# simdjson/simdjson

Hardware: NVIDIA H100
Metric: stage1 GB/s (bytes in / s) vs HBM roofline at 1/2/4/8 H100; CPU ref GB/s (higher is better)
Workload: dtype u8

## Files before the change

include/sjb200.h:

```cpp
#ifndef SJB200_H
#define SJB200_H

#include <stddef.h>
#include <stdint.h>

#if defined(__GNUC__)
#define SJB200_API __attribute__((visibility("default")))
#else
#define SJB200_API
#endif

#ifdef __cplusplus
extern "C" {
#endif

enum {
  SJB200_SUCCESS = 0,
  SJB200_CAPACITY = 1,
  SJB200_MEMALLOC = 2,
  SJB200_UTF8_ERROR = 11,
  SJB200_EMPTY = 13,
  SJB200_UNESCAPED_CHARS = 14,
  SJB200_UNCLOSED_STRING = 15,
  SJB200_UNSUPPORTED_ARCHITECTURE = 16,
  SJB200_UNEXPECTED_ERROR = 24
};

enum {
  SJB200_REGULAR = 0,
  SJB200_STREAMING_PARTIAL = 1,
  SJB200_STREAMING_FINAL = 2,
  SJB200_JSON_SEQUENCE_PARTIAL = 3,
  SJB200_JSON_SEQUENCE_FINAL = 4,
  SJB200_COMMA_DELIMITED_PARTIAL = 5,
  SJB200_COMMA_DELIMITED_FINAL = 6
};

typedef struct sjb200_ctx sjb200_ctx;

SJB200_API int sjb200_create(int device, size_t capacity_bytes, sjb200_ctx **out);
SJB200_API void sjb200_destroy(sjb200_ctx *ctx);
SJB200_API int sjb200_set_capacity(sjb200_ctx *ctx, size_t capacity_bytes);
SJB200_API size_t sjb200_capacity(const sjb200_ctx *ctx);
SJB200_API size_t sjb200_index_words(size_t capacity_bytes);
SJB200_API int sjb200_device(const sjb200_ctx *ctx);
SJB200_API const char *sjb200_last_cuda_error(const sjb200_ctx *ctx);
SJB200_API int sjb200_set_option(sjb200_ctx *ctx, const char *key, long value);
SJB200_API double sjb200_get_stat(sjb200_ctx *ctx, const char *key);

SJB200_API long sjb200_get_debug_timeline(sjb200_ctx *ctx, unsigned long long *out, size_t max_tiles);

SJB200_API int sjb200_pin_host_memory(sjb200_ctx *ctx, void *ptr, size_t bytes);
SJB200_API int sjb200_unpin_host_memory(sjb200_ctx *ctx, void *ptr);

SJB200_API int sjb200_stage1(sjb200_ctx *ctx, const uint8_t *buf, size_t len, int mode, uint32_t *idx_out, uint32_t *n_inout);
SJB200_API int sjb200_minify(sjb200_ctx *ctx, const uint8_t *buf, size_t len, uint8_t *dst, size_t *dst_len);
SJB200_API int sjb200_validate_utf8(sjb200_ctx *ctx, const uint8_t *buf, size_t len);

SJB200_API int sjb200_stage1_dev(sjb200_ctx *ctx, const uint8_t *d_buf, size_t len, int mode, uint32_t *d_idx, uint32_t *n_inout,
                      void *stream);
SJB200_API int sjb200_minify_dev(sjb200_ctx *ctx, const uint8_t *d_buf, size_t len, uint8_t *d_dst, size_t *dst_len, void *stream);
SJB200_API int sjb200_validate_utf8_dev(sjb200_ctx *ctx, const uint8_t *d_buf, size_t len, void *stream);

typedef struct {
  const uint8_t *d_buf;
  size_t len;
  uint32_t *d_idx;
  uint32_t n_structural_indexes;
  int error;
} sjb200_doc;
SJB200_API int sjb200_stage1_dev_batch(sjb200_ctx *ctx, sjb200_doc *docs, int ndocs, int mode, void *stream);

typedef struct {
  uint32_t index;
  uint32_t byte;
} sjb200_doc_boundary;
SJB200_API int sjb200_document_table_dev(sjb200_ctx *ctx, const uint8_t *d_buf, const uint32_t *d_idx, uint32_t n, sjb200_doc_boundary *d_table,
                              uint32_t capacity, uint32_t *ndocs_out, void *stream);

typedef struct {
  int error;
  uint32_t first_error_index;
  uint32_t n_strings;
  uint64_t string_bytes;
} sjb200_tokens_result;
SJB200_API size_t sjb200_string_buf_capacity(size_t len);
SJB200_API int sjb200_tokens_dev(sjb200_ctx *ctx, const uint8_t *d_buf, size_t len, const uint32_t *d_idx, uint32_t n, uint8_t *d_type, uint64_t *d_payload,
                      uint8_t *d_strbuf, size_t strbuf_capacity, sjb200_tokens_result *out, void *stream);

SJB200_API int sjb200_stage1_dev_enqueue(sjb200_ctx *ctx, const uint8_t *d_buf, size_t len, int mode, uint32_t *d_idx, void *stream);
SJB200_API int sjb200_stage1_dev_finish(sjb200_ctx *ctx, uint32_t *n_inout);
SJB200_API int sjb200_minify_dev_enqueue(sjb200_ctx *ctx, const uint8_t *d_buf, size_t len, uint8_t *d_dst, void *stream);
SJB200_API int sjb200_minify_dev_finish(sjb200_ctx *ctx, size_t *dst_len);
SJB200_API int sjb200_validate_utf8_dev_enqueue(sjb200_ctx *ctx, const uint8_t *d_buf, size_t len, void *stream);
SJB200_API int sjb200_validate_utf8_dev_finish(sjb200_ctx *ctx);

typedef struct {
  uint32_t ttable;
  uint32_t state_out;
  uint32_t flags;
  uint32_t reserved;
  uint64_t count;
} sjb200_shard_result;
SJB200_API int sjb200_stage1_shard_dev(sjb200_ctx *ctx, const uint8_t *d_buf, size_t len, uint32_t state_in, int last_shard,
                            uint32_t *d_idx, sjb200_shard_result *out, void *stream);
SJB200_API int sjb200_stage1_shard_dev_enqueue(sjb200_ctx *ctx, const uint8_t *d_buf, size_t len, uint32_t *d_idx, void *d_result,
                                    void *stream);
typedef struct sjb200_comm sjb200_comm;
#define SJB200_COMM_HANDLE_BYTES 64
typedef struct {
  uint64_t count;
  uint64_t base;
  uint64_t total_count;
  uint32_t state_in;
  uint32_t state_out;
  uint32_t final_state;
  uint32_t flags;
  uint32_t flags_all;
  uint32_t rescanned;
} sjb200_sharded_result;
SJB200_API int sjb200_comm_create(sjb200_ctx *ctx, int rank, int nranks , sjb200_comm **out);
SJB200_API void sjb200_comm_destroy(sjb200_comm *comm);
SJB200_API int sjb200_comm_get_handle(sjb200_comm *comm, void *handle );
SJB200_API int sjb200_comm_connect(sjb200_comm *comm, const void *handles );
SJB200_API int sjb200_comm_connect_local(sjb200_comm *comm, sjb200_comm *const *all );
SJB200_API int sjb200_stage1_sharded(sjb200_comm *comm, const uint8_t *d_shard, size_t len, int last_shard, uint32_t *d_idx,
                          sjb200_sharded_result *out, void *stream);
SJB200_API int sjb200_stage1_sharded_enqueue(sjb200_comm *comm, const uint8_t *d_shard, size_t len, int last_shard, uint32_t *d_idx,
                                  void *stream);
SJB200_API int sjb200_stage1_sharded_finish(sjb200_comm *comm, sjb200_sharded_result *out);

SJB200_API int sjb200_minify_sharded_enqueue(sjb200_comm *comm, const uint8_t *d_shard, size_t len, uint8_t *d_dst, void *stream);
SJB200_API int sjb200_minify_sharded_finish(sjb200_comm *comm, sjb200_sharded_result *out);
SJB200_API int sjb200_minify_sharded(sjb200_comm *comm, const uint8_t *d_shard, size_t len, uint8_t *d_dst, sjb200_sharded_result *out,
                          void *stream);
SJB200_API int sjb200_validate_utf8_sharded_enqueue(sjb200_comm *comm, const uint8_t *d_shard, size_t len, void *stream);
SJB200_API int sjb200_validate_utf8_sharded_finish(sjb200_comm *comm, sjb200_sharded_result *out);
SJB200_API int sjb200_validate_utf8_sharded(sjb200_comm *comm, const uint8_t *d_shard, size_t len, sjb200_sharded_result *out, void *stream);

typedef struct {
  sjb200_sharded_result shard;
  uint64_t n;
  uint64_t kept;
  uint64_t bytes_before;
  uint64_t total_bytes;
  uint32_t first_starts_document;
  uint32_t reserved;
} sjb200_sharded_stream_result;
SJB200_API int sjb200_stage1_sharded_stream_enqueue(sjb200_comm *comm, const uint8_t *d_shard, size_t len, int last_shard, int mode, uint32_t *d_idx,
                                         void *stream);
SJB200_API int sjb200_stage1_sharded_stream_finish(sjb200_comm *comm, sjb200_sharded_stream_result *out);
SJB200_API int sjb200_stage1_sharded_stream(sjb200_comm *comm, const uint8_t *d_shard, size_t len, int last_shard, int mode, uint32_t *d_idx,
                                 sjb200_sharded_stream_result *out, void *stream);

SJB200_API int sjb200_document_table_shard_dev(sjb200_ctx *ctx, const uint8_t *d_shard, const uint32_t *d_idx, uint32_t kept, int first_starts_document,
                                    sjb200_doc_boundary *d_table, uint32_t capacity, uint32_t *ndocs_out, void *stream);

typedef struct {
  uint64_t count;
  uint32_t len;
  uint32_t first_byte;
  uint32_t last_byte;
  uint32_t start_index;
  uint32_t start_byte;
  int32_t net_obj;
  int32_t net_arr;
  uint32_t role_first;
  uint32_t role_last;
  uint32_t has_start;
} sjb200_stream_summary;
typedef struct {
  uint64_t kept;
  uint64_t bytes_before;
  uint32_t first_starts_document;
  uint32_t nrewrites;
  uint32_t rewrite_pos[2];
  uint32_t rewrite_val[2];
} sjb200_stream_rank;
typedef struct {
  int error;
  uint32_t n_written;
  uint64_t n;
  uint64_t total_bytes;
} sjb200_stream_fold_result;
SJB200_API int sjb200_stream_fold(int mode, int nranks, uint32_t final_state, uint32_t flags_all, const sjb200_stream_summary *sums,
                       sjb200_stream_fold_result *res, sjb200_stream_rank *ranks );

SJB200_API uint32_t sjb200_fold_state(const uint32_t *ttables, int nshards_before);
SJB200_API size_t sjb200_shard_cut(const uint8_t *buf, size_t len, size_t nominal);
SJB200_API size_t sjb200_shard_cut_line(const uint8_t *buf, size_t len, size_t nominal, size_t window);

#ifdef __cplusplus
}
#endif
#endif
```

simdjson_b200/capi.py:

```python
import ctypes as C
import os

_HERE = os.path.dirname(os.path.abspath(__file__))
LIB_PATH = os.environ.get("SJB200_LIB") or os.path.join(_HERE, "libsjb200.so")

EXPORTS = [
    "sjb200_create", "sjb200_destroy", "sjb200_set_capacity", "sjb200_capacity", "sjb200_index_words", "sjb200_device",
    "sjb200_last_cuda_error", "sjb200_set_option", "sjb200_get_stat", "sjb200_pin_host_memory", "sjb200_unpin_host_memory", "sjb200_get_debug_timeline",
    "sjb200_stage1", "sjb200_minify", "sjb200_validate_utf8",
    "sjb200_stage1_dev", "sjb200_minify_dev", "sjb200_validate_utf8_dev", "sjb200_stage1_dev_batch",
    "sjb200_document_table_dev", "sjb200_stage1_dev_enqueue", "sjb200_stage1_dev_finish", "sjb200_minify_dev_enqueue", "sjb200_minify_dev_finish",
    "sjb200_validate_utf8_dev_enqueue", "sjb200_validate_utf8_dev_finish",
    "sjb200_stage1_shard_dev", "sjb200_stage1_shard_dev_enqueue", "sjb200_fold_state", "sjb200_shard_cut", "sjb200_shard_cut_line",
    "sjb200_comm_create", "sjb200_comm_destroy", "sjb200_comm_get_handle", "sjb200_comm_connect", "sjb200_comm_connect_local",
    "sjb200_stage1_sharded", "sjb200_stage1_sharded_enqueue", "sjb200_stage1_sharded_finish",
    "sjb200_minify_sharded", "sjb200_minify_sharded_enqueue", "sjb200_minify_sharded_finish",
    "sjb200_validate_utf8_sharded", "sjb200_validate_utf8_sharded_enqueue", "sjb200_validate_utf8_sharded_finish",
    "sjb200_tokens_dev", "sjb200_string_buf_capacity",
    "sjb200_stage1_sharded_stream", "sjb200_stage1_sharded_stream_enqueue", "sjb200_stage1_sharded_stream_finish",
    "sjb200_document_table_shard_dev", "sjb200_stream_fold",
]
COMM_HANDLE_BYTES = 64

SUCCESS, CAPACITY, MEMALLOC, UTF8_ERROR, EMPTY, UNESCAPED_CHARS, UNCLOSED_STRING, UNSUPPORTED_ARCHITECTURE, UNEXPECTED_ERROR = 0, 1, 2, 11, 13, 14, 15, 16, 24
ERROR_NAMES = {0: "SUCCESS", 1: "CAPACITY", 2: "MEMALLOC", 3: "TAPE_ERROR", 5: "STRING_ERROR", 6: "T_ATOM_ERROR", 7: "F_ATOM_ERROR", 8: "N_ATOM_ERROR",
               9: "NUMBER_ERROR", 10: "BIGINT_ERROR", 11: "UTF8_ERROR", 13: "EMPTY", 14: "UNESCAPED_CHARS", 15: "UNCLOSED_STRING",
               16: "UNSUPPORTED_ARCHITECTURE", 24: "UNEXPECTED_ERROR"}

REGULAR, STREAMING_PARTIAL, STREAMING_FINAL, JSON_SEQUENCE_PARTIAL, JSON_SEQUENCE_FINAL, COMMA_DELIMITED_PARTIAL, COMMA_DELIMITED_FINAL = range(7)


class Doc(C.Structure):
    _fields_ = [("d_buf", C.c_void_p), ("len", C.c_size_t), ("d_idx", C.c_void_p), ("n_structural_indexes", C.c_uint32), ("error", C.c_int)]


class TokensResult(C.Structure):
    _fields_ = [("error", C.c_int), ("first_error_index", C.c_uint32), ("n_strings", C.c_uint32), ("string_bytes", C.c_uint64)]


class ShardResult(C.Structure):
    _fields_ = [("ttable", C.c_uint32), ("state_out", C.c_uint32), ("flags", C.c_uint32), ("reserved", C.c_uint32), ("count", C.c_uint64)]


class ShardedResult(C.Structure):
    _fields_ = [("count", C.c_uint64), ("base", C.c_uint64), ("total_count", C.c_uint64), ("state_in", C.c_uint32), ("state_out", C.c_uint32),
                ("final_state", C.c_uint32), ("flags", C.c_uint32), ("flags_all", C.c_uint32), ("rescanned", C.c_uint32)]


class ShardedStreamResult(C.Structure):
    _fields_ = [("shard", ShardedResult), ("n", C.c_uint64), ("kept", C.c_uint64), ("bytes_before", C.c_uint64), ("total_bytes", C.c_uint64),
                ("first_starts_document", C.c_uint32), ("reserved", C.c_uint32)]


class StreamSummary(C.Structure):
    _fields_ = [("count", C.c_uint64), ("len", C.c_uint32), ("first_byte", C.c_uint32), ("last_byte", C.c_uint32), ("start_index", C.c_uint32),
                ("start_byte", C.c_uint32), ("net_obj", C.c_int32), ("net_arr", C.c_int32), ("role_first", C.c_uint32), ("role_last", C.c_uint32),
                ("has_start", C.c_uint32)]


class StreamRank(C.Structure):
    _fields_ = [("kept", C.c_uint64), ("bytes_before", C.c_uint64), ("first_starts_document", C.c_uint32), ("nrewrites", C.c_uint32),
                ("rewrite_pos", C.c_uint32 * 2), ("rewrite_val", C.c_uint32 * 2)]


class StreamFoldResult(C.Structure):
    _fields_ = [("error", C.c_int), ("n_written", C.c_uint32), ("n", C.c_uint64), ("total_bytes", C.c_uint64)]


def load():
    if not os.path.exists(LIB_PATH):
        raise ImportError(
            f"{LIB_PATH} is missing: build it with `python -c 'import __graft_entry__ as g; g.build()'` "
            "(nvcc, sm_90a).  simdjson_b200 has no CPU fallback.")
    L = C.CDLL(LIB_PATH)
    u8p, u32p, vp, sz = C.POINTER(C.c_uint8), C.POINTER(C.c_uint32), C.c_void_p, C.c_size_t
    sig = {
        "sjb200_create": (C.c_int, [C.c_int, sz, C.POINTER(vp)]),
        "sjb200_destroy": (None, [vp]),
        "sjb200_set_capacity": (C.c_int, [vp, sz]),
        "sjb200_capacity": (sz, [vp]),
        "sjb200_index_words": (sz, [sz]),
        "sjb200_device": (C.c_int, [vp]),
        "sjb200_last_cuda_error": (C.c_char_p, [vp]),
        "sjb200_set_option": (C.c_int, [vp, C.c_char_p, C.c_long]),
        "sjb200_get_stat": (C.c_double, [vp, C.c_char_p]),
        "sjb200_get_debug_timeline": (C.c_long, [vp, vp, sz]),
        "sjb200_pin_host_memory": (C.c_int, [vp, vp, sz]),
        "sjb200_unpin_host_memory": (C.c_int, [vp, vp]),
        "sjb200_stage1": (C.c_int, [vp, vp, sz, C.c_int, vp, u32p]),
        "sjb200_minify": (C.c_int, [vp, vp, sz, vp, C.POINTER(sz)]),
        "sjb200_validate_utf8": (C.c_int, [vp, vp, sz]),
        "sjb200_stage1_dev": (C.c_int, [vp, vp, sz, C.c_int, vp, u32p, vp]),
        "sjb200_minify_dev": (C.c_int, [vp, vp, sz, vp, C.POINTER(sz), vp]),
        "sjb200_validate_utf8_dev": (C.c_int, [vp, vp, sz, vp]),
        "sjb200_stage1_dev_batch": (C.c_int, [vp, C.POINTER(Doc), C.c_int, C.c_int, vp]),
        "sjb200_document_table_dev": (C.c_int, [vp, vp, vp, C.c_uint32, vp, C.c_uint32, u32p, vp]),
        "sjb200_stage1_dev_enqueue": (C.c_int, [vp, vp, sz, C.c_int, vp, vp]),
        "sjb200_stage1_dev_finish": (C.c_int, [vp, u32p]),
        "sjb200_minify_dev_enqueue": (C.c_int, [vp, vp, sz, vp, vp]),
        "sjb200_minify_dev_finish": (C.c_int, [vp, C.POINTER(sz)]),
        "sjb200_validate_utf8_dev_enqueue": (C.c_int, [vp, vp, sz, vp]),
        "sjb200_validate_utf8_dev_finish": (C.c_int, [vp]),
        "sjb200_stage1_shard_dev": (C.c_int, [vp, vp, sz, C.c_uint32, C.c_int, vp, C.POINTER(ShardResult), vp]),
        "sjb200_stage1_shard_dev_enqueue": (C.c_int, [vp, vp, sz, vp, vp, vp]),
        "sjb200_fold_state": (C.c_uint32, [u32p, C.c_int]),
        "sjb200_shard_cut": (sz, [vp, sz, sz]),
        "sjb200_shard_cut_line": (sz, [vp, sz, sz, sz]),
        "sjb200_comm_create": (C.c_int, [vp, C.c_int, C.c_int, C.POINTER(vp)]),
        "sjb200_comm_destroy": (None, [vp]),
        "sjb200_comm_get_handle": (C.c_int, [vp, vp]),
        "sjb200_comm_connect": (C.c_int, [vp, vp]),
        "sjb200_comm_connect_local": (C.c_int, [vp, C.POINTER(vp)]),
        "sjb200_stage1_sharded": (C.c_int, [vp, vp, sz, C.c_int, vp, C.POINTER(ShardedResult), vp]),
        "sjb200_stage1_sharded_enqueue": (C.c_int, [vp, vp, sz, C.c_int, vp, vp]),
        "sjb200_stage1_sharded_finish": (C.c_int, [vp, C.POINTER(ShardedResult)]),
        "sjb200_minify_sharded": (C.c_int, [vp, vp, sz, vp, C.POINTER(ShardedResult), vp]),
        "sjb200_minify_sharded_enqueue": (C.c_int, [vp, vp, sz, vp, vp]),
        "sjb200_minify_sharded_finish": (C.c_int, [vp, C.POINTER(ShardedResult)]),
        "sjb200_validate_utf8_sharded": (C.c_int, [vp, vp, sz, C.POINTER(ShardedResult), vp]),
        "sjb200_validate_utf8_sharded_enqueue": (C.c_int, [vp, vp, sz, vp]),
        "sjb200_validate_utf8_sharded_finish": (C.c_int, [vp, C.POINTER(ShardedResult)]),
        "sjb200_tokens_dev": (C.c_int, [vp, vp, sz, vp, C.c_uint32, vp, vp, vp, sz, C.POINTER(TokensResult), vp]),
        "sjb200_string_buf_capacity": (sz, [sz]),
        "sjb200_stage1_sharded_stream": (C.c_int, [vp, vp, sz, C.c_int, C.c_int, vp, C.POINTER(ShardedStreamResult), vp]),
        "sjb200_stage1_sharded_stream_enqueue": (C.c_int, [vp, vp, sz, C.c_int, C.c_int, vp, vp]),
        "sjb200_stage1_sharded_stream_finish": (C.c_int, [vp, C.POINTER(ShardedStreamResult)]),
        "sjb200_document_table_shard_dev": (C.c_int, [vp, vp, vp, C.c_uint32, C.c_int, vp, C.c_uint32, u32p, vp]),
        "sjb200_stream_fold": (C.c_int, [C.c_int, C.c_int, C.c_uint32, C.c_uint32, C.POINTER(StreamSummary), C.POINTER(StreamFoldResult),
                                         C.POINTER(StreamRank)]),
    }
    for name, (res, args) in sig.items():
        fn = getattr(L, name)
        fn.restype = res
        fn.argtypes = args
    _ = u8p
    return L
```

simdjson_b200/csrc/sjb200_capi.cu:

```cuda
#include <cuda.h>
#include <cuda_runtime.h>
#include <ctype.h>
#include <stdint.h>
#include <stdlib.h>
#include <string.h>

#include <algorithm>
#include <chrono>
#include <new>
#include <string>
#include <vector>

#include "../../include/sjb200.h"
#include "sjb200_bits.cuh"
#include "sjb200_docs.h"
#include "sjb200_tape.h"
#include "sjb200_finish.h"
#include "sjb200_hostpipe.h"
#include "sjb200_kernels.cuh"

using namespace sjb200;

namespace {

typedef CUresult (*PFN_encodeTiled)(CUtensorMap *, CUtensorMapDataType, cuuint32_t, void *, const cuuint64_t *, const cuuint64_t *,
                                    const cuuint32_t *, const cuuint32_t *, CUtensorMapInterleave, CUtensorMapSwizzle,
                                    CUtensorMapL2promotion, CUtensorMapFloatOOBfill);

constexpr int kCarrySlots = 1024;
constexpr size_t kMaxBytes = 0xFFFFFFFFull;

struct PendingCall {
  int kind = -1;
  int mode = 0;
  int early_error = -1;
  size_t len = 0;
  const uint8_t *d_buf = nullptr;
  uint32_t *d_idx = nullptr;
  uint8_t *d_dst = nullptr;
  cudaStream_t stream = nullptr;
  int carry_slot = 0;
};

}

struct sjb200_ctx {
  int device = 0;
  int sm_count = 0;
  size_t capacity = 0;
  cudaStream_t stream = nullptr;
  cudaStream_t copy_stream = nullptr;
  cudaStream_t out_stream = nullptr;
  std::vector<cudaEvent_t> chunk_events;
  uint8_t *d_in = nullptr;    size_t d_in_bytes = 0;
  uint32_t *d_idx = nullptr;  size_t d_idx_words = 0;
  uint8_t *d_out = nullptr;   size_t d_out_bytes = 0;
  Carry *d_carry = nullptr;
  uint32_t *d_flags = nullptr;
  uint32_t *d_ticket = nullptr;
  unsigned long long *d_count_desc = nullptr;
  size_t desc_tiles = 0;
  StreamFinish *d_sfin = nullptr;
  uint32_t *d_doc_scratch = nullptr; size_t doc_scratch_words = 0; uint32_t *d_ndocs = nullptr;
  void *d_tok_scratch = nullptr; size_t tok_scratch_bytes = 0; TokenTotals *d_tok_tot = nullptr;
  uint32_t *d_park = nullptr; size_t d_park_words = 0;
  int grid_u = 0;
  Carry *h_carry = nullptr;
  uint32_t *h_flags = nullptr;
  uint8_t *h_small = nullptr;
  StreamFinish *h_sfin = nullptr;
  uint8_t *h_tails = nullptr; uint8_t *d_tails = nullptr; const uint8_t **d_tail_ptrs = nullptr; size_t tails_cap = 0;
  uint32_t epoch = 0;
  int grid4 = 0;
  long opt_tok_stage = 1;
  long opt_use_tma = 1, opt_grid = 0, opt_chunk_bytes = 4 << 20, opt_time_kernel = 0;
  cudaEvent_t ev_k0 = nullptr, ev_k1 = nullptr;
  bool ev_valid = false;
  std::vector<cudaEvent_t> ev_pool;
  std::vector<uint32_t> ev_docs;
  size_t ev_used = 0;
  uint32_t ev_last_docs = 1;
  uint8_t *h_doctab = nullptr; uint8_t *d_doctab = nullptr; size_t doctab_bytes = 0;
  long opt_debug_timeline = 0;
  unsigned long long *d_debug = nullptr; size_t debug_tiles = 0; uint32_t debug_last_tiles = 0;
  unsigned long long launches = 0;
  unsigned long long ew_launches = 0;
  PFN_encodeTiled encode = nullptr;
  uint8_t *h_ring = nullptr; size_t ring_slot_bytes = 0; int ring_slots = 0;
  std::vector<cudaEvent_t> ring_events;
  CopyPool *pool = nullptr;
  long opt_force_grid = 0;
  long opt_ew_min_bytes = 0;
  long opt_host_skip_scan = 0;
  long opt_copy_threads = 4;
  long opt_ring_slots = 8;
  long opt_first_chunk_bytes = 512 << 10;
  long opt_stage_min_bytes = 1 << 20;
  long opt_zero_copy_out = 1;
  unsigned long long xchg_polls = 0, xchg_second_rounds = 0;
  double xchg_wait_ms = 0, xchg_evsync_ms = 0, xchg_enqueue_ms = 0;
  double t_wait_ms = 0, t_issue_ms = 0, t_sync_ms = 0;
  int last_input_path = 0, last_output_path = 0;
  PendingCall pending;
  std::string last_error;
};

namespace {

struct DeviceGuard {
  int prev = -1;
  explicit DeviceGuard(int dev) {
    cudaGetDevice(&prev);
    if (prev != dev) cudaSetDevice(dev);
  }
  ~DeviceGuard() {
    int cur = -1;
    cudaGetDevice(&cur);
    if (prev >= 0 && cur != prev) cudaSetDevice(prev);
  }
};

bool ok(sjb200_ctx *c, cudaError_t e, const char *what) {
  if (e == cudaSuccess) return true;
  c->last_error = std::string(what) + ": " + cudaGetErrorString(e);
  (void)cudaGetLastError();
  return false;
}

size_t index_words(size_t capacity) { return ((capacity + 63) / 64) * 64 + 9; }
uint32_t tiles_of(size_t len) { return uint32_t((len + kTileBytes - 1) / kTileBytes); }

template <typename T>
bool dev_alloc(sjb200_ctx *c, T **p, size_t count, const char *what) {
  void *q = nullptr;
  if (!ok(c, cudaMalloc(&q, count * sizeof(T)), what)) return false;
  *p = static_cast<T *>(q);
  return true;
}

void free_sized(sjb200_ctx *c) {
  cudaFree(c->d_in); c->d_in = nullptr; c->d_in_bytes = 0;
  cudaFree(c->d_idx); c->d_idx = nullptr; c->d_idx_words = 0;
  cudaFree(c->d_out); c->d_out = nullptr; c->d_out_bytes = 0;
  cudaFree(c->d_count_desc); c->d_count_desc = nullptr;
  c->desc_tiles = 0;
}

bool ensure_desc_n(sjb200_ctx *c, size_t need) {
  need = std::max<size_t>(need, 1);
  if (need <= c->desc_tiles) return true;
  cudaFree(c->d_count_desc); c->d_count_desc = nullptr;
  c->desc_tiles = 0;
  const size_t n = std::max(need, size_t(tiles_of(c->capacity)) + 1);
  if (!dev_alloc(c, &c->d_count_desc, n, "cudaMalloc(count_desc)")) return false;
  if (!ok(c, cudaMemsetAsync(c->d_count_desc, 0, n * sizeof(unsigned long long), c->stream), "memset desc")) return false;
  if (!ok(c, cudaStreamSynchronize(c->stream), "sync")) return false;
  c->desc_tiles = n;
  c->epoch = 0;
  return true;
}
bool ensure_desc(sjb200_ctx *c, size_t len) { return ensure_desc_n(c, tiles_of(len)); }

bool next_epoch(sjb200_ctx *c, cudaStream_t launch_stream, uint32_t *epoch) {
  c->epoch++;
  if (c->epoch >= (1u << 18)) {
    if (!ok(c, cudaMemsetAsync(c->d_count_desc, 0, c->desc_tiles * sizeof(unsigned long long), launch_stream), "memset desc")) return false;
    c->epoch = 1;
  }
  *epoch = c->epoch;
  return true;
}

bool make_tensor_map(sjb200_ctx *c, CUtensorMap *map, const uint8_t *d_buf, size_t len, bool *usable, int box_rows = kScan4BoxRows) {
  memset(map, 0, sizeof(*map));
  *usable = false;
  const uint64_t rows = len / 128;
  if (!c->opt_use_tma || c->encode == nullptr || rows == 0) return true;
  if ((reinterpret_cast<uintptr_t>(d_buf) & 15u) != 0) return true;
  cuuint64_t dims[2] = {128, rows};
  cuuint64_t strides[1] = {128};
  cuuint32_t box[2] = {128, (cuuint32_t)box_rows};
  cuuint32_t estr[2] = {1, 1};
  CUresult r = c->encode(map, CU_TENSOR_MAP_DATA_TYPE_UINT8, 2, const_cast<uint8_t *>(d_buf), dims, strides, box, estr,
                         CU_TENSOR_MAP_INTERLEAVE_NONE, CU_TENSOR_MAP_SWIZZLE_128B, CU_TENSOR_MAP_L2_PROMOTION_L2_256B,
                         CU_TENSOR_MAP_FLOAT_OOB_FILL_NONE);
  if (r != CUDA_SUCCESS) {
    c->last_error = "cuTensorMapEncodeTiled failed (" + std::to_string(int(r)) + "); using plain loads";
    return true;
  }
  *usable = true;
  return true;
}

bool use_scan4(const sjb200_ctx *, int kind) { return kind == kIndex || kind == kMinify; }
bool map_for(sjb200_ctx *c, int kind, CUtensorMap *map, const uint8_t *d_buf, size_t len, bool *usable) {
  (void)kind;
  return make_tensor_map(c, map, d_buf, len, usable, kScan4BoxRows);
}
int grid_cap(sjb200_ctx *c, int kind) {
  (void)kind;
  if (c->grid4 == 0) c->grid4 = scan4_max_ctas_per_sm() * c->sm_count;
  return c->opt_grid > 0 ? int(c->opt_grid) : c->grid4;
}
int grid_for(sjb200_ctx *c, int kind, uint32_t nelements) {
  if (c->opt_force_grid > 0) return int(c->opt_force_grid);
  return int(std::max<uint32_t>(1, std::min<uint32_t>(uint32_t(grid_cap(c, kind)), nelements)));
}

struct XchgTarget {
  unsigned long long *peer[kMaxRanks];
  uint32_t nranks, rank, slot, seq, kind;
};

cudaEvent_t time_begin(sjb200_ctx *c, cudaStream_t stream) {
  if (!c->opt_time_kernel) return nullptr;
  if (c->ev_used + 2 > c->ev_pool.size() && c->ev_pool.size() < 4096) {
    cudaEvent_t a, b;
    cudaEventCreate(&a); cudaEventCreate(&b);
    c->ev_pool.push_back(a); c->ev_pool.push_back(b);
    c->ev_docs.push_back(1);
  }
  if (c->ev_used + 2 > c->ev_pool.size()) return nullptr;
  cudaEventRecord(c->ev_pool[c->ev_used], stream);
  c->ev_used += 2;
  return c->ev_pool[c->ev_used - 1];
}
void time_end(sjb200_ctx *c, cudaStream_t stream, cudaEvent_t e1, bool launched, uint32_t docs) {
  if (!e1) return;
  cudaEventRecord(e1, stream);
  c->ev_docs[c->ev_used / 2 - 1] = docs;
  c->ev_k0 = c->ev_pool[c->ev_used - 2]; c->ev_k1 = e1; c->ev_valid = launched; c->ev_last_docs = docs;
}

bool enqueue_scan(sjb200_ctx *c, int kind, const CUtensorMap *map, bool tma, const uint8_t *d_buf, size_t len, uint32_t tile_begin,
                  uint32_t ntiles, bool has_last_tile, uint32_t prev_word, uint32_t *d_idx, uint8_t *d_dst, int carry_in_slot,
                  cudaStream_t stream, int carry_out_slot = -1, bool write_sentinels = false, Carry *external_out = nullptr,
                  Carry *host_out = nullptr, const XchgTarget *xchg = nullptr) {
  if (carry_out_slot < 0) carry_out_slot = (carry_in_slot < 0) ? 1 : (carry_in_slot ^ 1);
  ScanParams p;
  memset(&p, 0, sizeof(p));
  p.buf = d_buf;
  p.len = len;
  p.pos_base = 0;
  p.prev_word = prev_word;
  p.check_eof = has_last_tile ? 1u : 0u;
  p.use_tma = tma ? 1u : 0u;
  p.tile_begin = tile_begin;
  p.ntiles = ntiles;
  if (!next_epoch(c, stream, &p.epoch)) return false;
  p.idx_out = d_idx;
  p.dst = d_dst;
  p.carry_in = (carry_in_slot < 0) ? nullptr : c->d_carry + carry_in_slot;
  p.write_sentinels = write_sentinels ? 1u : 0u;
  p.carry_out = external_out ? external_out : c->d_carry + carry_out_slot;
  p.carry_out_host = use_scan4(c, kind) ? host_out : nullptr;
  p.flags = c->d_flags;
  p.count_desc = c->d_count_desc;
  p.ticket = c->d_ticket;
  if (xchg) {
    for (int r = 0; r < kMaxRanks; r++) p.xchg_peer[r] = xchg->peer[r];
    p.xchg_nranks = xchg->nranks; p.xchg_rank = xchg->rank; p.xchg_slot = xchg->slot; p.xchg_seq = xchg->seq; p.xchg_kind = xchg->kind;
  }
  p.debug = nullptr;
  if (c->opt_debug_timeline) {
    const uint32_t rows = std::max<uint32_t>(ntiles, 4096);
    if (c->debug_tiles < rows) {
      cudaFree(c->d_debug); c->d_debug = nullptr; c->debug_tiles = 0;
      if (dev_alloc(c, &c->d_debug, size_t(rows) * 8, "cudaMalloc(debug)")) c->debug_tiles = rows;
    }
    if (c->d_debug) { cudaMemsetAsync(c->d_debug, 0, size_t(rows) * 64, stream); p.debug = c->d_debug; c->debug_last_tiles = rows; }
  }
  cudaEvent_t e1 = time_begin(c, stream);
  bool launched;
  if (use_scan4(c, kind)) {
    const uint32_t tpe = uint32_t(scan4_tiles_per_element());
    const uint32_t nelem = (ntiles + tpe - 1) / tpe;
    const int grid = grid_for(c, kind, nelem);
    const bool ew = kind == kIndex && c->opt_ew_min_bytes > 0 && uint64_t(ntiles) * kTileBytes >= uint64_t(c->opt_ew_min_bytes);
    if (ew || scan4_parks_in_global()) {
      const size_t need = std::max(ew ? scan4_ew_park_words(grid_cap(c, kind)) : 0, scan4_parks_in_global() ? scan4_park_words(grid_cap(c, kind)) : 0);
      if (c->d_park_words < need) {
        cudaStreamSynchronize(c->stream);
        cudaFree(c->d_park); c->d_park = nullptr; c->d_park_words = 0;
        if (!dev_alloc(c, &c->d_park, need, "cudaMalloc(park)")) return false;
        c->d_park_words = need;
      }
      p.park = c->d_park;
    }
    launched = ew ? ok(c, launch_scan4_ew(map, p, grid, stream), "launch scan4 (emit warps)") : ok(c, launch_scan4(map, p, grid, kind == kMinify ? 2 : 0, stream), "launch scan4");
    c->ew_launches += (launched && ew) ? 1 : 0;
  } else {
    if (c->grid_u == 0) c->grid_u = utf8v2_max_ctas_per_sm() * c->sm_count;
    const uint64_t nblocks = (uint64_t(ntiles) * kTileBytes + 4095) / 4096;
    const uint64_t want = (nblocks + uint64_t(utf8v2_warps_per_cta()) - 1) / uint64_t(utf8v2_warps_per_cta());
    const int grid = c->opt_force_grid > 0 ? int(c->opt_force_grid) : int(std::max<uint64_t>(1, std::min<uint64_t>(uint64_t(c->opt_grid > 0 ? c->opt_grid : c->grid_u), want)));
    p.carry_out_host = host_out;
    launched = ok(c, launch_utf8v2(map, p, grid, stream), "launch utf8v2");
  }
  time_end(c, stream, e1, launched, 1);
  c->launches += launched ? 1 : 0;
  return launched;
}

class NullIndexWriter final : public IndexWriter {
 public:
  bool set3(uint32_t, uint32_t, uint32_t, uint32_t) override { return false; }
  bool final_fixup(uint32_t, uint32_t) override { return false; }
};
class NullReader final : public StructuralReader {
 public:
  uint32_t position(uint32_t) override { return 0; }
  uint8_t character(uint32_t) override { return 0; }
};

bool is_filter_mode(int mode) { return mode >= SJB200_JSON_SEQUENCE_PARTIAL; }

bool fetch_result(sjb200_ctx *c, cudaStream_t s) {
  return ok(c, cudaMemcpyAsync(c->h_carry + 1, c->d_carry + 1, sizeof(Carry), cudaMemcpyDeviceToHost, s), "D2H result");
}

}

extern "C" size_t sjb200_index_words(size_t capacity) { return index_words(capacity); }

extern "C" int sjb200_create(int device, size_t capacity, sjb200_ctx **out) {
  if (!out) return SJB200_UNEXPECTED_ERROR;
  *out = nullptr;
  int ndev = 0;
  if (cudaGetDeviceCount(&ndev) != cudaSuccess || device < 0 || device >= ndev) {
    (void)cudaGetLastError();
    return SJB200_UNSUPPORTED_ARCHITECTURE;
  }
  cudaDeviceProp prop;
  if (cudaGetDeviceProperties(&prop, device) != cudaSuccess || prop.major != 9 || prop.minor != 0) {
    (void)cudaGetLastError();
    return SJB200_UNSUPPORTED_ARCHITECTURE;
  }
  sjb200_ctx *c = new (std::nothrow) sjb200_ctx();
  if (!c) return SJB200_MEMALLOC;
  c->device = device;
  c->sm_count = prop.multiProcessorCount;
  DeviceGuard g(device);
  bool good = ok(c, cudaStreamCreateWithFlags(&c->stream, cudaStreamNonBlocking), "stream") &&
              ok(c, cudaStreamCreateWithFlags(&c->copy_stream, cudaStreamNonBlocking), "stream") &&
              ok(c, cudaStreamCreateWithFlags(&c->out_stream, cudaStreamNonBlocking), "stream") &&
              dev_alloc(c, &c->d_carry, kCarrySlots, "cudaMalloc(carry)") && dev_alloc(c, &c->d_flags, 1 + kCarrySlots, "cudaMalloc(flags)") &&
              dev_alloc(c, &c->d_ticket, 4, "cudaMalloc(ticket)") &&
              ok(c, cudaMemset(c->d_ticket, 0, 4 * sizeof(uint32_t)), "memset ticket") &&
              ok(c, cudaMemset(c->d_flags, 0, (1 + kCarrySlots) * sizeof(uint32_t)), "memset flags");
  void *hp = nullptr;
  good = good && ok(c, cudaMallocHost(&hp, kCarrySlots * sizeof(Carry)), "cudaMallocHost");
  c->h_carry = static_cast<Carry *>(hp);
  good = good && ok(c, cudaMallocHost(&hp, sizeof(uint32_t)), "cudaMallocHost");
  c->h_flags = static_cast<uint32_t *>(hp);
  good = good && ok(c, cudaMallocHost(&hp, 64), "cudaMallocHost");
  c->h_small = static_cast<uint8_t *>(hp);
  good = good && ok(c, cudaMallocHost(&hp, kCarrySlots * sizeof(StreamFinish)), "cudaMallocHost");
  c->h_sfin = static_cast<StreamFinish *>(hp);
  good = good && dev_alloc(c, &c->d_sfin, kCarrySlots, "cudaMalloc(stream finish)") && dev_alloc(c, &c->d_ndocs, 1, "cudaMalloc(ndocs)");
  if (good) {
    void *fn = nullptr;
    cudaDriverEntryPointQueryResult qres;
    if (cudaGetDriverEntryPoint("cuTensorMapEncodeTiled", &fn, cudaEnableDefault, &qres) == cudaSuccess &&
        qres == cudaDriverEntryPointSuccess)
      c->encode = reinterpret_cast<PFN_encodeTiled>(fn);
    else
      (void)cudaGetLastError();
  }
  if (!good) {
    sjb200_destroy(c);
    return SJB200_MEMALLOC;
  }
  for (const char *key : {"copy_threads", "ring_slots", "chunk_bytes", "first_chunk_bytes", "stage_min_bytes", "zero_copy_out"}) {
    std::string env = std::string("SJB200_") + key;
    for (auto &ch : env) ch = char(toupper((unsigned char)ch));
    if (const char *v = getenv(env.c_str())) sjb200_set_option(c, key, atol(v));
  }
  int rc = sjb200_set_capacity(c, capacity);
  if (rc != SJB200_SUCCESS) {
    sjb200_destroy(c);
    return rc;
  }
  *out = c;
  return SJB200_SUCCESS;
}

extern "C" void sjb200_destroy(sjb200_ctx *c) {
  if (!c) return;
  DeviceGuard g(c->device);
  if (c->stream) cudaStreamSynchronize(c->stream);
  free_sized(c);
  cudaFree(c->d_carry); cudaFree(c->d_flags); cudaFree(c->d_ticket); cudaFree(c->d_sfin); cudaFree(c->d_doc_scratch); cudaFree(c->d_ndocs); cudaFree(c->d_tok_scratch); cudaFree(c->d_tok_tot); cudaFree(c->d_tails); cudaFree(c->d_tail_ptrs); cudaFree(c->d_debug); cudaFree(c->d_park); cudaFree(c->d_doctab);
  if (c->h_doctab) cudaFreeHost(c->h_doctab);
  if (c->h_carry) cudaFreeHost(c->h_carry);
  if (c->h_flags) cudaFreeHost(c->h_flags);
  if (c->h_small) cudaFreeHost(c->h_small);
  if (c->h_sfin) cudaFreeHost(c->h_sfin);
  if (c->h_tails) cudaFreeHost(c->h_tails);
  delete c->pool; c->pool = nullptr;
  if (c->h_ring) cudaFreeHost(c->h_ring);
  for (auto e : c->ring_events) cudaEventDestroy(e);
  for (auto e : c->ev_pool) cudaEventDestroy(e);
  for (auto e : c->chunk_events) cudaEventDestroy(e);
  if (c->stream) cudaStreamDestroy(c->stream);
  if (c->copy_stream) cudaStreamDestroy(c->copy_stream);
  if (c->out_stream) cudaStreamDestroy(c->out_stream);
  delete c;
}

extern "C" int sjb200_set_capacity(sjb200_ctx *c, size_t capacity) {
  if (!c) return SJB200_UNEXPECTED_ERROR;
  if (capacity > kMaxBytes) return SJB200_CAPACITY;
  DeviceGuard g(c->device);
  if (capacity != c->capacity) {
    cudaStreamSynchronize(c->stream);
    free_sized(c);
  }
  c->capacity = capacity;
  if (!ensure_desc(c, capacity)) return SJB200_MEMALLOC;
  return SJB200_SUCCESS;
}

extern "C" size_t sjb200_capacity(const sjb200_ctx *c) { return c ? c->capacity : 0; }
extern "C" int sjb200_device(const sjb200_ctx *c) { return c ? c->device : -1; }
extern "C" const char *sjb200_last_cuda_error(const sjb200_ctx *c) { return c ? c->last_error.c_str() : ""; }

extern "C" long sjb200_get_debug_timeline(sjb200_ctx *c, unsigned long long *out, size_t max_tiles) {
  if (!c || !c->d_debug || !out) return 0;
  DeviceGuard g(c->device);
  const size_t n = std::min<size_t>(max_tiles, c->debug_last_tiles);
  cudaDeviceSynchronize();
  if (cudaMemcpy(out, c->d_debug, n * 64, cudaMemcpyDeviceToHost) != cudaSuccess) { (void)cudaGetLastError(); return 0; }
  return long(n);
}

extern "C" int sjb200_pin_host_memory(sjb200_ctx *c, void *ptr, size_t bytes) {
  if (!c || !ptr || bytes == 0) return SJB200_UNEXPECTED_ERROR;
  DeviceGuard g(c->device);
  return ok(c, cudaHostRegister(ptr, bytes, cudaHostRegisterPortable | cudaHostRegisterMapped), "cudaHostRegister") ? SJB200_SUCCESS : SJB200_MEMALLOC;
}
extern "C" int sjb200_unpin_host_memory(sjb200_ctx *c, void *ptr) {
  if (!c || !ptr) return SJB200_UNEXPECTED_ERROR;
  DeviceGuard g(c->device);
  return ok(c, cudaHostUnregister(ptr), "cudaHostUnregister") ? SJB200_SUCCESS : SJB200_UNEXPECTED_ERROR;
}

extern "C" double sjb200_get_stat(sjb200_ctx *c, const char *key) {
  if (!c || !key) return -1.0;
  if (!strcmp(key, "kernel_ms")) {
    if (!c->ev_valid) return -1.0;
    DeviceGuard g(c->device);
    float ms = 0.f;
    if (cudaEventElapsedTime(&ms, c->ev_k0, c->ev_k1) != cudaSuccess) { (void)cudaGetLastError(); return -1.0; }
    return double(ms) / double(c->ev_last_docs);
  }
  if (!strcmp(key, "kernel_ms_mean")) {
    DeviceGuard g(c->device);
    double sum = 0;
    size_t n = 0;
    for (size_t i = 0; i + 1 < c->ev_used; i += 2) {
      float ms = 0.f;
      if (cudaEventElapsedTime(&ms, c->ev_pool[i], c->ev_pool[i + 1]) == cudaSuccess) { sum += ms; n += c->ev_docs[i / 2]; } else (void)cudaGetLastError();
    }
    c->ev_used = 0;
    c->ev_valid = false;
    return n ? sum / double(n) : -1.0;
  }
  if (!strcmp(key, "launches")) return double(c->launches);
  if (!strcmp(key, "ew_launches")) return double(c->ew_launches);
  if (!strcmp(key, "grid_index")) return double(grid_for(c, kIndex, 0xFFFFFFFFu));
  if (!strcmp(key, "sm_count")) return double(c->sm_count);
  if (!strcmp(key, "host_wait_ms")) return c->t_wait_ms;
  if (!strcmp(key, "xchg_polls")) return double(c->xchg_polls);
  if (!strcmp(key, "xchg_second_rounds")) return double(c->xchg_second_rounds);
  if (!strcmp(key, "xchg_wait_ms")) return c->xchg_wait_ms;
  if (!strcmp(key, "xchg_evsync_ms")) return c->xchg_evsync_ms;
  if (!strcmp(key, "xchg_enqueue_ms")) return c->xchg_enqueue_ms;
  if (!strcmp(key, "host_issue_ms")) return c->t_issue_ms;
  if (!strcmp(key, "host_sync_ms")) return c->t_sync_ms;
  if (!strcmp(key, "input_path")) return double(c->last_input_path);
  if (!strcmp(key, "output_path")) return double(c->last_output_path);
  return -1.0;
}

extern "C" int sjb200_set_option(sjb200_ctx *c, const char *key, long value) {
  if (!c || !key) return SJB200_UNEXPECTED_ERROR;
  if (!strcmp(key, "use_tma")) c->opt_use_tma = value;
  else if (!strcmp(key, "grid")) c->opt_grid = value;
  else if (!strcmp(key, "tok_stage")) c->opt_tok_stage = value ? 1 : 0;
  else if (!strcmp(key, "time_kernel")) c->opt_time_kernel = value;
  else if (!strcmp(key, "debug_timeline")) c->opt_debug_timeline = value;
  else if (!strcmp(key, "chunk_bytes")) c->opt_chunk_bytes = std::max<long>(2 * kTileBytes, (value / (2 * kTileBytes)) * (2 * kTileBytes));
  else if (!strcmp(key, "force_grid")) c->opt_force_grid = value;
  else if (!strcmp(key, "ew_min_bytes")) c->opt_ew_min_bytes = value;
  else if (!strcmp(key, "host_skip_scan")) c->opt_host_skip_scan = value;
  else if (!strcmp(key, "copy_threads")) c->opt_copy_threads = std::max<long>(0, std::min<long>(value, 64));
  else if (!strcmp(key, "ring_slots")) c->opt_ring_slots = std::max<long>(2, std::min<long>(value, 64));
  else if (!strcmp(key, "stage_min_bytes")) c->opt_stage_min_bytes = std::max<long>(0, value);
  else if (!strcmp(key, "first_chunk_bytes")) c->opt_first_chunk_bytes = std::max<long>(2 * kTileBytes, (value / (2 * kTileBytes)) * (2 * kTileBytes));
  else if (!strcmp(key, "zero_copy_out")) c->opt_zero_copy_out = value;
  else return SJB200_UNEXPECTED_ERROR;
  return SJB200_SUCCESS;
}

namespace {
bool stage1_prepare(sjb200_ctx *c, PendingCall &pc, const uint8_t *d_buf, size_t len, int mode, uint32_t *d_idx, cudaStream_t s, int slot,
                    const uint8_t *tail3 ) {
  pc = PendingCall();
  pc.kind = kIndex; pc.mode = mode; pc.d_buf = d_buf; pc.d_idx = d_idx; pc.stream = s; pc.len = len; pc.carry_slot = slot;
  if (mode < SJB200_REGULAR || mode > SJB200_COMMA_DELIMITED_FINAL) { pc.early_error = SJB200_UNEXPECTED_ERROR; return false; }
  if (len > c->capacity) { pc.early_error = SJB200_CAPACITY; return false; }
  if (len == 0) { pc.early_error = SJB200_EMPTY; return false; }
  if (mode != SJB200_REGULAR) {
    const size_t k = std::min<size_t>(3, len);
    if (!tail3) {
      if (!ok(c, cudaMemcpyAsync(c->h_small, d_buf + len - k, k, cudaMemcpyDeviceToHost, s), "D2H tail") ||
          !ok(c, cudaStreamSynchronize(s), "sync"))
        { pc.early_error = SJB200_UNEXPECTED_ERROR; return false; }
      tail3 = c->h_small;
    }
    len = trim_partial_utf8_tail(tail3, k, len);
    pc.len = len;
    if (len == 0) { pc.early_error = SJB200_UTF8_ERROR; return false; }
  }
  return true;
}

void stage1_stream_epilogue(sjb200_ctx *c, PendingCall &pc) {
  if (pc.mode == SJB200_STREAMING_PARTIAL || pc.mode == SJB200_STREAMING_FINAL) {
    c->launches++;
    const int slot = pc.carry_slot;
    if (!ok(c, launch_stream_finish(pc.d_buf, pc.d_idx, c->d_carry + slot, uint32_t(pc.len), pc.mode, c->d_sfin + slot, c->h_sfin + slot, pc.stream), "stream finish"))
      pc.early_error = SJB200_UNEXPECTED_ERROR;
  }
}

void stage1_enqueue_into(sjb200_ctx *c, PendingCall &pc, const uint8_t *d_buf, size_t len, int mode, uint32_t *d_idx, cudaStream_t s, int slot) {
  if (!stage1_prepare(c, pc, d_buf, len, mode, d_idx, s, slot, nullptr)) return;
  len = pc.len;
  if (!ensure_desc(c, len)) { pc.early_error = SJB200_MEMALLOC; return; }
  CUtensorMap map;
  bool tma = false;
  map_for(c, kIndex, &map, d_buf, len, &tma);
  if (!enqueue_scan(c, kIndex, &map, tma, d_buf, len, 0, tiles_of(len), true, 0x20202020u, d_idx, nullptr, -1, s, slot, true, nullptr,
                    c->h_carry + slot) ||
      (!use_scan4(c, kIndex) &&
       !ok(c, cudaMemcpyAsync(c->h_carry + slot, c->d_carry + slot, sizeof(Carry), cudaMemcpyDeviceToHost, s), "D2H result")))
    { pc.early_error = SJB200_UNEXPECTED_ERROR; return; }
  stage1_stream_epilogue(c, pc);
}

int stage1_finish_from(sjb200_ctx *c, const PendingCall &pc, uint32_t *n_inout) {
  if (pc.early_error >= 0) return pc.early_error;
  if (pc.mode == SJB200_STREAMING_PARTIAL || pc.mode == SJB200_STREAMING_FINAL) {
    const StreamFinish &r = c->h_sfin[pc.carry_slot];
    if (r.n_written && n_inout) *n_inout = r.n;
    return r.err;
  }
  FinishInput in;
  in.mode = pc.mode; in.len = pc.len;
  in.count = c->h_carry[pc.carry_slot].count;
  in.state = c->h_carry[pc.carry_slot].state;
  in.flags = c->h_carry[pc.carry_slot].flags;
  in.sentinels_written = true;
  int rc;
  uint32_t n_local = n_inout ? *n_inout : 0;
  if (is_filter_mode(pc.mode)) {
    if (in.flags & kFlagInternal) return SJB200_UNEXPECTED_ERROR;
    if (in.flags & kFlagCtl) return SJB200_UNESCAPED_CHARS;
    uint32_t n = uint32_t(in.count);
    n_local = n;
    if (n == 0) { if (n_inout) *n_inout = 0; return SJB200_EMPTY; }
    const bool unclosed = (in.state >> 1) & 1u;
    const bool partial = (pc.mode == SJB200_JSON_SEQUENCE_PARTIAL || pc.mode == SJB200_COMMA_DELIMITED_PARTIAL);
    if (unclosed) {
      n--;
      if (partial) { n_local = n; if (n == 0) { if (n_inout) *n_inout = 0; return SJB200_CAPACITY; } }
    }
    const size_t need = filter_scratch_words(n);
    if (c->doc_scratch_words < need) {
      cudaFree(c->d_doc_scratch); c->d_doc_scratch = nullptr; c->doc_scratch_words = 0;
      if (!dev_alloc(c, &c->d_doc_scratch, need, "cudaMalloc(filter scratch)")) return SJB200_MEMALLOC;
      c->doc_scratch_words = need;
    }
    c->launches += 4;
    if (!ok(c, launch_stream_filter(pc.d_buf, uint32_t(pc.len), pc.d_idx, n, pc.mode, in.flags, c->d_doc_scratch, c->d_sfin + pc.carry_slot,
                                    c->h_sfin + pc.carry_slot, pc.stream), "stream filter") ||
        !ok(c, cudaStreamSynchronize(pc.stream), "sync"))
      return SJB200_UNEXPECTED_ERROR;
    const StreamFinish &r = c->h_sfin[pc.carry_slot];
    if (n_inout) *n_inout = r.n;
    return r.err;
  } else {
    NullReader reader;
    NullIndexWriter writer;
    bool dirty = false;
    rc = finish_stage1(in, reader, writer, &n_local, nullptr, nullptr, &dirty);
  }
  if (n_inout) *n_inout = n_local;
  return rc;
}

}

extern "C" int sjb200_stage1_dev_enqueue(sjb200_ctx *c, const uint8_t *d_buf, size_t len, int mode, uint32_t *d_idx, void *stream) {
  if (!c) return SJB200_UNEXPECTED_ERROR;
  DeviceGuard g(c->device);
  stage1_enqueue_into(c, c->pending, d_buf, len, mode, d_idx, stream ? static_cast<cudaStream_t>(stream) : c->stream, 1);
  return SJB200_SUCCESS;
}

extern "C" int sjb200_stage1_dev_finish(sjb200_ctx *c, uint32_t *n_inout) {
  if (!c || c->pending.kind != kIndex) return SJB200_UNEXPECTED_ERROR;
  DeviceGuard g(c->device);
  PendingCall pc = c->pending;
  c->pending.kind = -1;
  if (pc.early_error < 0 && !ok(c, cudaStreamSynchronize(pc.stream), "sync")) return SJB200_UNEXPECTED_ERROR;
  return stage1_finish_from(c, pc, n_inout);
}

namespace {
bool ranges_overlap(const void *a, size_t an, const void *b, size_t bn) {
  const uintptr_t x = reinterpret_cast<uintptr_t>(a), y = reinterpret_cast<uintptr_t>(b);
  return x < y + bn && y < x + an;
}
size_t out_bytes(const PendingCall &pc) { return 4 * (pc.len + 3); }

int enqueue_doc_groups(sjb200_ctx *c, std::vector<PendingCall> &calls, cudaStream_t s) {
  constexpr uint64_t kMaxGroupElems = 1u << 20;
  const uint32_t tpe = uint32_t(scan4_tiles_per_element());
  auto elems_of = [&](const PendingCall &pc) { return uint64_t((tiles_of(pc.len) + tpe - 1) / tpe); };
  std::vector<std::vector<int>> groups;
  uint64_t g_elems = 0, max_elems = 0;
  for (int i = 0; i < int(calls.size()); i++) {
    const PendingCall &pc = calls[size_t(i)];
    if (pc.early_error >= 0) continue;
    bool split = groups.empty() || groups.back().size() == size_t(kMaxLaunchDocs) || g_elems + elems_of(pc) > kMaxGroupElems;
    for (size_t k = 0; !split && k < groups.back().size(); k++) {
      const PendingCall &q = calls[size_t(groups.back()[k])];
      split = ranges_overlap(pc.d_buf, pc.len, q.d_idx, out_bytes(q)) || ranges_overlap(pc.d_idx, out_bytes(pc), q.d_idx, out_bytes(q)) ||
              ranges_overlap(pc.d_idx, out_bytes(pc), q.d_buf, q.len);
    }
    if (split) { groups.emplace_back(); g_elems = 0; }
    groups.back().push_back(i);
    g_elems += elems_of(pc);
    max_elems = std::max(max_elems, g_elems);
  }
  if (groups.empty()) return SJB200_SUCCESS;
  if (!ensure_desc_n(c, max_elems)) return SJB200_MEMALLOC;
  std::vector<size_t> off(groups.size() + 1, 0);
  for (size_t g = 0; g < groups.size(); g++) {
    const size_t n = groups[g].size() > 1 ? groups[g].size() : 0;
    off[g + 1] = off[g] + ((n * sizeof(DocEntry) + 127) & ~size_t(127)) + n * sizeof(CUtensorMap);
  }
  if (off.back() > c->doctab_bytes) {
    if (c->h_doctab) cudaFreeHost(c->h_doctab);
    cudaFree(c->d_doctab);
    c->h_doctab = nullptr; c->d_doctab = nullptr; c->doctab_bytes = 0;
    void *hp = nullptr;
    if (!ok(c, cudaMallocHost(&hp, off.back()), "cudaMallocHost(doc tables)") || !dev_alloc(c, &c->d_doctab, off.back(), "cudaMalloc(doc tables)"))
      return SJB200_MEMALLOC;
    c->h_doctab = static_cast<uint8_t *>(hp);
    c->doctab_bytes = off.back();
  }
  static_assert(sizeof(DocEntry) == 64 && sizeof(CUtensorMap) == 128, "table layout");
  for (size_t g = 0; g < groups.size(); g++) {
    const std::vector<int> &G = groups[g];
    if (G.size() == 1) {
      PendingCall &pc = calls[size_t(G[0])];
      CUtensorMap map;
      bool tma = false;
      map_for(c, kIndex, &map, pc.d_buf, pc.len, &tma);
      if (!enqueue_scan(c, kIndex, &map, tma, pc.d_buf, pc.len, 0, tiles_of(pc.len), true, 0x20202020u, pc.d_idx, nullptr, -1, s, pc.carry_slot, true,
                        nullptr, c->h_carry + pc.carry_slot))
        pc.early_error = SJB200_UNEXPECTED_ERROR;
      else
        stage1_stream_epilogue(c, pc);
      continue;
    }
    const size_t n = G.size();
    DocEntry *he = reinterpret_cast<DocEntry *>(c->h_doctab + off[g]);
    const size_t maps_at = off[g] + ((n * sizeof(DocEntry) + 127) & ~size_t(127));
    CUtensorMap *hm = reinterpret_cast<CUtensorMap *>(c->h_doctab + maps_at);
    const CUtensorMap *dm = reinterpret_cast<const CUtensorMap *>(c->d_doctab + maps_at);
    uint32_t elems = 0, tiles = 0;
    for (size_t k = 0; k < n; k++) {
      const PendingCall &pc = calls[size_t(G[k])];
      bool tma = false;
      map_for(c, kIndex, &hm[k], pc.d_buf, pc.len, &tma);
      DocEntry &e = he[k];
      e.buf = pc.d_buf;
      e.idx_out = pc.d_idx;
      e.carry_out = c->d_carry + pc.carry_slot;
      e.carry_out_host = c->h_carry + pc.carry_slot;
      e.flags = c->d_flags + 1 + pc.carry_slot;
      e.tmap = tma ? static_cast<const void *>(dm + k) : nullptr;
      e.len = uint32_t(pc.len);
      e.scan_end = uint32_t(pc.len);
      e.first_elem = elems;
      e.nelem = uint32_t(elems_of(pc));
      elems += e.nelem;
      tiles += tiles_of(pc.len);
    }
    ScanParams p;
    memset(&p, 0, sizeof(p));
    p.prev_word = 0x20202020u;
    p.check_eof = 1;
    p.write_sentinels = 1;
    p.ntiles = tiles;
    p.flags = c->d_flags;
    p.count_desc = c->d_count_desc;
    p.ticket = c->d_ticket;
    p.docs = reinterpret_cast<const DocEntry *>(c->d_doctab + off[g]);
    p.ndocs = uint32_t(n);
    bool good = next_epoch(c, s, &p.epoch) &&
                ok(c, cudaMemcpyAsync(c->d_doctab + off[g], c->h_doctab + off[g], off[g + 1] - off[g], cudaMemcpyHostToDevice, s), "H2D doc table");
    if (good) {
      CUtensorMap unused;
      memset(&unused, 0, sizeof(unused));
      cudaEvent_t e1 = time_begin(c, s);
      good = ok(c, launch_scan4(&unused, p, grid_for(c, kIndex, elems), 0, s), "launch scan4 (documents)");
      time_end(c, s, e1, good, uint32_t(n));
      c->launches += good ? 1 : 0;
    }
    for (size_t k = 0; k < n; k++) {
      PendingCall &pc = calls[size_t(G[k])];
      if (good) stage1_stream_epilogue(c, pc);
      else pc.early_error = SJB200_UNEXPECTED_ERROR;
    }
  }
  return SJB200_SUCCESS;
}
}

extern "C" int sjb200_stage1_dev_batch(sjb200_ctx *c, sjb200_doc *docs, int ndocs, int mode, void *stream) {
  if (!c || (!docs && ndocs > 0) || ndocs < 0) return SJB200_UNEXPECTED_ERROR;
  DeviceGuard g(c->device);
  cudaStream_t s = stream ? static_cast<cudaStream_t>(stream) : c->stream;
  std::vector<PendingCall> calls;
  int done = 0;
  while (done < ndocs) {
    const int group = std::min(ndocs - done, kCarrySlots - 2);
    calls.assign(size_t(group), PendingCall());
    const uint8_t *tails = nullptr;
    if (mode != SJB200_REGULAR) {
      if (c->tails_cap < size_t(group)) {
        if (c->h_tails) cudaFreeHost(c->h_tails);
        cudaFree(c->d_tails); cudaFree(c->d_tail_ptrs);
        c->h_tails = nullptr; c->d_tails = nullptr; c->d_tail_ptrs = nullptr; c->tails_cap = 0;
        void *hp = nullptr;
        if (!ok(c, cudaMallocHost(&hp, size_t(group) * 20), "cudaMallocHost(tails)") || !dev_alloc(c, &c->d_tails, size_t(group) * 4, "cudaMalloc(tails)") ||
            !dev_alloc(c, &c->d_tail_ptrs, size_t(group) * 2, "cudaMalloc(tail ptrs)"))
          return SJB200_MEMALLOC;
        c->h_tails = static_cast<uint8_t *>(hp);
        c->tails_cap = size_t(group);
      }
      const uint8_t **hptr = reinterpret_cast<const uint8_t **>(c->h_tails);
      uint64_t *hlen = reinterpret_cast<uint64_t *>(c->h_tails + size_t(group) * 8);
      uint8_t *hout = c->h_tails + size_t(group) * 16;
      for (int i = 0; i < group; i++) { hptr[i] = docs[done + i].d_buf; hlen[i] = (docs[done + i].len <= c->capacity) ? docs[done + i].len : 0; }
      const uint64_t *dlen = reinterpret_cast<const uint64_t *>(c->d_tail_ptrs + group);
      if (!ok(c, cudaMemcpyAsync(c->d_tail_ptrs, c->h_tails, size_t(group) * 16, cudaMemcpyHostToDevice, s), "H2D tail ptrs") ||
          !ok(c, launch_gather_tails(c->d_tail_ptrs, dlen, uint32_t(group), c->d_tails, s), "gather tails") ||
          !ok(c, cudaMemcpyAsync(hout, c->d_tails, size_t(group) * 4, cudaMemcpyDeviceToHost, s), "D2H tails") || !ok(c, cudaStreamSynchronize(s), "sync"))
        return SJB200_UNEXPECTED_ERROR;
      c->launches++;
      tails = hout;
    }
    for (int i = 0; i < group; i++) {
      sjb200_doc &d = docs[done + i];
      stage1_prepare(c, calls[size_t(i)], d.d_buf, d.len, mode, d.d_idx, s, 1 + i, tails ? tails + 4 * size_t(i) : nullptr);
    }
    const int rc = enqueue_doc_groups(c, calls, s);
    if (rc != SJB200_SUCCESS) return rc;
    if (!ok(c, cudaStreamSynchronize(s), "sync")) return SJB200_UNEXPECTED_ERROR;
    for (int i = 0; i < group; i++) {
      sjb200_doc &d = docs[done + i];
      d.error = stage1_finish_from(c, calls[size_t(i)], &d.n_structural_indexes);
    }
    done += group;
  }
  return SJB200_SUCCESS;
}

extern "C" int sjb200_document_table_dev(sjb200_ctx *c, const uint8_t *d_buf, const uint32_t *d_idx, uint32_t n, sjb200_doc_boundary *d_table,
                                         uint32_t capacity, uint32_t *ndocs_out, void *stream) {
  return sjb200_document_table_shard_dev(c, d_buf, d_idx, n, 1, d_table, capacity, ndocs_out, stream);
}

extern "C" int sjb200_document_table_shard_dev(sjb200_ctx *c, const uint8_t *d_buf, const uint32_t *d_idx, uint32_t n, int first_starts_document,
                                               sjb200_doc_boundary *d_table, uint32_t capacity, uint32_t *ndocs_out, void *stream) {
  if (!c || !d_buf || !d_idx || !ndocs_out || (capacity && !d_table)) return SJB200_UNEXPECTED_ERROR;
  *ndocs_out = 0;
  if (n == 0) return SJB200_SUCCESS;
  DeviceGuard g(c->device);
  cudaStream_t s = stream ? static_cast<cudaStream_t>(stream) : c->stream;
  const size_t need = doc_table_scratch_words(n);
  if (c->doc_scratch_words < need) {
    cudaFree(c->d_doc_scratch); c->d_doc_scratch = nullptr; c->doc_scratch_words = 0;
    if (!dev_alloc(c, &c->d_doc_scratch, need, "cudaMalloc(doc scratch)")) return SJB200_MEMALLOC;
    c->doc_scratch_words = need;
  }
  static_assert(sizeof(sjb200_doc_boundary) == sizeof(sjb200_doc_boundary_t), "layout");
  if (!ok(c, launch_doc_table(d_buf, d_idx, n, first_starts_document != 0, c->d_doc_scratch, reinterpret_cast<sjb200_doc_boundary_t *>(d_table), capacity,
                              c->d_ndocs, s), "doc table") ||
      !ok(c, cudaMemcpyAsync(c->h_small, c->d_ndocs, sizeof(uint32_t), cudaMemcpyDeviceToHost, s), "D2H ndocs") || !ok(c, cudaStreamSynchronize(s), "sync"))
    return SJB200_UNEXPECTED_ERROR;
  c->launches += 3;
  memcpy(ndocs_out, c->h_small, sizeof(uint32_t));
  return SJB200_SUCCESS;
}

extern "C" size_t sjb200_string_buf_capacity(size_t len) { return ((5 * (len / 3) + 64) + 63) / 64 * 64; }

extern "C" int sjb200_tokens_dev(sjb200_ctx *c, const uint8_t *d_buf, size_t len, const uint32_t *d_idx, uint32_t n, uint8_t *d_type, uint64_t *d_payload,
                                 uint8_t *d_strbuf, size_t strbuf_capacity, sjb200_tokens_result *out, void *stream) {
  if (!c || !out || (n && (!d_buf || !d_idx || !d_type || !d_payload)) || (strbuf_capacity && !d_strbuf)) return SJB200_UNEXPECTED_ERROR;
  out->error = SJB200_SUCCESS; out->first_error_index = 0xFFFFFFFFu; out->n_strings = 0; out->string_bytes = 0;
  DeviceGuard g(c->device);
  cudaStream_t s = stream ? static_cast<cudaStream_t>(stream) : c->stream;
  const size_t need = tokens_scratch_bytes(n);
  if (c->tok_scratch_bytes < need) {
    cudaFree(c->d_tok_scratch); c->d_tok_scratch = nullptr; c->tok_scratch_bytes = 0;
    if (cudaMalloc(&c->d_tok_scratch, need) != cudaSuccess) { c->last_error = "cudaMalloc(token scratch)"; return SJB200_MEMALLOC; }
    c->tok_scratch_bytes = need;
  }
  if (!c->d_tok_tot && cudaMalloc(reinterpret_cast<void **>(&c->d_tok_tot), sizeof(TokenTotals)) != cudaSuccess) { c->last_error = "cudaMalloc(token totals)"; return SJB200_MEMALLOC; }
  static_assert(sizeof(TokenTotals) <= 64, "h_small");
  if (!ok(c, launch_tokens(d_buf, len, d_idx, n, d_type, d_payload, d_strbuf, strbuf_capacity, c->d_tok_scratch, c->d_tok_tot, int(c->opt_tok_stage), s), "tokens") ||
      !ok(c, cudaMemcpyAsync(c->h_small, c->d_tok_tot, sizeof(TokenTotals), cudaMemcpyDeviceToHost, s), "D2H token totals") || !ok(c, cudaStreamSynchronize(s), "sync"))
    return SJB200_UNEXPECTED_ERROR;
  c->launches += n ? 3 : 1;
  TokenTotals t;
  memcpy(&t, c->h_small, sizeof(t));
  out->n_strings = t.n_strings;
  out->string_bytes = t.string_bytes;
  if (t.first_error != ~0ull) {
    out->first_error_index = uint32_t(t.first_error >> 8);
    out->error = int(t.first_error & 0xFFull);
  } else if (t.string_bytes > strbuf_capacity) {
    out->error = SJB200_CAPACITY;
  }
  return out->error;
}

extern "C" int sjb200_stage1_dev(sjb200_ctx *c, const uint8_t *d_buf, size_t len, int mode, uint32_t *d_idx, uint32_t *n_inout,
                                 void *stream) {
  int rc = sjb200_stage1_dev_enqueue(c, d_buf, len, mode, d_idx, stream);
  if (rc != SJB200_SUCCESS) return rc;
  return sjb200_stage1_dev_finish(c, n_inout);
}

extern "C" int sjb200_minify_dev_enqueue(sjb200_ctx *c, const uint8_t *d_buf, size_t len, uint8_t *d_dst, void *stream) {
  if (!c) return SJB200_UNEXPECTED_ERROR;
  DeviceGuard g(c->device);
  cudaStream_t s = stream ? static_cast<cudaStream_t>(stream) : c->stream;
  PendingCall &pc = c->pending;
  pc = PendingCall();
  pc.kind = kMinify; pc.d_buf = d_buf; pc.d_dst = d_dst; pc.stream = s; pc.len = len;
  if (len > kMaxBytes) { pc.early_error = SJB200_CAPACITY; return SJB200_SUCCESS; }
  if (len == 0) { pc.early_error = SJB200_SUCCESS; return SJB200_SUCCESS; }
  if (!ensure_desc(c, len)) { pc.early_error = SJB200_MEMALLOC; return SJB200_SUCCESS; }
  CUtensorMap map;
  bool tma = false;
  map_for(c, kMinify, &map, d_buf, len, &tma);
  if (!enqueue_scan(c, kMinify, &map, tma, d_buf, len, 0, tiles_of(len), true, 0x20202020u, nullptr, d_dst, -1, s, 1) ||
      !fetch_result(c, s))
    pc.early_error = SJB200_UNEXPECTED_ERROR;
  pc.carry_slot = 1;
  return SJB200_SUCCESS;
}

extern "C" int sjb200_minify_dev_finish(sjb200_ctx *c, size_t *dst_len) {
  if (!c || c->pending.kind != kMinify) return SJB200_UNEXPECTED_ERROR;
  DeviceGuard g(c->device);
  PendingCall pc = c->pending;
  c->pending.kind = -1;
  if (dst_len) *dst_len = 0;
  if (pc.early_error >= 0) return pc.early_error;
  if (!ok(c, cudaStreamSynchronize(pc.stream), "sync")) return SJB200_UNEXPECTED_ERROR;
  if (c->h_carry[pc.carry_slot].flags & kFlagInternal) return SJB200_UNEXPECTED_ERROR;
  if ((c->h_carry[pc.carry_slot].state >> 1) & 1u) return SJB200_UNCLOSED_STRING;
  if (dst_len) *dst_len = size_t(c->h_carry[pc.carry_slot].count);
  return SJB200_SUCCESS;
}

extern "C" int sjb200_minify_dev(sjb200_ctx *c, const uint8_t *d_buf, size_t len, uint8_t *d_dst, size_t *dst_len, void *stream) {
  int rc = sjb200_minify_dev_enqueue(c, d_buf, len, d_dst, stream);
  if (rc != SJB200_SUCCESS) return rc;
  return sjb200_minify_dev_finish(c, dst_len);
}

extern "C" int sjb200_validate_utf8_dev_enqueue(sjb200_ctx *c, const uint8_t *d_buf, size_t len, void *stream) {
  if (!c) return SJB200_UNEXPECTED_ERROR;
  DeviceGuard g(c->device);
  cudaStream_t s = stream ? static_cast<cudaStream_t>(stream) : c->stream;
  PendingCall &pc = c->pending;
  pc = PendingCall();
  pc.kind = kUtf8; pc.d_buf = d_buf; pc.stream = s; pc.len = len;
  if (len == 0) { pc.early_error = SJB200_SUCCESS; return SJB200_SUCCESS; }
  if (len > kMaxBytes) { pc.early_error = SJB200_CAPACITY; return SJB200_SUCCESS; }
  CUtensorMap map;
  bool tma = false;
  map_for(c, kUtf8, &map, d_buf, len, &tma);
  if (!enqueue_scan(c, kUtf8, &map, tma, d_buf, len, 0, tiles_of(len), true, 0x20202020u, nullptr, nullptr, -1, s, 1) ||
      !fetch_result(c, s))
    pc.early_error = SJB200_UNEXPECTED_ERROR;
  return SJB200_SUCCESS;
}

extern "C" int sjb200_validate_utf8_dev_finish(sjb200_ctx *c) {
  if (!c || c->pending.kind != kUtf8) return -1;
  DeviceGuard g(c->device);
  PendingCall pc = c->pending;
  c->pending.kind = -1;
  if (pc.early_error == SJB200_SUCCESS) return 1;
  if (pc.early_error > 0) return -1;
  if (!ok(c, cudaStreamSynchronize(pc.stream), "sync")) return -1;
  if (c->h_carry[1].flags & kFlagInternal) return -1;
  return (c->h_carry[1].flags & kFlagUtf8) ? 0 : 1;
}

extern "C" int sjb200_validate_utf8_dev(sjb200_ctx *c, const uint8_t *d_buf, size_t len, void *stream) {
  if (sjb200_validate_utf8_dev_enqueue(c, d_buf, len, stream) != SJB200_SUCCESS) return -1;
  return sjb200_validate_utf8_dev_finish(c);
}

namespace {

bool ensure_input(sjb200_ctx *c, size_t len) {
  const size_t need = std::max(len, c->capacity) + 256;
  if (c->d_in_bytes >= need) return true;
  cudaFree(c->d_in); c->d_in = nullptr; c->d_in_bytes = 0;
  if (!dev_alloc(c, &c->d_in, need, "cudaMalloc(input)")) return false;
  c->d_in_bytes = need;
  return true;
}
bool ensure_index(sjb200_ctx *c, size_t len) {
  const size_t need = index_words(std::max(len, c->capacity));
  if (c->d_idx_words >= need) return true;
  cudaFree(c->d_idx); c->d_idx = nullptr; c->d_idx_words = 0;
  if (!dev_alloc(c, &c->d_idx, need, "cudaMalloc(index)")) return false;
  c->d_idx_words = need;
  return true;
}
bool ensure_output(sjb200_ctx *c, size_t len) {
  const size_t need = len + 256;
  if (c->d_out_bytes >= need) return true;
  cudaFree(c->d_out); c->d_out = nullptr; c->d_out_bytes = 0;
  if (!dev_alloc(c, &c->d_out, need, "cudaMalloc(output)")) return false;
  c->d_out_bytes = need;
  return true;
}

bool ensure_ring(sjb200_ctx *c, size_t slot_bytes) {
  const int slots = int(c->opt_ring_slots);
  if (c->h_ring && c->ring_slot_bytes >= slot_bytes && c->ring_slots == slots) return true;
  if (c->h_ring) { cudaFreeHost(c->h_ring); c->h_ring = nullptr; c->ring_slot_bytes = 0; c->ring_slots = 0; }
  void *q = nullptr;
  if (!ok(c, cudaMallocHost(&q, slot_bytes * size_t(slots)), "cudaMallocHost(ring)")) return false;
  c->h_ring = static_cast<uint8_t *>(q);
  c->ring_slot_bytes = slot_bytes;
  c->ring_slots = slots;
  while (c->ring_events.size() < size_t(slots)) {
    cudaEvent_t e;
    if (!ok(c, cudaEventCreateWithFlags(&e, cudaEventDisableTiming), "event")) return false;
    c->ring_events.push_back(e);
  }
  return true;
}
bool ensure_pool(sjb200_ctx *c) {
  if (!c->pool) c->pool = new (std::nothrow) CopyPool();
  return c->pool && c->pool->start(int(c->opt_copy_threads));
}

bool scan_host_document(sjb200_ctx *c, int kind, const uint8_t *buf, size_t len, uint32_t *d_idx, uint8_t *d_dst, void *host_out,
                        size_t elt, bool direct_out, int *final_slot) {
  size_t chunk = size_t(c->opt_chunk_bytes);
  const size_t min_chunk = ((len / (kCarrySlots - 8)) / (2 * kTileBytes) + 1) * (2 * kTileBytes);
  if (chunk < min_chunk) chunk = min_chunk;
  std::vector<size_t> bounds;
  bounds.push_back(0);
  for (size_t c0 = std::min<size_t>(chunk, size_t(c->opt_first_chunk_bytes)); bounds.back() < len;) {
    bounds.push_back(std::min(len, bounds.back() + c0));
    c0 = std::min(chunk, c0 * 2);
  }
  const size_t nchunks = bounds.size() - 1;
  const bool drain = !direct_out && elt != 0 && host_out != nullptr;
  while (c->chunk_events.size() < 2 * nchunks) {
    cudaEvent_t e;
    if (!ok(c, cudaEventCreateWithFlags(&e, cudaEventDisableTiming), "event")) return false;
    c->chunk_events.push_back(e);
  }
  int in_path = 0;
  {
    cudaPointerAttributes attr;
    if (cudaPointerGetAttributes(&attr, buf) == cudaSuccess) {
      if (attr.type == cudaMemoryTypeHost) in_path = 2;
    } else {
      (void)cudaGetLastError();
    }
    if (in_path == 0 && c->opt_copy_threads > 0 && len >= size_t(c->opt_stage_min_bytes) && ensure_ring(c, chunk) && ensure_pool(c)) in_path = 1;
  }
  c->last_input_path = in_path;
  c->last_output_path = direct_out ? 1 : 0;
  CUtensorMap map;
  bool tma = false;
  map_for(c, kind, &map, c->d_in, len, &tma);
  auto launch_chunk = [&](size_t k, const uint8_t *src) -> bool {
    const size_t off = bounds[k];
    const size_t bytes = bounds[k + 1] - off;
    cudaEvent_t copied = c->chunk_events[2 * k], scanned = c->chunk_events[2 * k + 1];
    if (!ok(c, cudaMemcpyAsync(c->d_in + off, src, bytes, cudaMemcpyHostToDevice, c->copy_stream), "H2D chunk") ||
        !ok(c, cudaEventRecord(copied, c->copy_stream), "event record") || !ok(c, cudaStreamWaitEvent(c->stream, copied, 0), "wait event"))
      return false;
    const bool last = (k + 1 == nchunks);
    if (c->opt_host_skip_scan) return true;
    if (!enqueue_scan(c, kind, &map, tma, c->d_in, len, uint32_t(off / kTileBytes), tiles_of(bytes), last, 0x20202020u, d_idx, d_dst,
                      k == 0 ? -1 : int(k), c->stream, int(k + 1), false, nullptr, c->h_carry + k + 1))
      return false;
    if (!use_scan4(c, kind) &&
        !ok(c, cudaMemcpyAsync(c->h_carry + k + 1, c->d_carry + k + 1, sizeof(Carry), cudaMemcpyDeviceToHost, c->stream), "D2H carry"))
      return false;
    return !drain || ok(c, cudaEventRecord(scanned, c->stream), "event record");
  };
  if (in_path == 1) {
    CopyPool &pool = *c->pool;
    const int slots = c->ring_slots;
    pool.begin(buf, bounds.data(), nchunks, c->h_ring, c->ring_slot_bytes, slots);
    pool.allow(size_t(slots));
    size_t issued = 0, released = 0;
    uint32_t idle = 0;
    bool good = true;
// ... 675 lines not shown
```

simdjson_b200/csrc/sjb200_kernels.cu:

```cuda
#include "sjb200_kernels.cuh"

#include "sjb200_bits.cuh"
#include "sjb200_scan4.cuh"
#include "sjb200_utf8.cuh"

namespace sjb200 {

__global__ void __launch_bounds__(scan4::kThreads4, (SJB200_SCAN4_WARPS > 8) ? 1 : SJB200_SCAN4_MIN_CTAS)
    scan4_kernel(const __grid_constant__ CUtensorMap tmap, const ScanParams p) {
  extern __shared__ uint8_t smem_raw4[];
  scan4::scan4_body<0>(&tmap, p, smem_raw4, sj_smem_u32(smem_raw4));
}
__global__ void __launch_bounds__(scan4::kThreads4, (SJB200_SCAN4_WARPS > 8) ? 1 : SJB200_SCAN4_MIN_CTAS)
    scan4_minify_kernel(const __grid_constant__ CUtensorMap tmap, const ScanParams p) {
  extern __shared__ uint8_t smem_raw4[];
  scan4::scan4_body<2>(&tmap, p, smem_raw4, sj_smem_u32(smem_raw4));
}

__global__ void __launch_bounds__(utf8v2::kThreadsU, utf8v2::kCtasPerSmU)
    utf8v2_kernel(const __grid_constant__ CUtensorMap tmap, const ScanParams p) {
  extern __shared__ uint8_t smem_raw_u[];
  utf8v2::utf8_body(&tmap, p, smem_raw_u, sj_smem_u32(smem_raw_u));
}

__global__ void gather_tails_kernel(const uint8_t *const *bufs, const uint64_t *lens, uint32_t ndocs, uint8_t *out) {
  const uint32_t i = blockIdx.x * blockDim.x + threadIdx.x;
  if (i >= ndocs) return;
  const uint64_t len = lens[i];
  const uint32_t k = len < 3 ? uint32_t(len) : 3u;
  for (uint32_t b = 0; b < 4; b++) out[4 * i + b] = (b < k) ? bufs[i][len - k + b] : 0;
}
__global__ void write_sentinels_kernel(uint32_t *idx, uint32_t n, uint32_t a, uint32_t b, uint32_t c) {
  idx[n] = a;
  idx[n + 1] = b;
  idx[n + 2] = c;
}

__global__ void xchg_post_kernel(ScanParams p, unsigned long long w0, unsigned long long w1) {
  const uint32_t r = threadIdx.x;
  if (r < p.xchg_nranks) {
    unsigned long long *rec = p.xchg_peer[r] + (size_t(p.xchg_slot) * kMaxRanks + p.xchg_rank) * 2;
    sj_st_sys_u64(rec, w0);
    sj_st_sys_u64(rec + 1, w1);
  }
}

cudaError_t launch_scan4(const CUtensorMap *tmap, const ScanParams &p, int grid, int mode, cudaStream_t stream) {
  static bool configured[64] = {};
  int dev = 0;
  cudaGetDevice(&dev);
  if (dev < 0 || dev >= 64 || !configured[dev]) {
    cudaError_t e = cudaFuncSetAttribute(scan4_kernel, cudaFuncAttributeMaxDynamicSharedMemorySize, scan4::kSmemBytes4);
    if (e == cudaSuccess) e = cudaFuncSetAttribute(scan4_minify_kernel, cudaFuncAttributeMaxDynamicSharedMemorySize, scan4::kSmemBytes4);
    if (e != cudaSuccess) return e;
    if (dev >= 0 && dev < 64) configured[dev] = true;
  }
  if (mode == 2) scan4_minify_kernel<<<grid, scan4::kThreads4, scan4::kSmemBytes4, stream>>>(*tmap, p);
  else scan4_kernel<<<grid, scan4::kThreads4, scan4::kSmemBytes4, stream>>>(*tmap, p);
  return cudaGetLastError();
}

cudaError_t launch_utf8v2(const CUtensorMap *tmap, const ScanParams &p, int grid, cudaStream_t stream) {
  static bool configured[64] = {};
  int dev = 0;
  cudaGetDevice(&dev);
  if (dev < 0 || dev >= 64 || !configured[dev]) {
    cudaError_t e = cudaFuncSetAttribute(utf8v2_kernel, cudaFuncAttributeMaxDynamicSharedMemorySize, utf8v2::kSmemBytesU);
    if (e != cudaSuccess) return e;
    if (dev >= 0 && dev < 64) configured[dev] = true;
  }
  utf8v2_kernel<<<grid, utf8v2::kThreadsU, utf8v2::kSmemBytesU, stream>>>(*tmap, p);
  return cudaGetLastError();
}
int utf8v2_max_ctas_per_sm() {
  int n = 0;
  cudaFuncSetAttribute(utf8v2_kernel, cudaFuncAttributeMaxDynamicSharedMemorySize, utf8v2::kSmemBytesU);
  cudaError_t e = cudaOccupancyMaxActiveBlocksPerMultiprocessor(&n, utf8v2_kernel, utf8v2::kThreadsU, utf8v2::kSmemBytesU);
  return (e == cudaSuccess && n > 0) ? n : 1;
}
int utf8v2_warps_per_cta() { return utf8v2::kWarpsU; }

size_t scan4_park_words(int grid) { return size_t(grid) * scan4::kParkRing * scan4::kParkSlotWords + 8; }
int scan4_parks_in_global() { return scan4::kGPark > 0 ? 1 : 0; }
int scan4_tiles_per_element() { return scan4::kElemBytes / kTileBytes; }

int scan4_max_ctas_per_sm() {
  int n = 0;
  cudaFuncSetAttribute(scan4_kernel, cudaFuncAttributeMaxDynamicSharedMemorySize, scan4::kSmemBytes4);
  cudaError_t e = cudaOccupancyMaxActiveBlocksPerMultiprocessor(&n, scan4_kernel, scan4::kThreads4, scan4::kSmemBytes4);
  return (e == cudaSuccess && n > 0) ? n : 1;
}

cudaError_t launch_gather_tails(const uint8_t *const *bufs, const uint64_t *lens, uint32_t ndocs, uint8_t *out, cudaStream_t stream) {
  if (ndocs == 0) return cudaSuccess;
  gather_tails_kernel<<<(ndocs + 127) / 128, 128, 0, stream>>>(bufs, lens, ndocs, out);
  return cudaGetLastError();
}

cudaError_t launch_xchg_post(const ScanParams &p, unsigned long long w0, unsigned long long w1, cudaStream_t stream) {
  xchg_post_kernel<<<1, 32, 0, stream>>>(p, w0, w1);
  return cudaGetLastError();
}

cudaError_t launch_write_sentinels(uint32_t *idx, uint32_t n, uint32_t a, uint32_t b, uint32_t c, cudaStream_t stream) {
  write_sentinels_kernel<<<1, 1, 0, stream>>>(idx, n, a, b, c);
  return cudaGetLastError();
}

}
```

simdjson_b200/csrc/sjb200_kernels.cuh:

```cuda
#pragma once
#include <cuda.h>
#include <cuda_runtime.h>
#include <stdint.h>

#include "sjb200_common.h"
#include "sjb200_params.h"

namespace sjb200 {

cudaError_t launch_scan4(const CUtensorMap *tmap, const ScanParams &p, int grid, int mode ,
                         cudaStream_t stream);
size_t scan4_park_words(int grid);
int scan4_tiles_per_element();
int scan4_parks_in_global();
int scan4_max_ctas_per_sm();
cudaError_t launch_scan4_ew(const CUtensorMap *tmap, const ScanParams &p, int grid, cudaStream_t stream);
size_t scan4_ew_park_words(int grid);
constexpr int kScan4BoxRows = 32;
cudaError_t launch_utf8v2(const CUtensorMap *tmap, const ScanParams &p, int grid, cudaStream_t stream);
int utf8v2_max_ctas_per_sm();
int utf8v2_warps_per_cta();
cudaError_t launch_gather_tails(const uint8_t *const *bufs, const uint64_t *lens, uint32_t ndocs, uint8_t *out, cudaStream_t stream);
cudaError_t launch_xchg_post(const ScanParams &p, unsigned long long w0, unsigned long long w1, cudaStream_t stream);
cudaError_t launch_write_sentinels(uint32_t *idx, uint32_t n, uint32_t a, uint32_t b, uint32_t c, cudaStream_t stream);

}
```

simdjson_b200/csrc/sjb200_params.h:

```cpp
#pragma once
#include <stddef.h>
#include <stdint.h>

#include "sjb200_common.h"

namespace sjb200 {

constexpr int kTileBytes = 32 * 1024;
constexpr int kTileRows = kTileBytes / 128;
constexpr int kMaxRanks = 8;
constexpr int kXchgSteps = 64;
#ifndef SJB200_SCAN4_MIN_CTAS
#define SJB200_SCAN4_MIN_CTAS 2
#endif

enum : int { kIndex = 0, kMinify = 1, kUtf8 = 2, kStream = 3 };

struct Carry {
  uint64_t count;
  uint32_t state;
  uint32_t ttable;
  uint32_t flags;
  uint32_t reserved;
};

struct DocEntry {
  const uint8_t *buf;
  uint32_t *idx_out;
  Carry *carry_out;
  Carry *carry_out_host;
  uint32_t *flags;
  const void *tmap;
  uint32_t len;
  uint32_t scan_end;
  uint32_t first_elem;
  uint32_t nelem;
};
constexpr int kMaxLaunchDocs = 64;

struct ScanParams {
  const uint8_t *buf;
  uint64_t len;
  uint32_t pos_base;
  uint32_t prev_word;
  uint32_t check_eof;
  uint32_t use_tma;
  uint32_t tile_begin;
  uint32_t ntiles;
  uint32_t epoch;
  uint32_t *idx_out;
  uint8_t *dst;
  uint32_t write_sentinels;
  const Carry *carry_in;
  Carry *carry_out;
  Carry *carry_out_host;
  uint32_t *flags;
  unsigned long long *count_desc;
  uint32_t *ticket;
  uint32_t *park;
  unsigned long long *debug;
  unsigned long long *xchg_peer[kMaxRanks];
  uint32_t xchg_nranks, xchg_rank, xchg_slot, xchg_seq;
  uint32_t xchg_kind;
  const DocEntry *docs;
  uint32_t ndocs;
};

#if defined(__CUDACC__)
#define SJ_PARAMS_HD __host__ __device__
#else
#define SJ_PARAMS_HD
#endif
SJ_PARAMS_HD inline unsigned long long xchg_word0(uint32_t seq, uint64_t count) {
  return ((unsigned long long)(seq & 0x7FFFFFFFu) << 33) | (count & 0x1FFFFFFFFull);
}
SJ_PARAMS_HD inline unsigned long long xchg_word1(uint32_t seq, uint32_t state, uint32_t ttable, uint32_t flags, int kind) {
  return ((unsigned long long)seq << 32) | ((unsigned long long)(uint32_t(kind) & 3u) << 24) | ((unsigned long long)(flags & 0xFFu) << 16) |
         ((unsigned long long)(ttable & 0x3Fu) << 8) | (state & 7u);
}
SJ_PARAMS_HD inline int xchg_kind(unsigned long long w1) { return int(uint32_t(w1 >> 24) & 3u); }
SJ_PARAMS_HD inline bool xchg_complete(unsigned long long w0, unsigned long long w1, uint32_t seq) {
  return uint32_t(w0 >> 33) == (seq & 0x7FFFFFFFu) && uint32_t(w1 >> 32) == seq;
}
SJ_PARAMS_HD inline uint64_t xchg_count(unsigned long long w0) { return w0 & 0x1FFFFFFFFull; }

constexpr int kSumWords = 8;
constexpr size_t kXchgRecordWords = size_t(kXchgSteps) * 2 * kMaxRanks * 2;
constexpr size_t kXchgWindowWords = kXchgRecordWords + size_t(kXchgSteps) * kMaxRanks * kSumWords;
SJ_PARAMS_HD inline size_t xchg_summary_at(uint32_t seq, uint32_t rank) {
  return kXchgRecordWords + (size_t(seq % uint32_t(kXchgSteps)) * kMaxRanks + rank) * kSumWords;
}

}
```

simdjson_b200/csrc/sjb200_scan4.cuh:

```cuda
#pragma once
#include "sjb200_bits.cuh"
#include "sjb200_params.h"
#include "sjb200_simt.cuh"

namespace sjb200 {
namespace scan4 {

#ifndef SJB200_SCAN4_WARPS
#define SJB200_SCAN4_WARPS 16
#endif
constexpr int kScanWarps = SJB200_SCAN4_WARPS;
constexpr int kBlockBytes = 4096;
constexpr int kBlockRows = kBlockBytes / 128;
constexpr int kChainWarps = 1;
#ifndef SJB200_SCAN4_EMITW
#define SJB200_SCAN4_EMITW 0
#endif
constexpr int kEmitWarps = SJB200_SCAN4_EMITW;
constexpr int kThreads4 = 32 * (kScanWarps + kChainWarps + kEmitWarps);
#ifndef SJB200_SCAN4_PARK
#define SJB200_SCAN4_PARK 3
#endif
constexpr int kPark = SJB200_SCAN4_PARK;
constexpr int kLag = kPark - 1;
constexpr int kNS = 32;
constexpr int kParkSlotWords = 2 * kScanWarps * 32 * 4 + kScanWarps * 32;
#ifndef SJB200_SCAN4_GPARK
#define SJB200_SCAN4_GPARK 8
#endif
constexpr int kGPark = (SJB200_SCAN4_EMITW > 0) ? SJB200_SCAN4_GPARK : 0;
constexpr int kParkRing = (kGPark > 0) ? kGPark : 1;
constexpr int kParkFree = (kGPark > 0) ? kGPark : kPark;
#ifndef SJB200_SCAN4_LOOKK
#define SJB200_SCAN4_LOOKK 10
#endif
constexpr int kLookK = SJB200_SCAN4_LOOKK;
static_assert(kLag >= 1 && 2 * kLag + 3 <= kNS && 2 * kGPark + 4 <= kNS && (kNS & (kNS - 1)) == 0, "slot ring");
#ifndef SJB200_SCAN4_TRACE
#define SJB200_SCAN4_TRACE 0
#endif
constexpr int kTraceIters = 8, kTracePoints = 12;
#if SJB200_SCAN4_TRACE
#define SJ_TRACE4(pt)                                                                                              \
  do {                                                                                                             \
    if (lane == 0 && (warp == 0 || warp == 9) && j < uint32_t(kTraceIters)) S->trace[warp ? 1 : 0][j][pt] = sj_clock32(); \
  } while (0)
#else
#define SJ_TRACE4(pt) do { } while (0)
#endif
constexpr uint32_t kSpinLimit4 = 1u << 21;
constexpr uint32_t kStageWords = kBlockBytes / 4;
constexpr int kElemBytes = kScanWarps * kBlockBytes;
static_assert(kElemBytes % kTileBytes == 0 && kScanWarps <= 16, "an element is a whole number of tiles of the launch parameter block");
SJ_DEV uint32_t elements_of(const ScanParams &p) { return uint32_t((uint64_t(p.ntiles) * kTileBytes + kElemBytes - 1) / kElemBytes); }

enum : uint32_t { kDescNone = 0, kDescAgg = 1, kDescInc = 2 };

struct Smem {
  uint8_t ring[kScanWarps][2][kBlockBytes];
  uint8_t estage[kEmitWarps > 0 ? kEmitWarps : 1][kBlockBytes];
  sj_u4 park[kGPark > 0 ? 1 : kPark][2][kGPark > 0 ? 1 : kScanWarps * 32];
  uint32_t parkpre[kGPark > 0 ? 1 : kPark][kGPark > 0 ? 1 : kScanWarps * 32];
  uint32_t compact_lut[16];
  alignas(16) DocEntry doc[kMaxLaunchDocs];
  uint32_t ndocs;
  uint32_t ticket[kNS];
  uint32_t tdoc[kNS];
  uint32_t summary[kNS][kScanWarps];
  uint32_t arrived[kNS];
  uint32_t elem[kNS][4];
  uint32_t pre[kNS][2][kScanWarps];
  uint32_t res_pol[kNS][kScanWarps];
  uint32_t res_base[kNS][kScanWarps];
  sj_mbar_t full[kScanWarps][2];
  sj_mbar_t ticket_ready[kNS];
  sj_mbar_t scanned[kNS];
  sj_mbar_t resolved[kNS];
  sj_mbar_t efull[kEmitWarps > 0 ? kEmitWarps : 1];
  sj_mbar_t park_free[kParkFree];
  uint32_t emitted_cnt[kNS];
  uint32_t emit_next;
  uint32_t scan_done;
#if SJB200_SCAN4_TRACE
  uint32_t trace[2][kTraceIters][kTracePoints];
  unsigned long long trace_cta[4];
#endif
};
constexpr int kSmemBytes4 = int(sizeof(Smem)) + 1024;

SJ_DEV uint32_t swz(uint32_t off) { return off ^ ((off >> 3) & 0x70u); }

SJ_DEV unsigned long long pack_agg(uint32_t epoch, uint32_t par, uint32_t c0, uint32_t c1) {
  return ((unsigned long long)epoch << 46) | ((unsigned long long)kDescAgg << 44) | ((unsigned long long)(par & 1u) << 38) |
         ((unsigned long long)c1 << 19) | c0;
}
SJ_DEV unsigned long long pack_inc(uint32_t epoch, uint32_t s_out, uint32_t count) {
  return ((unsigned long long)epoch << 46) | ((unsigned long long)kDescInc << 44) | ((unsigned long long)(s_out & 1u) << 32) | count;
}

struct Eff {
  uint32_t p, a, b;
};
SJ_DEV Eff compose(const Eff &o, const Eff &n) {
  Eff r;
  r.p = o.p ^ n.p;
  r.a = o.a + (o.p ? n.b : n.a);
  r.b = o.b + (o.p ? n.a : n.b);
  return r;
}

#ifndef SJB200_SCAN4_POLL_SCALE
#define SJB200_SCAN4_POLL_SCALE 1
#endif
SJ_DEV bool wait_bar(sj_mbar_t *bar, uint32_t parity, const ScanParams &p, unsigned ns) {
  uint32_t spins = 0;
  while (!sj_mbar_try_wait(bar, parity)) {
    if (++spins > kSpinLimit4) {
      sj_atomic_or(p.flags, kFlagInternal);
      return false;
    }
    sj_nanosleep(ns * SJB200_SCAN4_POLL_SCALE);
  }
  return true;
}

SJ_DEV bool byte_is_scalar(uint32_t b) {
  const bool ws = b == 0x20u || b == 0x09u || b == 0x0Au || b == 0x0Du;
  const bool op = b == 0x2Cu || b == 0x3Au || b == 0x5Bu || b == 0x5Du || b == 0x7Bu || b == 0x7Du || b == 0x0Cu || b == 0x1Au;
  return !(ws || op);
}

SJ_DEV uint64_t run_back(const uint8_t *buf, uint64_t end, uint64_t floor, unsigned lane, bool *hit_floor) {
  uint64_t cur = end, total = 0;
  *hit_floor = false;
  uint32_t steps = 0;
  for (;;) {
    if (cur == floor) {
      *hit_floor = true;
      return total;
    }
    if (steps >= 4 && cur - floor >= 512 && ((reinterpret_cast<uintptr_t>(buf) + cur) & 15u) == 0) {
      const sj_u4 v = sj_ldg_u4(buf + cur - 16 * (uint64_t(lane) + 1));
      const bool allbs = (v.x == 0x5C5C5C5Cu) && (v.y == 0x5C5C5C5Cu) && (v.z == 0x5C5C5C5Cu) && (v.w == 0x5C5C5C5Cu);
      const uint32_t m = sj_ballot(!allbs);
      if (m == 0) {
        total += 512;
        cur -= 512;
        continue;
      }
      const uint32_t f = uint32_t(sj_ffs(m) - 1);
      total += 16ull * f;
      cur -= 16ull * f;
    }
    const uint64_t avail64 = cur - floor;
    const uint32_t avail = avail64 < 32 ? uint32_t(avail64) : 32u;
    const bool isbs = lane < avail && sj_ldg_u8(buf + cur - 1 - lane) == 0x5Cu;
    const uint32_t m = sj_ballot(!isbs);
    if (m != 0) {
      const uint32_t f = uint32_t(sj_ffs(m) - 1);
      total += f;
      if (f == avail && avail < 32) *hit_floor = true;
      return total;
    }
    total += 32;
    cur -= 32;
    steps++;
  }
}
SJ_DEV uint64_t run_forward(const uint8_t *buf, uint64_t begin, uint64_t limit, unsigned lane) {
  uint64_t cur = begin, total = 0;
  uint32_t steps = 0;
  for (;;) {
    if (cur >= limit) return total;
    if (steps >= 4 && limit - cur >= 512 && ((reinterpret_cast<uintptr_t>(buf) + cur) & 15u) == 0) {
      const sj_u4 v = sj_ldg_u4(buf + cur + 16 * uint64_t(lane));
      const bool allbs = (v.x == 0x5C5C5C5Cu) && (v.y == 0x5C5C5C5Cu) && (v.z == 0x5C5C5C5Cu) && (v.w == 0x5C5C5C5Cu);
      const uint32_t m = sj_ballot(!allbs);
      if (m == 0) {
        total += 512;
        cur += 512;
        continue;
      }
      const uint32_t f = uint32_t(sj_ffs(m) - 1);
      total += 16ull * f;
      cur += 16ull * f;
    }
    const uint64_t avail64 = limit - cur;
    const uint32_t avail = avail64 < 32 ? uint32_t(avail64) : 32u;
    const bool isbs = lane < avail && sj_ldg_u8(buf + cur + lane) == 0x5Cu;
    const uint32_t m = sj_ballot(!isbs);
    if (m != 0) return total + uint32_t(sj_ffs(m) - 1);
    total += 32;
    cur += 32;
    steps++;
  }
}

SJ_DEV uint32_t boundary_state(const uint8_t *buf, uint64_t pos, uint64_t launch_start, uint32_t cin_state, uint32_t pw, unsigned lane) {
  if (pos == launch_start) return cin_state & 5u;
  const uint32_t b1 = pw >> 24;
  if (b1 != 0x5Cu && b1 != 0x22u) return byte_is_scalar(b1) ? 4u : 0u;
  const uint32_t b2 = (pw >> 16) & 0xFFu, b3 = (pw >> 8) & 0xFFu, b4 = pw & 0xFFu;
  const bool isq = (b1 == 0x22u);
  uint32_t run = 0xFFFFFFFFu;
  if (pos - launch_start >= 4) {
    if (isq) {
      if (b2 != 0x5Cu) run = 0;
      else if (b3 != 0x5Cu) run = 1;
      else if (b4 != 0x5Cu) run = 2;
    } else {
      if (b2 != 0x5Cu) run = 1;
      else if (b3 != 0x5Cu) run = 2;
      else if (b4 != 0x5Cu) run = 3;
    }
  }
  uint32_t odd;
  if (run != 0xFFFFFFFFu) {
    odd = run & 1u;
  } else {
    const uint64_t end = isq ? pos - 1 : pos;
    bool hit = false;
    const uint64_t r = run_back(buf, end, launch_start, lane, &hit);
    odd = uint32_t(r + ((hit && (cin_state & 1u)) ? 1u : 0u)) & 1u;
  }
  if (isq) return odd << 2;
  return odd | 4u;
}

SJ_DEV uint32_t word_before(const uint8_t *buf, uint32_t prev_word, uint64_t pos) {
  if (pos == 0) return prev_word;
  if (pos >= 4 && ((reinterpret_cast<uintptr_t>(buf) + pos) & 3u) == 0) return sj_ldg_u32(buf + pos - 4);
  uint32_t w = 0;
  for (int d = 1; d <= 4; d++) {
    const uint32_t b = (pos >= uint64_t(d)) ? sj_ldg_u8(buf + pos - d) : ((prev_word >> (8 * (4 - d + int(pos)))) & 0xFFu);
    w |= b << (8 * (4 - d));
  }
  return w;
}

SJ_DEV void fill_block_guarded(uint8_t *T, const uint8_t *buf, uint64_t len, uint64_t bstart, unsigned lane) {
  const bool aligned = (reinterpret_cast<uintptr_t>(buf) & 15u) == 0;
  for (uint32_t c = lane; c < uint32_t(kBlockBytes / 16); c += 32) {
    const uint64_t g = bstart + uint64_t(c) * 16;
    sj_u4 v;
    if (aligned && g + 16 <= len) {
      v = sj_ldg_u4(buf + g);
    } else {
      uint32_t w[4];
      for (int k = 0; k < 4; k++) {
        uint32_t x = 0;
        for (int b = 0; b < 4; b++) {
          const uint64_t q = g + 4 * k + b;
          const uint32_t byte = (q < len) ? sj_ldg_u8(buf + q) : 0x20u;
          x |= byte << (8 * b);
        }
        w[k] = x;
      }
      v = sj_make_u4(w[0], w[1], w[2], w[3]);
    }
    *reinterpret_cast<sj_u4 *>(T + swz(c * 16)) = v;
  }
}

SJ_DEV void load_unit(const uint8_t *T, uint32_t off, uint32_t w[8]) {
  const sj_u4 a = *reinterpret_cast<const sj_u4 *>(T + swz(off));
  const sj_u4 b = *reinterpret_cast<const sj_u4 *>(T + swz(off + 16));
  w[0] = a.x; w[1] = a.y; w[2] = a.z; w[3] = a.w;
  w[4] = b.x; w[5] = b.y; w[6] = b.z; w[7] = b.w;
}

template <bool kMin>
SJ_DEV uint32_t scan_block(const uint8_t *T, uint32_t pw0, uint32_t e_in, uint32_t c_in, unsigned lane, uint32_t *flags, sj_u4 *park0,
                           sj_u4 *park1, uint32_t *parkpre, uint32_t valid_bytes) {
  const uint32_t lane_off = lane * 128u;
  uint32_t bs[4], qu[4], op[4], sc[4], cl[4];
  uint32_t uerr = 0;
  if (kMin) {
#pragma unroll
    for (int u = 0; u < 4; u++) {
      uint32_t w8[8], pl[8];
      load_unit(T, lane_off + 32u * u, w8);
      transpose32(w8, pl);
      const unit_classes c = classify(pl);
      bs[u] = c.bs; qu[u] = c.qu; op[u] = c.op; sc[u] = c.sc; cl[u] = 0;
    }
  } else {
    uint32_t hi = 0;
#pragma unroll
    for (int c = 0; c < 8; c++) {
      const sj_u4 v = *reinterpret_cast<const sj_u4 *>(T + swz(lane_off + 16u * c));
      hi |= v.x | v.y | v.z | v.w;
    }
    if (!sj_any((hi & 0x80808080u) != 0)) {
#pragma unroll
      for (int u = 0; u < 4; u++) {
        uint32_t w8[8], pl[8];
        load_unit(T, lane_off + 32u * u, w8);
        transpose32(w8, pl);
        const unit_classes c = classify(pl);
        bs[u] = c.bs; qu[u] = c.qu; op[u] = c.op; sc[u] = c.sc; cl[u] = c.ctl;
      }
      if (lane == 0 && utf8_carry_pending(utf8_carry_from_prev_word(pw0))) uerr = 1u;
    } else {
      const uint32_t pw = (lane == 0) ? pw0 : *reinterpret_cast<const uint32_t *>(T + swz(lane_off - 4));
      utf8_carry uc = utf8_carry_from_prev_word(pw);
#pragma unroll
      for (int u = 0; u < 4; u++) {
        uint32_t w8[8], pl[8];
        load_unit(T, lane_off + 32u * u, w8);
        transpose32(w8, pl);
        const unit_classes c = classify(pl);
        bs[u] = c.bs; qu[u] = c.qu; op[u] = c.op; sc[u] = c.sc; cl[u] = c.ctl;
        uerr |= utf8_check_unit(pl, uc);
      }
    }
  }
  if (!kMin && sj_any(uerr != 0) && lane == 0) sj_atomic_or(flags, kFlagUtf8);

  uint32_t qr[4];
  {
    const uint32_t bsany = bs[0] | bs[1] | bs[2] | bs[3];
    if (sj_any(bsany != 0)) {
      uint32_t escaped[4];
      const uint32_t esc_out0 = escape_scan<4>(bs, escaped);
#pragma unroll
      for (int u = 0; u < 4; u++) qr[u] = qu[u] & ~escaped[u];
      const bool allbs = (bs[0] & bs[1] & bs[2] & bs[3]) == 0xFFFFFFFFu;
      const uint32_t G = sj_ballot(esc_out0 != 0);
      const uint32_t P = sj_ballot(allbs);
      uint32_t cout_unused;
      const uint32_t carries = escape_carries(G, P, e_in & 1u, &cout_unused) & ~P;
      if (carries != 0) {
        const int nlead = leading_backslashes<4>(bs);
        const uint32_t bit = ((carries >> lane) & 1u) ? (1u << (nlead & 31)) : 0u;
#pragma unroll
        for (int u = 0; u < 4; u++) qr[u] ^= qu[u] & (((nlead >> 5) == u) ? bit : 0u);
      }
    } else {
#pragma unroll
      for (int u = 0; u < 4; u++) qr[u] = qu[u];
      if ((e_in & 1u) && lane == 0) qr[0] ^= qu[0] & 1u;
    }
  }

  const uint32_t lp = uint32_t(sj_popc(qr[0] ^ qr[1] ^ qr[2] ^ qr[3])) & 1u;
  const uint32_t pb = sj_ballot(lp != 0);
  uint32_t instr = uint32_t(sj_popc(pb & ((1u << lane) - 1u))) & 1u;
  const uint32_t par = uint32_t(sj_popc(pb)) & 1u;
  uint32_t scal_prev = sj_shfl_up((sc[3] & ~qr[3]) >> 31, 1);
  if (lane == 0) scal_prev = c_in & 1u;
  uint32_t prev_nq = scal_prev << 31;
  uint32_t e0[4], e1[4];
  uint32_t hit0 = 0, hit1 = 0, cnt = 0;
#pragma unroll
  for (int u = 0; u < 4; u++) {
    const uint32_t in_string = prefix_xor32(qr[u]) ^ (0u - instr);
    instr = in_string >> 31;
    if (kMin) {
      const uint32_t ws = ~(op[u] | sc[u]);
      const int nv = int(valid_bytes) - int(lane_off) - 32 * u;
      const uint32_t valid = nv >= 32 ? 0xFFFFFFFFu : (nv <= 0 ? 0u : ((1u << nv) - 1u));
      e0[u] = ~(ws & ~in_string) & valid;
      e1[u] = ~(ws & in_string) & valid;
      cnt += uint32_t(sj_popc(e0[u])) | (uint32_t(sj_popc(e1[u])) << 16);
      continue;
    }
    const uint32_t nq = sc[u] & ~qr[u];
    const uint32_t follows = shl_in(prev_nq, nq, 1);
    prev_nq = nq;
    const uint32_t pm = op[u] | (sc[u] & ~follows);
    const uint32_t tail0 = in_string ^ qr[u];
    e0[u] = pm & ~tail0;
    e1[u] = pm & tail0;
    hit0 |= cl[u] & in_string;
    hit1 |= cl[u] & ~in_string;
    cnt += uint32_t(sj_popc(e0[u])) | (uint32_t(sj_popc(e1[u])) << 16);
  }
  uint32_t incl = cnt;
#pragma unroll
  for (int d = 1; d < 32; d <<= 1) {
    const uint32_t t = sj_shfl_up(incl, d);
    if (int(lane) >= d) incl += t;
  }
  const uint32_t total = sj_shfl(incl, 31);
  const unsigned tid = sj_tid();
  park0[tid] = sj_make_u4(e0[0], e0[1], e0[2], e0[3]);
  park1[tid] = sj_make_u4(e1[0], e1[1], e1[2], e1[3]);
  parkpre[tid] = incl - cnt;
  const uint32_t h0 = sj_any(hit0 != 0) ? 1u : 0u, h1 = sj_any(hit1 != 0) ? 1u : 0u;
  return total | (par << 29) | (h0 << 30) | (h1 << 31);
}

#define SJ_EMIT_STEP(m, q, pb)                   \
  {                                              \
    const bool has = (m) != 0;                   \
    const uint32_t h = sj_bfind(m);              \
    (q)--;                                       \
    if (has) *(q) = (pb) + h;                    \
    (m) &= ~(1u << (h & 31u));                   \
  }
SJ_DEV void emit_columns(const sj_u4 ev, uint32_t off, uint32_t pos_lane, uint32_t *dst) {
  uint32_t m0 = ev.x, m1 = ev.y, m2 = ev.z, m3 = ev.w;
  const uint32_t c0 = uint32_t(sj_popc(m0)), c1 = uint32_t(sj_popc(m1)), c2 = uint32_t(sj_popc(m2)), c3 = uint32_t(sj_popc(m3));
  uint32_t *q0 = dst + (off + c0);
  uint32_t *q1 = q0 + c1, *q2 = q1 + c2, *q3 = q2 + c3;
  const uint32_t pb0 = pos_lane, pb1 = pos_lane + 32u, pb2 = pos_lane + 64u, pb3 = pos_lane + 96u;
  const uint32_t c01 = c0 > c1 ? c0 : c1, c23 = c2 > c3 ? c2 : c3;
  const uint32_t n = sj_reduce_max(c01 > c23 ? c01 : c23);
#pragma unroll 2
  for (uint32_t k = 0; k < n; k++) {
    SJ_EMIT_STEP(m0, q0, pb0)
    SJ_EMIT_STEP(m1, q1, pb1)
    SJ_EMIT_STEP(m2, q2, pb2)
    SJ_EMIT_STEP(m3, q3, pb3)
  }
}
#undef SJ_EMIT_STEP

SJ_DEV_NOINLINE void emit_columns_dense(const sj_u4 ev, uint32_t off, uint32_t pos_lane, uint32_t *dst) {
  const uint32_t m4[4] = {ev.x, ev.y, ev.z, ev.w};
// ... 17 lines not shown
  const uint32_t total = pol ? ((sum >> 16) & 0x1FFFu) : (sum & 0xFFFFu);
  if (total == 0) return;
  const uint32_t elem = S->ticket[ns];
  const DocEntry &D = S->doc[S->tdoc[ns]];
  const uint32_t off = (prew >> (16 * pol)) & 0xFFFFu;
  const uint32_t pos_lane = p.pos_base + p.tile_begin * uint32_t(kTileBytes) + (elem - D.first_elem) * uint32_t(kElemBytes) + warp * uint32_t(kBlockBytes) + lane * 128u;
  uint32_t *out = D.idx_out + (out_base + S->res_base[ns][warp]);
  if (total + 3 <= kStageWords) {
    const uint32_t a = uint32_t((reinterpret_cast<uintptr_t>(out) >> 2) & 3u);
    sj_syncwarp();
    emit_columns(ev, off, pos_lane, stg + a);
    sj_syncwarp();
    const uint32_t head = (total < ((4u - a) & 3u)) ? total : ((4u - a) & 3u);
    const uint32_t nvec = (total - head) >> 2;
    const uint32_t tail = total - head - (nvec << 2);
    if (lane < head) out[lane] = stg[a + lane];
    const sj_u4 *sv = reinterpret_cast<const sj_u4 *>(stg + a + head);
    sj_u4 *gv = reinterpret_cast<sj_u4 *>(out + head);
    for (uint32_t i = lane; i < nvec; i += 32) gv[i] = sv[i];
    if (lane < tail) out[head + (nvec << 2) + lane] = stg[a + head + (nvec << 2) + lane];
    sj_syncwarp();
  } else {
    emit_columns_dense(ev, off, pos_lane, out);
  }
  if (!SJB200_SCAN4_TRACE && p.debug != nullptr && warp == 0 && lane == 0) p.debug[uint64_t(elem) * 8 + 5] = sj_globaltimer();
}

SJ_DEV void emit_from_smem(Smem *S, const ScanParams &p, uint64_t out_base, uint32_t e, unsigned warp, unsigned lane, uint32_t *stg) {
  const uint32_t pol = S->res_pol[e % kNS][warp] & 1u;
  const unsigned tid = warp * 32 + lane;
  emit_block(S, p, out_base, e, warp, lane, S->park[kGPark > 0 ? 0 : e % kPark][pol][kGPark > 0 ? 0 : tid], S->parkpre[kGPark > 0 ? 0 : e % kPark][kGPark > 0 ? 0 : tid], stg);
}

SJ_DEV uint32_t *park_slot(const ScanParams &p, uint32_t e) { return p.park + (size_t(sj_cta()) * kParkRing + (e % uint32_t(kParkRing))) * size_t(kParkSlotWords); }

SJ_DEV uint32_t compact_entry(uint32_t nib) {
  uint32_t sel = 0, cnt = 0;
  for (uint32_t b = 0; b < 4; b++)
    if ((nib >> b) & 1u) { sel |= b << (4 * cnt); cnt++; }
  for (uint32_t i = cnt; i < 4; i++) sel |= 4u << (4 * i);
  return sel;
}

SJ_DEV bool minify_fetch_issue(Smem *S, const sj_tensor_map *tmap, const ScanParams &p, uint32_t e, unsigned warp, unsigned lane, uint8_t *slot, sj_mbar_t *bar,
                               uint64_t launch_start) {
  const uint64_t bstart = launch_start + uint64_t(S->ticket[e % kNS]) * kElemBytes + uint64_t(warp) * kBlockBytes;
  const uint64_t row = bstart / 128;
  const bool by_tma = p.use_tma && (row + kBlockRows <= p.len / 128);
  sj_syncwarp();
  if (by_tma && lane == 0) {
    sj_fence_proxy_async();
    sj_mbar_arrive_expect_tx(bar, kBlockBytes);
    sj_tma_load_rows(slot, tmap, bar, uint32_t(row));
  }
  return by_tma;
}

SJ_DEV bool emit_minify_block(Smem *S, const sj_tensor_map *tmap, const ScanParams &p, uint64_t out_base, uint32_t e, unsigned warp, unsigned lane,
                              const sj_u4 kv, uint32_t prew, uint8_t *slot, sj_mbar_t *bar, uint32_t parity, uint64_t launch_start, int fetched = -1) {
  const int ns = int(e % kNS);
  const uint32_t sum = S->summary[ns][warp];
  const uint32_t pol = S->res_pol[ns][warp] & 1u;
  const uint32_t total = pol ? ((sum >> 16) & 0x1FFFu) : (sum & 0xFFFFu);
  if (fetched < 0 && total == 0) return false;
  const uint32_t elem = S->ticket[ns];
  const uint64_t bstart = launch_start + uint64_t(elem) * kElemBytes + uint64_t(warp) * kBlockBytes;
  const bool by_tma = fetched < 0 ? minify_fetch_issue(S, tmap, p, e, warp, lane, slot, bar, launch_start) : fetched != 0;
  if (by_tma) {
    wait_bar(bar, parity, p, 32);
  } else {
    if (total == 0) return false;
    fill_block_guarded(slot, p.buf, p.len, bstart, lane);
    sj_syncwarp();
  }
  if (total == 0) return by_tma;
  uint32_t w[32];
#pragma unroll
  for (int c = 0; c < 8; c++) {
    const sj_u4 v = *reinterpret_cast<const sj_u4 *>(slot + swz(lane * 128u + 16u * c));
    w[4 * c] = v.x; w[4 * c + 1] = v.y; w[4 * c + 2] = v.z; w[4 * c + 3] = v.w;
  }
  const uint32_t off = (prew >> (16 * pol)) & 0xFFFFu;
  sj_syncwarp();
  if (off < uint32_t(kBlockBytes)) *reinterpret_cast<uint32_t *>(slot + swz(off & ~3u)) = 0u;
  if (lane == 31 && total < uint32_t(kBlockBytes)) *reinterpret_cast<uint32_t *>(slot + swz(total & ~3u)) = 0u;
  sj_syncwarp();
  const uint32_t keep[4] = {kv.x, kv.y, kv.z, kv.w};
  uint32_t cn[4];
#pragma unroll
  for (int q = 0; q < 4; q++) cn[q] = keep[q] - ((keep[q] >> 1) & 0x77777777u) - ((keep[q] >> 2) & 0x33333333u) - ((keep[q] >> 3) & 0x11111111u);
#pragma unroll
  for (int i = 0; i < 32; i++) w[i] = byte_perm(w[i], 0u, S->compact_lut[(keep[i >> 3] >> (4 * (i & 7))) & 15u]);
  const uint32_t wa0 = off & ~3u;
  uint32_t carry = 0, sh = 8u * (off & 3u), wa = wa0, first = 0;
#pragma unroll
  for (int i = 0; i < 32; i++) {
    const uint32_t c8 = (i & 7) == 0 ? (cn[i >> 3] << 3) & 0x38u : (cn[i >> 3] >> (4 * (i & 7) - 3)) & 0x38u;
    const uint32_t merged = carry | (w[i] << sh);
    const uint32_t tot = sh + c8;
    const bool done = tot >= 32u;
    const bool is_first = wa == wa0;
    if (done && !is_first) *reinterpret_cast<uint32_t *>(slot + swz(wa)) = merged;
    first = (done && is_first) ? merged : first;
    carry = done ? sj_funnel_l(w[i], 0u, int(sh)) : merged;
    wa += done ? 4u : 0u;
    sh = tot & 31u;
  }
  if (wa != wa0) sj_atomic_or(reinterpret_cast<uint32_t *>(slot + swz(wa0)), first);
  if (sh) sj_atomic_or(reinterpret_cast<uint32_t *>(slot + swz(wa)), carry);
  sj_syncwarp();
  uint8_t *dst = p.dst + (out_base + S->res_base[ns][warp]);
  const uint32_t a = uint32_t(reinterpret_cast<uintptr_t>(dst) & 15u);
  const uint32_t head = (total < ((16u - a) & 15u)) ? total : ((16u - a) & 15u);
  const uint32_t nvec = (total - head) >> 4;
  const uint32_t tail = total - head - (nvec << 4);
  if (lane < head) dst[lane] = slot[swz(lane)];
  const uint32_t hw = head >> 2;
  const int hs = int(8u * (head & 3u));
  for (uint32_t i = lane; i < nvec; i += 32) {
    const sj_u4 A = *reinterpret_cast<const sj_u4 *>(slot + swz(16u * i));
    sj_u4 B = A;
    if (head) B = *reinterpret_cast<const sj_u4 *>(slot + swz(16u * i + 16u));
    uint32_t x0, x1, x2, x3, x4;
    if (hw == 0) { x0 = A.x; x1 = A.y; x2 = A.z; x3 = A.w; x4 = B.x; }
    else if (hw == 1) { x0 = A.y; x1 = A.z; x2 = A.w; x3 = B.x; x4 = B.y; }
    else if (hw == 2) { x0 = A.z; x1 = A.w; x2 = B.x; x3 = B.y; x4 = B.z; }
    else { x0 = A.w; x1 = B.x; x2 = B.y; x3 = B.z; x4 = B.w; }
    *reinterpret_cast<sj_u4 *>(dst + head + 16u * i) = sj_make_u4(sj_funnel_r(x0, x1, hs), sj_funnel_r(x1, x2, hs), sj_funnel_r(x2, x3, hs), sj_funnel_r(x3, x4, hs));
  }
  if (lane < tail) dst[head + (nvec << 4) + lane] = slot[swz(head + (nvec << 4) + lane)];
  sj_syncwarp();
  if (p.debug != nullptr && warp == 0 && lane == 0) p.debug[uint64_t(elem) * 8 + 5] = sj_globaltimer();
  return by_tma;
}

SJ_DEV void compose_element(Smem *S, const ScanParams &p, int ns, uint32_t t, uint32_t doc_first, unsigned lane) {
  const uint32_t r = (lane < uint32_t(kScanWarps)) ? S->summary[ns][lane] : 0u;
  const uint32_t c0 = r & 0xFFFFu, c1 = (r >> 16) & 0x1FFFu, h0 = (r >> 30) & 1u, h1 = r >> 31;
  const uint32_t P = sj_ballot(((r >> 29) & 1u) != 0);
  const uint32_t s = uint32_t(sj_popc(P & ((1u << lane) - 1u))) & 1u;
  const uint32_t a = s ? c1 : c0, b = s ? c0 : c1;
  const uint32_t A = sj_reduce_add(a), B = sj_reduce_add(b);
  const uint32_t HA = sj_any((s ? h1 : h0) != 0) ? 1u : 0u, HB = sj_any((s ? h0 : h1) != 0) ? 1u : 0u;
  const uint32_t par = uint32_t(sj_popc(P)) & 1u;
  if (lane == 0) {
    if (t > doc_first) sj_st_relaxed_u64(p.count_desc + t, pack_agg(p.epoch, par, A, B));
    S->elem[ns][0] = par;
    S->elem[ns][1] = A;
    S->elem[ns][2] = B;
    S->elem[ns][3] = HA | (HB << 1);
  }
  uint32_t ia = a, ib = b;
#pragma unroll
  for (int d = 1; d < kScanWarps; d <<= 1) {
    const uint32_t xa = sj_shfl_up(ia, d), xb = sj_shfl_up(ib, d);
    if (int(lane) >= d) { ia += xa; ib += xb; }
  }
  if (lane < uint32_t(kScanWarps)) {
    S->pre[ns][0][lane] = (s << 31) | (ia - a);
    S->pre[ns][1][lane] = ((s ^ 1u) << 31) | (ib - b);
  }
  sj_syncwarp();
}

SJ_DEV void publish_ticket(Smem *S, uint32_t j, uint32_t value, uint32_t hint, unsigned lane) {
  if (lane == 0) {
    uint32_t d = hint;
    while (d + 1 < S->ndocs && S->doc[d + 1].first_elem <= value) d++;
    S->ticket[j % kNS] = value;
    S->tdoc[j % kNS] = d;
    sj_mbar_arrive(&S->ticket_ready[j % kNS]);
  }
  sj_syncwarp();
}

SJ_DEV uint32_t wait_ticket(Smem *S, uint32_t j, const ScanParams &p) {
  if (!wait_bar(&S->ticket_ready[j % kNS], (j / kNS) & 1u, p, 100)) return 0xFFFFFFFFu;
  return S->ticket[j % kNS];
}

SJ_DEV uint32_t launch_elements(const Smem *S) { return S->doc[S->ndocs - 1].first_elem + S->doc[S->ndocs - 1].nelem; }

SJ_DEV bool issue_load(Smem *S, uint32_t d, const ScanParams &p, uint32_t le, unsigned warp, unsigned lane, int r, uint32_t *pw_out, uint32_t *fenced) {
  const DocEntry &D = S->doc[d];
  const uint64_t bstart = uint64_t(p.tile_begin) * kTileBytes + uint64_t(le) * kElemBytes + uint64_t(warp) * kBlockBytes;
  const uint64_t row = bstart / 128;
  const bool full = D.tmap != nullptr && bstart < D.scan_end && (row + kBlockRows <= D.len / 128);
  sj_syncwarp();
  if (lane == 0) {
    if (full) {
      if (p.ndocs > 0 && d != *fenced) {
        sj_fence_tensormap_acquire(D.tmap);
        *fenced = d;
      }
      sj_fence_proxy_async();
      sj_mbar_arrive_expect_tx(&S->full[warp][r], kBlockBytes);
      sj_tma_load_rows(S->ring[warp][r], static_cast<const sj_tensor_map *>(D.tmap), &S->full[warp][r], uint32_t(row));
    }
    *pw_out = (bstart < D.len) ? word_before(D.buf, p.prev_word, bstart) : 0x20202020u;
  }
  return full;
}

template <int kMode>
SJ_DEV void emit_role(Smem *S, const sj_tensor_map *tmap, const ScanParams &p, const Carry &cin, unsigned lane, uint8_t *stage, sj_mbar_t *fetch_bar,
                      uint32_t fetch_phase);

template <int kMode>
SJ_DEV void scan_role(Smem *S, const sj_tensor_map *tmap, const ScanParams &p, const Carry &cin, unsigned warp, unsigned lane, uint32_t first_ticket) {
  const uint32_t nelem = launch_elements(S);
  const uint64_t launch_start = uint64_t(p.tile_begin) * kTileBytes;
  constexpr bool kMin = (kMode == 2);
  const uint64_t out_base = cin.count;
  uint32_t full_phase = 0;
  uint32_t pw_cur = 0x20202020u, pw_next = 0x20202020u;
  bool tma_cur = false, tma_next = false;
  if (warp == 0) publish_ticket(S, 0, first_ticket, 0, lane);
  uint32_t t = wait_ticket(S, 0, p);
  uint32_t fenced = 0xFFFFFFFFu;
  if (t < nelem) tma_cur = issue_load(S, S->tdoc[0], p, t - S->doc[S->tdoc[0]].first_elem, warp, lane, 0, &pw_cur, &fenced);
  if (warp == 0) {
    if (tma_cur) wait_bar(&S->full[0][0], 0u, p, 32);
    uint32_t a1 = 0;
    if (lane == 0) a1 = sj_atomic_add(p.ticket, 1u);
    publish_ticket(S, 1, a1, S->tdoc[0], lane);
  }
  uint32_t ne = 0;
  uint32_t j = 0;
  constexpr bool kEmitW = (kEmitWarps > 0);
  for (;; j++) {
    if (t >= nelem) break;
    const int r = int(j & 1u);
    SJ_TRACE4(0);
    const uint32_t tn = wait_ticket(S, j + 1, p);
    if (warp == (j % uint32_t(kScanWarps))) {
      uint32_t a = 0;
      if (lane == 0) a = sj_atomic_add(p.ticket, 1u);
      publish_ticket(S, j + 2, a, S->tdoc[(j + 1) % kNS], lane);
    }
    SJ_TRACE4(1);
    if (tn < nelem) {
      const uint32_t dn = S->tdoc[(j + 1) % kNS];
      tma_next = issue_load(S, dn, p, tn - S->doc[dn].first_elem, warp, lane, r ^ 1, &pw_next, &fenced);
    }
    SJ_TRACE4(2);
    uint8_t *T = S->ring[warp][r];
    const DocEntry &D = S->doc[S->tdoc[j % kNS]];
    const uint64_t bstart = launch_start + uint64_t(t - D.first_elem) * kElemBytes + uint64_t(warp) * kBlockBytes;
    if (!SJB200_SCAN4_TRACE && p.debug != nullptr && warp == 0 && lane == 0) {
      p.debug[uint64_t(t) * 8 + 0] = sj_globaltimer();
      p.debug[uint64_t(t) * 8 + 7] = ((unsigned long long)sj_smid() << 48) | ((unsigned long long)sj_cta() << 32) | j;
    }
    uint32_t summary = 0;
    if (bstart < D.scan_end) {
      if (tma_cur) {
        wait_bar(&S->full[warp][r], (full_phase >> r) & 1u, p, 32);
        full_phase ^= 1u << r;
      } else {
        fill_block_guarded(T, D.buf, D.len, bstart, lane);
        sj_syncwarp();
      }
      SJ_TRACE4(3);
      const uint32_t pw0 = sj_shfl(pw_cur, 0);
      const uint32_t st = boundary_state(D.buf, bstart, launch_start, cin.state, pw0, lane);
      SJ_TRACE4(4);
      {
        if (kEmitW && j >= uint32_t(kParkFree)) wait_bar(&S->park_free[j % kParkFree], ((j / kParkFree) - 1u) & 1u, p, 64);
        const uint64_t left = D.len - bstart;
        const uint32_t valid = left < uint64_t(kBlockBytes) ? uint32_t(left) : uint32_t(kBlockBytes);
        if (kEmitW && kGPark > 0) {
          uint32_t *slot = park_slot(p, j);
          summary = scan_block<kMin>(T, pw0, st & 1u, (st >> 2) & 1u, lane, D.flags, reinterpret_cast<sj_u4 *>(slot), reinterpret_cast<sj_u4 *>(slot) + kScanWarps * 32,
                                     slot + 2 * kScanWarps * 32 * 4, valid);
        } else {
          summary = scan_block<kMin>(T, pw0, st & 1u, (st >> 2) & 1u, lane, D.flags, S->park[j % kPark][0], S->park[j % kPark][1], S->parkpre[j % kPark], valid);
        }
      }
    }
    if (!SJB200_SCAN4_TRACE && p.debug != nullptr && warp == 0 && lane == 0) p.debug[uint64_t(t) * 8 + 1] = sj_globaltimer();
    int fetched = -1;
    if (kMin && !kEmitW && j >= uint32_t(kLag)) fetched = minify_fetch_issue(S, tmap, p, ne, warp, lane, T, &S->full[warp][r], launch_start) ? 1 : 0;
    SJ_TRACE4(5);
    {
      const int ns = int(j % kNS);
      uint32_t last = 0;
      if (lane == 0) {
        S->summary[ns][warp] = summary;
        sj_fence_block();
        last = (sj_atomic_add(&S->arrived[ns], 1u) == uint32_t(kScanWarps - 1)) ? 1u : 0u;
      }
      if (sj_shfl(last, 0)) {
        sj_fence_block();
        if (!SJB200_SCAN4_TRACE && p.debug != nullptr && lane == 0) p.debug[uint64_t(t) * 8 + 3] = sj_globaltimer();
        compose_element(S, p, ns, t, D.first_elem, lane);
        if (lane == 0) {
          S->arrived[ns] = 0;
          sj_mbar_arrive(&S->scanned[ns]);
        }
      }
    }
    SJ_TRACE4(6);
    SJ_TRACE4(7);
    if (!kEmitW && j >= uint32_t(kLag)) {
      wait_bar(&S->resolved[ne % kNS], (ne / kNS) & 1u, p, 64);
      SJ_TRACE4(8);
      if (!SJB200_SCAN4_TRACE && p.debug != nullptr && warp == 0 && lane == 0) p.debug[uint64_t(S->ticket[ne % kNS]) * 8 + 2] = sj_globaltimer();
      if (kMin) {
        const uint32_t pol = S->res_pol[ne % kNS][warp] & 1u;
        if (emit_minify_block(S, tmap, p, out_base, ne, warp, lane, S->park[kGPark > 0 ? 0 : ne % kPark][pol][kGPark > 0 ? 0 : warp * 32 + lane], S->parkpre[kGPark > 0 ? 0 : ne % kPark][kGPark > 0 ? 0 : warp * 32 + lane], T,
                              &S->full[warp][r], (full_phase >> r) & 1u, launch_start, fetched))
          full_phase ^= 1u << r;
      } else {
        emit_from_smem(S, p, out_base, ne, warp, lane, reinterpret_cast<uint32_t *>(T));
      }
      ne++;
      SJ_TRACE4(9);
    }
    t = tn;
    tma_cur = tma_next;
    pw_cur = pw_next;
  }
  if (kEmitW) {
    if (warp == 0 && lane == 0) sj_st_release_u32(&S->scan_done, j);
    sj_syncwarp();
    emit_role<kMode>(S, tmap, p, cin, lane, S->ring[warp][0], &S->full[warp][0], full_phase & 1u);
  } else {
    while (ne < j) {
      wait_bar(&S->resolved[ne % kNS], (ne / kNS) & 1u, p, 64);
      if (kMin) {
        const uint32_t pol = S->res_pol[ne % kNS][warp] & 1u;
        if (emit_minify_block(S, tmap, p, out_base, ne, warp, lane, S->park[kGPark > 0 ? 0 : ne % kPark][pol][kGPark > 0 ? 0 : warp * 32 + lane], S->parkpre[kGPark > 0 ? 0 : ne % kPark][kGPark > 0 ? 0 : warp * 32 + lane],
                              S->ring[warp][0], &S->full[warp][0], full_phase & 1u, launch_start))
          full_phase ^= 1u;
      } else {
        emit_from_smem(S, p, out_base, ne, warp, lane, reinterpret_cast<uint32_t *>(S->ring[warp][0]));
      }
      ne++;
    }
  }
}

template <int kMode>
SJ_DEV void emit_role(Smem *S, const sj_tensor_map *tmap, const ScanParams &p, const Carry &cin, unsigned lane, uint8_t *stage, sj_mbar_t *fetch_bar,
                      uint32_t fetch_phase) {
  const uint64_t out_base = cin.count;
  const uint64_t launch_start = uint64_t(p.tile_begin) * kTileBytes;
  uint32_t *stg = reinterpret_cast<uint32_t *>(stage);
  for (;;) {
    uint32_t q = 0;
    if (lane == 0) q = sj_atomic_add(&S->emit_next, 1u);
    q = sj_shfl(q, 0);
    const uint32_t e = q / uint32_t(kScanWarps), b = q % uint32_t(kScanWarps);
    uint32_t spins = 0;
    for (;;) {
      if (sj_mbar_try_wait(&S->resolved[e % kNS], (e / kNS) & 1u)) break;
      const uint32_t done = sj_ld_acquire_u32(&S->scan_done);
      if (done != 0xFFFFFFFFu && e >= done) return;
      if (++spins > kSpinLimit4) {
        sj_atomic_or(p.flags, kFlagInternal);
        return;
      }
      sj_nanosleep(32);
    }
    const uint32_t pol = S->res_pol[e % kNS][b] & 1u;
    const unsigned tid = b * 32u + lane;
    sj_u4 ev;
    uint32_t prew;
    if (kGPark > 0) {
      const uint32_t *slot = park_slot(p, e);
      ev = sj_ld_u4(slot + (pol * kScanWarps * 32 + tid) * 4);
      prew = sj_ld_u32(slot + 2 * kScanWarps * 32 * 4 + tid);
    } else {
      ev = S->park[kGPark > 0 ? 0 : e % kPark][pol][kGPark > 0 ? 0 : tid];
      prew = S->parkpre[kGPark > 0 ? 0 : e % kPark][kGPark > 0 ? 0 : tid];
    }
    if (kMode == 2) {
      if (emit_minify_block(S, tmap, p, out_base, e, b, lane, ev, prew, stage, fetch_bar, fetch_phase, launch_start)) fetch_phase ^= 1u;
    } else {
      emit_block(S, p, out_base, e, b, lane, ev, prew, stg);
    }
    sj_syncwarp();
    if (lane == 0) {
      sj_fence_block();
      if (sj_atomic_add(&S->emitted_cnt[e % kNS], 1u) == uint32_t(kScanWarps - 1)) {
        S->emitted_cnt[e % kNS] = 0;
        sj_mbar_arrive(&S->park_free[e % kParkFree]);
      }
    }
  }
}


SJ_DEV void look_back(const ScanParams &p, uint32_t t, unsigned lane, uint32_t *s_in, uint32_t *base, uint32_t doc_first = 0) {
  Eff acc;
  acc.p = 0; acc.a = 0; acc.b = 0;
  int64_t newest = int64_t(t) - 1;
  const uint32_t key_agg = (p.epoch << 2) | kDescAgg;
  for (;;) {
    const int64_t first = newest - int64_t(lane);
    unsigned long long d[kLookK];
    uint32_t pend = 0;
#pragma unroll
    for (int k = 0; k < kLookK; k++) {
      d[k] = 0;
      if (first - 32 * k >= int64_t(doc_first)) pend |= 1u << k;
    }
    const uint32_t want = pend;
    uint32_t inc_dist = 0xFFFFFFFFu, needed = (1u << kLookK) - 1u;
    uint32_t spins = 0;
    for (;;) {
      const uint32_t todo = pend;
#pragma unroll
      for (int k = 0; k < kLookK; k++)
        if (todo & (1u << k)) d[k] = sj_ld_relaxed_u64(p.count_desc + (first - 32 * k));
      uint32_t okm = 0, incm = 0;
#pragma unroll
      for (int k = 0; k < kLookK; k++) {
        const uint32_t rel = uint32_t(d[k] >> 44) - key_agg;
        if (rel <= 1u) okm |= 1u << k;
        if (rel == 1u) incm |= 1u << k;
      }
      pend &= ~okm;
      incm &= want;
      const uint32_t my_dist = incm ? uint32_t(sj_ffs(incm) - 1) * 32u + lane : 0xFFFFFFFFu;
      inc_dist = sj_reduce_min(my_dist);
      if (inc_dist != 0xFFFFFFFFu) {
        const uint32_t nk = (inc_dist > lane) ? (inc_dist - lane + 31u) / 32u : 0u;
        needed = (1u << nk) - 1u;
      }
      if (!sj_any((pend & needed) != 0)) break;
      if (++spins > kSpinLimit4) {
        sj_atomic_or(p.flags, kFlagInternal);
        break;
      }
    }
    const uint32_t use = want & ~pend & needed;
    uint32_t bal[kLookK];
#pragma unroll
    for (int k = 0; k < kLookK; k++) bal[k] = sj_ballot(((use >> k) & 1u) && ((uint32_t(d[k] >> 38) & 1u) != 0));
    uint32_t older = 0;
    uint32_t sa = 0, sb = 0;
#pragma unroll
    for (int k = kLookK - 1; k >= 0; k--) {
      const uint32_t rel = (uint32_t(sj_popc((bal[k] >> lane) >> 1)) ^ older) & 1u;
      if ((use >> k) & 1u) {
        const uint32_t a = uint32_t(d[k]) & 0x7FFFFu, b = uint32_t(d[k] >> 19) & 0x7FFFFu;
        sa += rel ? b : a;
        sb += rel ? a : b;
      }
      older ^= uint32_t(sj_popc(bal[k])) & 1u;
    }
    Eff win;
    win.p = older;
    win.a = sj_reduce_add(sa);
    win.b = sj_reduce_add(sb);
    acc = compose(win, acc);
    if (inc_dist != 0xFFFFFFFFu) {
      const uint32_t ik = inc_dist >> 5, il = inc_dist & 31u;
      uint32_t sk = 0, ck = 0;
#pragma unroll
      for (int k = 0; k < kLookK; k++)
        if (uint32_t(k) == ik) { sk = uint32_t(d[k] >> 32) & 1u; ck = uint32_t(d[k]); }
      sk = sj_shfl(sk, int(il));
      ck = sj_shfl(ck, int(il));
      *s_in = sk ^ acc.p;
      *base = ck + (sk ? acc.b : acc.a);
      return;
    }
    newest -= 32 * kLookK;
    if (newest < int64_t(doc_first)) {
      sj_atomic_or(p.flags, kFlagInternal);
      *s_in = acc.p;
      *base = acc.a;
      return;
    }
  }
}

SJ_DEV void finalize_launch(const ScanParams &p, const DocEntry &D, const Carry &cin, uint32_t s_out, uint64_t count_total, unsigned lane) {
  const uint64_t launch_start = uint64_t(p.tile_begin) * kTileBytes;
  const uint64_t end_real = D.scan_end;
  const uint32_t st = boundary_state(D.buf, end_real, launch_start, cin.state, word_before(D.buf, p.prev_word, end_real), lane);
  const uint32_t e_a = st & 1u, c_a = (st >> 2) & 1u, par_a = (s_out ^ (cin.state >> 1)) & 1u;
  const uint64_t nlead = run_forward(D.buf, launch_start, end_real, lane);
  uint32_t e_o = e_a, c_o = c_a, par_o = par_a;
  if (launch_start + nlead >= end_real) {
    e_o ^= 1u;
  } else if (sj_ldg_u8(D.buf + launch_start + nlead) == 0x22u) {
    par_o ^= 1u;
    if (launch_start + nlead == end_real - 1) c_o ^= 1u;
  }
  const uint32_t ein = cin.state & 1u;
  const uint32_t T0 = ein ? (e_o | (par_o << 1) | (c_o << 2)) : (e_a | (par_a << 1) | (c_a << 2));
  const uint32_t T1 = ein ? (e_a | (par_a << 1) | (c_a << 2)) : (e_o | (par_o << 1) | (c_o << 2));
  if (lane == 0) {
    D.carry_out->count = count_total;
    D.carry_out->state = e_a | (s_out << 1) | (c_a << 2);
    D.carry_out->ttable = T0 | (T1 << 3);
    if (D.carry_out_host != nullptr) {
      D.carry_out_host->count = count_total;
      D.carry_out_host->state = e_a | (s_out << 1) | (c_a << 2);
      D.carry_out_host->ttable = T0 | (T1 << 3);
    }
    if (p.write_sentinels) {
      uint32_t *tail = D.idx_out + count_total;
      tail[0] = D.len;
      tail[1] = D.len;
      tail[2] = 0;
    }
    if (p.check_eof) {
      const uint32_t tw = word_before(D.buf, p.prev_word, D.len);
      if (utf8_carry_pending(utf8_carry_from_prev_word(tw))) sj_atomic_or(D.flags, kFlagUtf8);
    }
  }
}

SJ_DEV void chain_role(Smem *S, const ScanParams &p, const Carry &cin, unsigned lane, unsigned c) {
  const uint32_t nelem = launch_elements(S);
  for (uint32_t j = c;; j += uint32_t(kChainWarps)) {
    const int ns = int(j % kNS);
    const uint32_t t = wait_ticket(S, j, p);
    if (t >= nelem) break;
    const DocEntry &D = S->doc[S->tdoc[ns]];
    uint32_t s_in = (cin.state >> 1) & 1u, base = 0;
    if (t > D.first_elem) look_back(p, t, lane, &s_in, &base, D.first_elem);
    wait_bar(&S->scanned[ns], (j / kNS) & 1u, p, 64);
    if (!SJB200_SCAN4_TRACE && p.debug != nullptr && lane == 0) p.debug[uint64_t(t) * 8 + 6] = sj_globaltimer();
    const uint32_t par = S->elem[ns][0], b0 = S->elem[ns][1], b1 = S->elem[ns][2], hits = S->elem[ns][3];
    const uint32_t mine_total = s_in ? b1 : b0;
    const uint32_t s_out = s_in ^ par;
    if (lane == 0) sj_st_relaxed_u64(p.count_desc + t, pack_inc(p.epoch, s_out, base + mine_total));
    if (lane < uint32_t(kScanWarps)) {
      const uint32_t pk = S->pre[ns][s_in][lane];
      S->res_pol[ns][lane] = pk >> 31;
      S->res_base[ns][lane] = base + (pk & 0x7FFFFFFFu);
    }
    const uint32_t hit0 = hits & 1u, hit1 = (hits >> 1) & 1u;
    if (lane == 0 && (s_in ? hit1 : hit0)) sj_atomic_or(D.flags, kFlagCtl);
    sj_syncwarp();
    if (lane == 0) sj_mbar_arrive(&S->resolved[ns]);
    if (!SJB200_SCAN4_TRACE && p.debug != nullptr && lane == 0) p.debug[uint64_t(t) * 8 + 4] = sj_globaltimer();
    if (t == D.first_elem + D.nelem - 1) finalize_launch(p, D, cin, s_out, cin.count + base + mine_total, lane);
  }
}

template <int kMode>
SJ_DEV void scan4_body(const sj_tensor_map *tmap, const ScanParams &p, uint8_t *smem_raw, uint32_t smem_raw_addr) {
  Smem *S = reinterpret_cast<Smem *>(smem_raw + ((1024u - (smem_raw_addr & 1023u)) & 1023u));
  const unsigned tid = sj_tid(), lane = tid & 31u, warp = tid >> 5;
#if SJB200_SCAN4_TRACE
  if (tid == 0) {
    S->trace_cta[0] = sj_globaltimer();
    for (int a = 0; a < 2; a++)
      for (int b = 0; b < kTraceIters; b++)
        for (int cc = 0; cc < kTracePoints; cc++) S->trace[a][b][cc] = 0;
  }
#endif
  uint32_t first_ticket = 0;
  if (tid == 0) first_ticket = sj_atomic_add(p.ticket, 1u);
  Carry cin;
  cin.count = 0; cin.state = 0; cin.ttable = 0; cin.flags = 0; cin.reserved = 0;
  if (p.carry_in != nullptr) cin = *p.carry_in;
  if (tid < unsigned(kNS)) {
    sj_mbar_init(&S->ticket_ready[tid], 1);
    sj_mbar_init(&S->scanned[tid], 1);
    sj_mbar_init(&S->resolved[tid], 1);
    S->arrived[tid] = 0;
    S->emitted_cnt[tid] = 0;
  } else if (tid < unsigned(kNS + 2 * kScanWarps)) {
    const unsigned k = tid - unsigned(kNS);
    sj_mbar_init(&S->full[k >> 1][k & 1u], 1);
  } else if (tid < unsigned(kNS + 2 * kScanWarps + kParkFree)) {
    sj_mbar_init(&S->park_free[tid - unsigned(kNS + 2 * kScanWarps)], 1);
  } else if (tid < unsigned(kNS + 2 * kScanWarps + kParkFree + (kEmitWarps > 0 ? kEmitWarps : 1))) {
    sj_mbar_init(&S->efull[tid - unsigned(kNS + 2 * kScanWarps + kParkFree)], 1);
  }
  if (tid == 0) {
    S->emit_next = 0;
    S->scan_done = 0xFFFFFFFFu;
  }
  if (tid < unsigned(kNS + 2 * kScanWarps + kParkFree + (kEmitWarps > 0 ? kEmitWarps : 1))) sj_fence_mbar_init();
  if (kMode == 2 && tid < 16) S->compact_lut[tid] = compact_entry(tid);
  if (p.ndocs > 0) {
    const uint32_t nw = p.ndocs * uint32_t(sizeof(DocEntry) / 16);
    for (uint32_t i = tid; i < nw; i += unsigned(kThreads4))
      reinterpret_cast<sj_u4 *>(S->doc)[i] = sj_ldg_u4(reinterpret_cast<const uint8_t *>(p.docs) + 16 * size_t(i));
    if (tid == 0) S->ndocs = p.ndocs;
  } else if (tid == 0) {
    DocEntry &D = S->doc[0];
    const uint64_t launch_end = (uint64_t(p.tile_begin) + p.ntiles) * kTileBytes;
    D.buf = p.buf;
    D.idx_out = p.idx_out;
    D.carry_out = p.carry_out;
    D.carry_out_host = p.carry_out_host;
    D.flags = p.flags;
    D.tmap = p.use_tma ? static_cast<const void *>(tmap) : nullptr;
    D.len = uint32_t(p.len);
    D.scan_end = uint32_t(p.len < launch_end ? p.len : launch_end);
    D.first_elem = 0;
    D.nelem = elements_of(p);
    S->ndocs = 1;
  }
  sj_syncthreads();
#if SJB200_SCAN4_TRACE
  if (tid == 0) S->trace_cta[1] = sj_globaltimer();
#endif
  if (warp < unsigned(kScanWarps)) scan_role<kMode>(S, tmap, p, cin, warp, lane, first_ticket);
  else if (warp < unsigned(kScanWarps + kChainWarps)) chain_role(S, p, cin, lane, warp - unsigned(kScanWarps));
  else emit_role<kMode>(S, tmap, p, cin, lane, S->estage[warp - unsigned(kScanWarps + kChainWarps)], &S->efull[warp - unsigned(kScanWarps + kChainWarps)], 0u);
#if SJB200_SCAN4_TRACE
  if (tid == 0) S->trace_cta[2] = sj_globaltimer();
#endif
  sj_syncthreads();
#if SJB200_SCAN4_TRACE
  if (tid == 0 && p.debug != nullptr) {
    unsigned long long *row = p.debug + size_t(sj_cta()) * (1 + 2 * kTraceIters) * 8;
    row[0] = S->trace_cta[0]; row[1] = S->trace_cta[1]; row[2] = S->trace_cta[2]; row[3] = sj_globaltimer(); row[4] = sj_smid();
    for (int a = 0; a < 2; a++)
      for (int b = 0; b < kTraceIters; b++) {
        unsigned long long *q = row + size_t(1 + a * kTraceIters + b) * 8;
        for (int cc = 0; cc < 6; cc++) q[cc] = (unsigned long long)S->trace[a][b][2 * cc] | ((unsigned long long)S->trace[a][b][2 * cc + 1] << 32);
      }
  }
#endif
  if (tid == 0) {
    sj_threadfence();
    const uint32_t done = sj_atomic_add(p.ticket + 1, 1u);
    if (done == sj_nctas() - 1) {
      p.ticket[0] = 0;
      p.ticket[1] = 0;
      p.ticket[2] = 0;
      const uint32_t fl_launch = sj_atomic_exch(p.flags, 0u);
      uint32_t fl = fl_launch;
      for (uint32_t d = 0; d < S->ndocs; d++) {
        const DocEntry &D = S->doc[d];
        fl = fl_launch | (D.flags != p.flags ? sj_atomic_exch(D.flags, 0u) : 0u);
        D.carry_out->flags = fl;
        if (D.carry_out_host != nullptr) D.carry_out_host->flags = fl;
      }
      if (p.xchg_nranks != 0) {
        const volatile Carry *co = p.carry_out;
        const unsigned long long w0 = xchg_word0(p.xchg_seq, co->count),
                                 w1 = xchg_word1(p.xchg_seq, co->state, co->ttable, kMode == 2 ? (fl & uint32_t(kFlagInternal)) : fl, kMode == 2 ? kMinify : int(p.xchg_kind));
        for (uint32_t r = 0; r < p.xchg_nranks; r++) {
          unsigned long long *rec = p.xchg_peer[r] + (size_t(p.xchg_slot) * kMaxRanks + p.xchg_rank) * 2;
          sj_st_sys_u64(rec, w0);
          sj_st_sys_u64(rec + 1, w1);
        }
      }
      sj_threadfence();
    }
  }
}

}
}
```

simdjson_b200/csrc/sjb200_simt.cuh:

```cuda
#pragma once
#include <stdint.h>

#if defined(SJB200_HOST_EMU)
#include <pthread.h>
#include <sched.h>
#include <string.h>
#include <time.h>

#include <atomic>
#include <mutex>
#include <new>

#define SJ_DEV inline
#define SJ_DEV_NOINLINE

namespace sjb200 {
namespace simt {

struct WarpShared {
  pthread_barrier_t bar;
  uint32_t vals[2][32];
};
struct CtaShared {
  pthread_barrier_t bar;
  uint8_t *smem;
};
struct ThreadCtx {
  unsigned tid = 0, cta = 0, nctas = 0;
  unsigned phase = 0;
  WarpShared *warp = nullptr;
  CtaShared *ctas = nullptr;
};
extern thread_local ThreadCtx tctx;

inline uint32_t exchange(uint32_t v, unsigned &ph) {
  ThreadCtx &t = tctx;
  ph = t.phase;
  t.warp->vals[ph][t.tid & 31u] = v;
  pthread_barrier_wait(&t.warp->bar);
  t.phase ^= 1u;
  return 0;
}

}

struct alignas(16) sj_u4 { uint32_t x, y, z, w; };
SJ_DEV sj_u4 sj_make_u4(uint32_t x, uint32_t y, uint32_t z, uint32_t w) { sj_u4 v; v.x = x; v.y = y; v.z = z; v.w = w; return v; }
SJ_DEV sj_u4 sj_ldg_u4(const void *p) { sj_u4 v; memcpy(&v, p, 16); return v; }
SJ_DEV uint32_t sj_ldg_u32(const void *p) { uint32_t v; memcpy(&v, p, 4); return v; }
SJ_DEV uint32_t sj_ldg_u8(const uint8_t *p) { return *p; }
SJ_DEV sj_u4 sj_ld_u4(const void *p) { sj_u4 v; memcpy(&v, p, 16); return v; }
SJ_DEV uint32_t sj_ld_u32(const void *p) { uint32_t v; memcpy(&v, p, 4); return v; }

SJ_DEV unsigned sj_tid() { return simt::tctx.tid; }
SJ_DEV unsigned sj_cta() { return simt::tctx.cta; }
SJ_DEV unsigned sj_nctas() { return simt::tctx.nctas; }
SJ_DEV uint8_t *sj_smem_base() { return simt::tctx.ctas->smem; }

SJ_DEV uint32_t sj_shfl(uint32_t v, int src) {
  unsigned ph;
  simt::exchange(v, ph);
  return simt::tctx.warp->vals[ph][src & 31];
}
SJ_DEV uint32_t sj_shfl_up(uint32_t v, int d) {
  unsigned ph;
  simt::exchange(v, ph);
  const int lane = int(simt::tctx.tid & 31u);
  return lane >= d ? simt::tctx.warp->vals[ph][lane - d] : v;
}
SJ_DEV uint32_t sj_shfl_down(uint32_t v, int d) {
  unsigned ph;
  simt::exchange(v, ph);
  const int lane = int(simt::tctx.tid & 31u);
  return lane + d < 32 ? simt::tctx.warp->vals[ph][lane + d] : v;
}
SJ_DEV uint32_t sj_ballot(bool pred) {
  unsigned ph;
  simt::exchange(pred ? 1u : 0u, ph);
  uint32_t m = 0;
  for (int i = 0; i < 32; i++) m |= (simt::tctx.warp->vals[ph][i] & 1u) << i;
  return m;
}
SJ_DEV bool sj_any(bool pred) { return sj_ballot(pred) != 0; }
SJ_DEV uint32_t sj_reduce_max(uint32_t v) {
  unsigned ph;
  simt::exchange(v, ph);
  uint32_t m = 0;
  for (int i = 0; i < 32; i++) m = simt::tctx.warp->vals[ph][i] > m ? simt::tctx.warp->vals[ph][i] : m;
  return m;
}
SJ_DEV uint32_t sj_reduce_min(uint32_t v) {
  unsigned ph;
  simt::exchange(v, ph);
  uint32_t m = 0xFFFFFFFFu;
  for (int i = 0; i < 32; i++) m = simt::tctx.warp->vals[ph][i] < m ? simt::tctx.warp->vals[ph][i] : m;
  return m;
}
SJ_DEV uint32_t sj_reduce_add(uint32_t v) {
  unsigned ph;
  simt::exchange(v, ph);
  uint32_t m = 0;
  for (int i = 0; i < 32; i++) m += simt::tctx.warp->vals[ph][i];
  return m;
}
SJ_DEV void sj_syncwarp() {
  unsigned ph;
  simt::exchange(0, ph);
}
SJ_DEV void sj_syncthreads() { pthread_barrier_wait(&simt::tctx.ctas->bar); }

SJ_DEV int sj_popc(uint32_t x) { return __builtin_popcount(x); }
SJ_DEV int sj_ffs(uint32_t x) { return __builtin_ffs(int(x)); }
SJ_DEV uint32_t sj_bfind(uint32_t x) { return x ? uint32_t(31 - __builtin_clz(x)) : 0xFFFFFFFFu; }
SJ_DEV uint32_t sj_funnel_l(uint32_t lo, uint32_t hi, int n) { return n ? ((hi << n) | (lo >> (32 - n))) : hi; }
SJ_DEV uint32_t sj_funnel_r(uint32_t lo, uint32_t hi, int n) { return n ? ((lo >> n) | (hi << (32 - n))) : lo; }

SJ_DEV uint32_t sj_atomic_add(uint32_t *p, uint32_t v) { return __atomic_fetch_add(p, v, __ATOMIC_SEQ_CST); }
SJ_DEV uint32_t sj_atomic_or(uint32_t *p, uint32_t v) { return __atomic_fetch_or(p, v, __ATOMIC_SEQ_CST); }
SJ_DEV uint32_t sj_atomic_exch(uint32_t *p, uint32_t v) { return __atomic_exchange_n(p, v, __ATOMIC_SEQ_CST); }
SJ_DEV unsigned long long sj_ld_relaxed_u64(const unsigned long long *p) { return __atomic_load_n(p, __ATOMIC_ACQUIRE); }
SJ_DEV void sj_st_relaxed_u64(unsigned long long *p, unsigned long long v) { __atomic_store_n(p, v, __ATOMIC_RELEASE); }
SJ_DEV void sj_threadfence() { __atomic_thread_fence(__ATOMIC_SEQ_CST); }
SJ_DEV void sj_st_sys_u64(unsigned long long *p, unsigned long long v) { __atomic_store_n(p, v, __ATOMIC_RELEASE); }
SJ_DEV void sj_fence_gpu_release() { __atomic_thread_fence(__ATOMIC_SEQ_CST); }
SJ_DEV uint32_t sj_ld_relaxed_u32(const uint32_t *p) { return __atomic_load_n(p, __ATOMIC_ACQUIRE); }
SJ_DEV void sj_fence_block() { __atomic_thread_fence(__ATOMIC_SEQ_CST); }
SJ_DEV void sj_st_release_u32(uint32_t *p, uint32_t v) { __atomic_store_n(p, v, __ATOMIC_RELEASE); }
SJ_DEV uint32_t sj_ld_acquire_u32(const uint32_t *p) { return __atomic_load_n(p, __ATOMIC_ACQUIRE); }
SJ_DEV void sj_nanosleep(unsigned) {
  struct timespec ts = {0, 20000};
  nanosleep(&ts, nullptr);
}
SJ_DEV unsigned sj_smid() { return simt::tctx.cta; }
SJ_DEV unsigned long long sj_globaltimer() {
  struct timespec ts;
  clock_gettime(CLOCK_MONOTONIC, &ts);
  return (unsigned long long)ts.tv_sec * 1000000000ull + (unsigned long long)ts.tv_nsec;
}
SJ_DEV uint32_t sj_clock32() { return uint32_t(sj_globaltimer()); }

struct sj_tensor_map {
  const uint8_t *base;
  uint64_t rows;
  uint32_t box_rows;
};
struct sj_mbar_t {
  std::mutex mu;
  uint32_t count = 0, pending = 0, phase = 0;
  int64_t tx = 0;
  struct Copy { uint8_t *dst; const uint8_t *src; uint32_t rows; uint32_t bytes; } q[4];
  int nq = 0;
};
namespace simt {
inline void mbar_check_complete(sj_mbar_t *b) {
  if (b->pending == 0 && b->tx == 0) {
    b->phase ^= 1u;
    b->pending = b->count;
  }
}
inline void mbar_run_copies(sj_mbar_t *b) {
  for (int i = 0; i < b->nq; i++) {
    const sj_mbar_t::Copy &c = b->q[i];
    for (uint32_t r = 0; r < c.rows; r++)
      for (uint32_t col = 0; col < 128; col++) {
        const uint32_t off = r * 128 + col;
        c.dst[off ^ ((off >> 3) & 0x70u)] = c.src[size_t(r) * 128 + col];
      }
    b->tx -= int64_t(c.bytes);
  }
  b->nq = 0;
  mbar_check_complete(b);
}
}
SJ_DEV void sj_mbar_init(sj_mbar_t *b, uint32_t count) {
  new (b) sj_mbar_t();
  b->count = b->pending = count;
}
SJ_DEV void sj_fence_mbar_init() {}
SJ_DEV void sj_fence_proxy_async() {}
SJ_DEV void sj_fence_tensormap_acquire(const void *) {}
SJ_DEV void sj_mbar_arrive(sj_mbar_t *b) {
  std::lock_guard<std::mutex> g(b->mu);
  b->pending--;
  simt::mbar_check_complete(b);
}
SJ_DEV void sj_mbar_arrive_expect_tx(sj_mbar_t *b, uint32_t bytes) {
  std::lock_guard<std::mutex> g(b->mu);
  b->tx += int64_t(bytes);
  b->pending--;
  simt::mbar_check_complete(b);
}
SJ_DEV bool sj_mbar_try_wait(sj_mbar_t *b, uint32_t parity) {
  {
    std::lock_guard<std::mutex> g(b->mu);
    if (b->nq) simt::mbar_run_copies(b);
    if (b->phase != parity) return true;
  }
  struct timespec ts = {0, 20000};
  nanosleep(&ts, nullptr);
  return false;
}
SJ_DEV void sj_tma_load_rows(uint8_t *dst, const sj_tensor_map *map, sj_mbar_t *bar, uint32_t row) {
  std::lock_guard<std::mutex> g(bar->mu);
  sj_mbar_t::Copy &c = bar->q[bar->nq++];
  c.dst = dst;
  c.src = map->base + size_t(row) * 128;
  c.rows = map->box_rows;
  c.bytes = map->box_rows * 128;
}

}

#else
#include <cuda.h>
#include <cuda_runtime.h>

#define SJ_DEV __device__ __forceinline__
#define SJ_DEV_NOINLINE static __device__ __noinline__

namespace sjb200 {

constexpr uint32_t kFullMask = 0xFFFFFFFFu;

typedef uint4 sj_u4;
SJ_DEV sj_u4 sj_make_u4(uint32_t x, uint32_t y, uint32_t z, uint32_t w) { return make_uint4(x, y, z, w); }
SJ_DEV sj_u4 sj_ldg_u4(const void *p) { return __ldg(reinterpret_cast<const uint4 *>(p)); }
SJ_DEV uint32_t sj_ldg_u32(const void *p) { return __ldg(reinterpret_cast<const uint32_t *>(p)); }
SJ_DEV uint32_t sj_ldg_u8(const uint8_t *p) { return __ldg(p); }
SJ_DEV sj_u4 sj_ld_u4(const void *p) { return *reinterpret_cast<const uint4 *>(p); }
SJ_DEV uint32_t sj_ld_u32(const void *p) { return *reinterpret_cast<const uint32_t *>(p); }

SJ_DEV unsigned sj_tid() { return threadIdx.x; }
SJ_DEV unsigned sj_cta() { return blockIdx.x; }
SJ_DEV unsigned sj_nctas() { return gridDim.x; }

SJ_DEV uint32_t sj_shfl(uint32_t v, int src) { return __shfl_sync(kFullMask, v, src); }
SJ_DEV uint32_t sj_shfl_up(uint32_t v, int d) { return __shfl_up_sync(kFullMask, v, d); }
SJ_DEV uint32_t sj_shfl_down(uint32_t v, int d) { return __shfl_down_sync(kFullMask, v, d); }
SJ_DEV uint32_t sj_ballot(bool pred) { return __ballot_sync(kFullMask, pred); }
SJ_DEV bool sj_any(bool pred) { return __any_sync(kFullMask, pred); }
SJ_DEV uint32_t sj_reduce_max(uint32_t v) { return __reduce_max_sync(kFullMask, v); }
SJ_DEV uint32_t sj_reduce_min(uint32_t v) { return __reduce_min_sync(kFullMask, v); }
SJ_DEV uint32_t sj_reduce_add(uint32_t v) { return __reduce_add_sync(kFullMask, v); }
SJ_DEV void sj_syncwarp() { __syncwarp(); }
SJ_DEV void sj_syncthreads() { __syncthreads(); }
SJ_DEV int sj_popc(uint32_t x) { return __popc(x); }
SJ_DEV int sj_ffs(uint32_t x) { return __ffs(int(x)); }
SJ_DEV uint32_t sj_bfind(uint32_t x) {
  uint32_t r;
  asm("bfind.u32 %0, %1;" : "=r"(r) : "r"(x));
  return r;
}
SJ_DEV uint32_t sj_funnel_l(uint32_t lo, uint32_t hi, int n) { return __funnelshift_l(lo, hi, n); }
SJ_DEV uint32_t sj_funnel_r(uint32_t lo, uint32_t hi, int n) { return __funnelshift_r(lo, hi, n); }

SJ_DEV uint32_t sj_atomic_add(uint32_t *p, uint32_t v) { return atomicAdd(p, v); }
SJ_DEV uint32_t sj_atomic_or(uint32_t *p, uint32_t v) { return atomicOr(p, v); }
SJ_DEV uint32_t sj_atomic_exch(uint32_t *p, uint32_t v) { return atomicExch(p, v); }
SJ_DEV unsigned long long sj_ld_relaxed_u64(const unsigned long long *p) {
  unsigned long long v;
  asm volatile("ld.relaxed.gpu.global.u64 %0, [%1];" : "=l"(v) : "l"(p) : "memory");
  return v;
}
SJ_DEV void sj_st_relaxed_u64(unsigned long long *p, unsigned long long v) {
  asm volatile("st.relaxed.gpu.global.u64 [%0], %1;" ::"l"(p), "l"(v) : "memory");
}
SJ_DEV void sj_threadfence() { __threadfence(); }
SJ_DEV void sj_st_sys_u64(unsigned long long *p, unsigned long long v) {
  asm volatile("st.relaxed.sys.global.u64 [%0], %1;" ::"l"(p), "l"(v) : "memory");
}
SJ_DEV void sj_fence_gpu_release() { asm volatile("fence.acq_rel.gpu;" ::: "memory"); }
SJ_DEV uint32_t sj_ld_relaxed_u32(const uint32_t *p) {
  uint32_t v;
  asm volatile("ld.relaxed.gpu.global.u32 %0, [%1];" : "=r"(v) : "l"(p) : "memory");
  return v;
}
SJ_DEV void sj_fence_block() { __threadfence_block(); }
SJ_DEV void sj_st_release_u32(uint32_t *p, uint32_t v) {
  __threadfence_block();
  *reinterpret_cast<volatile uint32_t *>(p) = v;
}
SJ_DEV uint32_t sj_ld_acquire_u32(const uint32_t *p) {
  const uint32_t v = *reinterpret_cast<const volatile uint32_t *>(p);
  __threadfence_block();
  return v;
}
SJ_DEV void sj_nanosleep(unsigned ns) { __nanosleep(ns); }
SJ_DEV unsigned sj_smid() {
  unsigned r;
  asm volatile("mov.u32 %0, %%smid;" : "=r"(r));
  return r;
}
SJ_DEV unsigned long long sj_globaltimer() {
  unsigned long long t;
  asm volatile("mov.u64 %0, %globaltimer;" : "=l"(t));
  return t;
}
SJ_DEV uint32_t sj_clock32() { return uint32_t(clock64()); }

typedef CUtensorMap sj_tensor_map;
typedef unsigned long long sj_mbar_t;

SJ_DEV uint32_t sj_smem_u32(const void *p) { return (uint32_t)__cvta_generic_to_shared(p); }
SJ_DEV void sj_mbar_init(sj_mbar_t *bar, uint32_t count) {
  asm volatile("mbarrier.init.shared::cta.b64 [%0], %1;" ::"r"(sj_smem_u32(bar)), "r"(count) : "memory");
}
SJ_DEV void sj_fence_mbar_init() { asm volatile("fence.mbarrier_init.release.cluster;" ::: "memory"); }
SJ_DEV void sj_fence_proxy_async() { asm volatile("fence.proxy.async.shared::cta;" ::: "memory"); }
SJ_DEV void sj_fence_tensormap_acquire(const void *map) {
  asm volatile("fence.proxy.tensormap::generic.acquire.sys [%0], 128;" ::"l"(map) : "memory");
}
SJ_DEV void sj_mbar_arrive(sj_mbar_t *bar) {
  asm volatile("mbarrier.arrive.release.cta.shared::cta.b64 _, [%0];" ::"r"(sj_smem_u32(bar)) : "memory");
}
SJ_DEV void sj_mbar_arrive_expect_tx(sj_mbar_t *bar, uint32_t bytes) {
  asm volatile("mbarrier.arrive.expect_tx.shared::cta.b64 _, [%0], %1;" ::"r"(sj_smem_u32(bar)), "r"(bytes) : "memory");
}
SJ_DEV bool sj_mbar_try_wait(sj_mbar_t *bar, uint32_t parity) {
  uint32_t ok;
  asm volatile(
      "{\n"
      ".reg .pred p;\n"
      "mbarrier.try_wait.parity.acquire.cta.shared::cta.b64 p, [%1], %2, 0x1000;\n"
      "selp.u32 %0, 1, 0, p;\n"
      "}\n"
      : "=r"(ok)
      : "r"(sj_smem_u32(bar)), "r"(parity)
      : "memory");
  return ok != 0;
}
SJ_DEV void sj_tma_load_rows(uint8_t *dst, const sj_tensor_map *map, sj_mbar_t *bar, uint32_t row) {
  asm volatile(
      "cp.async.bulk.tensor.2d.shared::cluster.global.mbarrier::complete_tx::bytes [%0], [%1, {%3, %4}], [%2];" ::"r"(sj_smem_u32(dst)),
      "l"(map), "r"(sj_smem_u32(bar)), "r"(0), "r"(int(row))
      : "memory");
}

}
#endif
```

simdjson_b200/implementation.py:

```python
import ctypes as C

import numpy as np

from . import capi
from .capi import (CAPACITY, EMPTY, MEMALLOC, REGULAR, SUCCESS, UNEXPECTED_ERROR, UNSUPPORTED_ARCHITECTURE, UTF8_ERROR)

_LIB = None


def lib():
    global _LIB
    if _LIB is None:
        _LIB = capi.load()
    return _LIB


def _host_u8(buf):
    if isinstance(buf, np.ndarray):
        return np.ascontiguousarray(buf, dtype=np.uint8)
    return np.frombuffer(bytes(buf), dtype=np.uint8)


def _is_torch(x):
    return type(x).__module__.startswith("torch")


def _stream_ptr(stream):
    if stream is None:
        import torch
        return C.c_void_p(torch.cuda.current_stream().cuda_stream)
    if hasattr(stream, "cuda_stream"):
        return C.c_void_p(stream.cuda_stream)
    return C.c_void_p(int(stream))


class dom_parser_implementation:

    def __init__(self, device=0):
        self._ctx = C.c_void_p()
        self._device = device
        self._capacity = 0
        self.n_structural_indexes = 0
        self.structural_indexes = None
        self.next_structural_index = 0
        self._d_idx = None

    def _create(self, capacity):
        rc = lib().sjb200_create(self._device, capacity, C.byref(self._ctx))
        if rc == SUCCESS:
            self._after_capacity(capacity)
        return rc

    def close(self):
        if self._ctx:
            self._unpin()
            lib().sjb200_destroy(self._ctx)
            self._ctx = C.c_void_p()

    def _unpin(self):
        if getattr(self, "_pinned", False) and self.structural_indexes is not None:
            lib().sjb200_unpin_host_memory(self._ctx, self.structural_indexes.ctypes.data)
        self._pinned = False

    def __del__(self):
        try:
            self.close()
        except Exception:
            pass

    def _after_capacity(self, capacity):
        self._capacity = capacity
        self._unpin()
        words = lib().sjb200_index_words(capacity)
        self.structural_indexes = np.zeros(words, dtype=np.uint32)
        self.structural_indexes[0] = 0
        self._pinned = lib().sjb200_pin_host_memory(self._ctx, self.structural_indexes.ctypes.data, words * 4) == SUCCESS
        self.n_structural_indexes = 0
        self._d_idx = None

    def capacity(self):
        return self._capacity

    def set_capacity(self, capacity):
        rc = lib().sjb200_set_capacity(self._ctx, capacity)
        if rc == SUCCESS:
            self._after_capacity(capacity)
        return rc

    def set_option(self, key, value):
        return lib().sjb200_set_option(self._ctx, key.encode(), int(value))

    def get_stat(self, key):
        return lib().sjb200_get_stat(self._ctx, key.encode())

    def last_cuda_error(self):
        return lib().sjb200_last_cuda_error(self._ctx).decode()

    def stage1(self, buf, mode=REGULAR):
        a = _host_u8(buf)
        n = C.c_uint32(self.n_structural_indexes)
        ptr = a.ctypes.data if len(a) else None
        rc = lib().sjb200_stage1(self._ctx, ptr, len(a), mode, self.structural_indexes.ctypes.data, C.byref(n))
        self.n_structural_indexes = n.value
        if rc in (SUCCESS, UTF8_ERROR) or (rc == EMPTY and len(a) > 0):
            self.next_structural_index = 0
        return rc

    def device_index_buffer(self, nbytes=None):
        import torch
        if nbytes is None and self._d_idx is not None:
            return self._d_idx
        words = lib().sjb200_index_words(self._capacity if nbytes is None else nbytes)
        if self._d_idx is None or self._d_idx.numel() < words:
            self._d_idx = torch.empty(words, dtype=torch.int32, device=f"cuda:{self._device}")
        return self._d_idx

    def stage1_device(self, d_buf, mode=REGULAR, d_idx=None, stream=None):
        if d_idx is None:
            d_idx = self.device_index_buffer(d_buf.numel())
        n = C.c_uint32(self.n_structural_indexes)
        rc = lib().sjb200_stage1_dev(self._ctx, d_buf.data_ptr(), d_buf.numel(), mode, d_idx.data_ptr(), C.byref(n), _stream_ptr(stream))
        self.n_structural_indexes = n.value
        return rc

    def stage1_device_batch(self, d_bufs, d_idxs, mode=REGULAR, stream=None):
        n = len(d_bufs)
        docs = (capi.Doc * n)()
        for i in range(n):
            docs[i].d_buf = d_bufs[i].data_ptr()
            docs[i].len = d_bufs[i].numel()
            docs[i].d_idx = d_idxs[i].data_ptr()
            docs[i].n_structural_indexes = 0
        rc = lib().sjb200_stage1_dev_batch(self._ctx, docs, n, mode, _stream_ptr(stream))
        if rc != SUCCESS:
            raise RuntimeError("sjb200_stage1_dev_batch failed: " + self.last_cuda_error())
        return [(docs[i].error, docs[i].n_structural_indexes) for i in range(n)]

    def stage1_device_enqueue(self, d_buf, mode=REGULAR, d_idx=None, stream=None):
        if d_idx is None:
            d_idx = self.device_index_buffer(d_buf.numel())
        return lib().sjb200_stage1_dev_enqueue(self._ctx, d_buf.data_ptr(), d_buf.numel(), mode, d_idx.data_ptr(), _stream_ptr(stream))

    def stage1_device_finish(self):
        n = C.c_uint32(self.n_structural_indexes)
        rc = lib().sjb200_stage1_dev_finish(self._ctx, C.byref(n))
        self.n_structural_indexes = n.value
        return rc

    def tokens_device(self, d_buf, d_idx=None, n=None, strbuf_capacity=None, stream=None):
        import torch
        if d_idx is None:
            d_idx = self.device_index_buffer()
        if n is None:
            n = self.n_structural_indexes
        cap = lib().sjb200_string_buf_capacity(d_buf.numel()) if strbuf_capacity is None else strbuf_capacity
        dev = d_buf.device
        d_type = torch.empty(max(n, 1), dtype=torch.uint8, device=dev)
        d_payload = torch.empty(max(n, 1), dtype=torch.int64, device=dev)
        d_strbuf = torch.empty(max(cap, 1), dtype=torch.uint8, device=dev)
        res = capi.TokensResult()
        lib().sjb200_tokens_dev(self._ctx, d_buf.data_ptr(), d_buf.numel(), d_idx.data_ptr(), n, d_type.data_ptr(), d_payload.data_ptr(),
                                d_strbuf.data_ptr() if cap else None, cap, C.byref(res), _stream_ptr(stream))
        return res, d_type[:n], d_payload[:n], d_strbuf

    def stage1_shard_device(self, d_buf, state_in=0, last_shard=True, d_idx=None, stream=None):
        if d_idx is None:
            d_idx = self.device_index_buffer(d_buf.numel())
        res = capi.ShardResult()
        rc = lib().sjb200_stage1_shard_dev(self._ctx, d_buf.data_ptr(), d_buf.numel(), state_in, int(last_shard), d_idx.data_ptr(),
                                           C.byref(res), _stream_ptr(stream))
        return rc, res

    def stage1_shard_device_enqueue(self, d_buf, d_result, d_idx=None, stream=None):
        if d_idx is None:
            d_idx = self.device_index_buffer(d_buf.numel())
        return lib().sjb200_stage1_shard_dev_enqueue(self._ctx, d_buf.data_ptr(), d_buf.numel(), d_idx.data_ptr(), d_result.data_ptr(),
                                                     _stream_ptr(stream))

    def _minify_host(self, buf):
        a = _host_u8(buf)
        dst = np.empty(max(len(a), 1), dtype=np.uint8)
        dl = C.c_size_t(0)
        rc = lib().sjb200_minify(self._ctx, a.ctypes.data if len(a) else None, len(a), dst.ctypes.data, C.byref(dl))
        return rc, dst[: dl.value]

    def _validate_utf8_host(self, buf):
        a = _host_u8(buf)
        return bool(lib().sjb200_validate_utf8(self._ctx, a.ctypes.data if len(a) else None, len(a)))

    def minify_device(self, d_buf, d_dst, stream=None):
        dl = C.c_size_t(0)
        rc = lib().sjb200_minify_dev(self._ctx, d_buf.data_ptr(), d_buf.numel(), d_dst.data_ptr(), C.byref(dl), _stream_ptr(stream))
        return rc, dl.value

    def minify_device_enqueue(self, d_buf, d_dst, stream=None):
        return lib().sjb200_minify_dev_enqueue(self._ctx, d_buf.data_ptr(), d_buf.numel(), d_dst.data_ptr(), _stream_ptr(stream))

    def minify_device_finish(self):
        dl = C.c_size_t(0)
        rc = lib().sjb200_minify_dev_finish(self._ctx, C.byref(dl))
        return rc, dl.value

    def validate_utf8_device(self, d_buf, stream=None):
        return lib().sjb200_validate_utf8_dev(self._ctx, d_buf.data_ptr(), d_buf.numel(), _stream_ptr(stream))

    def validate_utf8_device_enqueue(self, d_buf, stream=None):
        return lib().sjb200_validate_utf8_dev_enqueue(self._ctx, d_buf.data_ptr(), d_buf.numel(), _stream_ptr(stream))

    def validate_utf8_device_finish(self):
        return lib().sjb200_validate_utf8_dev_finish(self._ctx)


class implementation:

    def __init__(self, device=0):
        self._device = device
        self._util = None

    def name(self):
        return "b200"

    def description(self):
        return "NVIDIA H100 (sm_90a) stage 1"

    def required_instruction_sets(self):
        return 0

    def supported_by_runtime_system(self):
        p = dom_parser_implementation(self._device)
        rc = p._create(0)
        p.close()
        return rc == SUCCESS

    def create_dom_parser_implementation(self, capacity, max_depth=1024):
        _ = max_depth
        p = dom_parser_implementation(self._device)
        rc = p._create(capacity)
        return (rc, p) if rc == SUCCESS else (rc, None)

    def _utility(self):
        if self._util is None:
            rc, p = self.create_dom_parser_implementation(0)
            if rc != SUCCESS:
                raise RuntimeError(f"sjb200_create failed: {capi.ERROR_NAMES.get(rc, rc)}")
            self._util = p
        return self._util

    def minify(self, buf):
        return self._utility()._minify_host(buf)

    def validate_utf8(self, buf):
        return self._utility()._validate_utf8_host(buf)


_ACTIVE = {}


def get_active_implementation(device=0):
    if device not in _ACTIVE:
        _ACTIVE[device] = implementation(device)
    return _ACTIVE[device]


def minify(buf, device=0):
    return get_active_implementation(device).minify(buf)


def validate_utf8(buf, device=0):
    return get_active_implementation(device).validate_utf8(buf)
```

Before: 963.4.

## Chain batched scan launches with PDL, cache tensor maps, and batch doc-table uploads

```diff
diff --git a/include/sjb200.h b/include/sjb200.h
--- a/include/sjb200.h
+++ b/include/sjb200.h
@@ -49,6 +49,7 @@
 SJB200_API double sjb200_get_stat(sjb200_ctx *ctx, const char *key);
 
 SJB200_API long sjb200_get_debug_timeline(sjb200_ctx *ctx, unsigned long long *out, size_t max_tiles);
+SJB200_API long sjb200_get_launch_stamps(sjb200_ctx *ctx, unsigned long long *out, size_t max_launches);
 
 SJB200_API int sjb200_pin_host_memory(sjb200_ctx *ctx, void *ptr, size_t bytes);
 SJB200_API int sjb200_unpin_host_memory(sjb200_ctx *ctx, void *ptr);
diff --git a/simdjson_b200/capi.py b/simdjson_b200/capi.py
--- a/simdjson_b200/capi.py
+++ b/simdjson_b200/capi.py
@@ -7,6 +7,7 @@
 EXPORTS = [
     "sjb200_create", "sjb200_destroy", "sjb200_set_capacity", "sjb200_capacity", "sjb200_index_words", "sjb200_device",
     "sjb200_last_cuda_error", "sjb200_set_option", "sjb200_get_stat", "sjb200_pin_host_memory", "sjb200_unpin_host_memory", "sjb200_get_debug_timeline",
+    "sjb200_get_launch_stamps",
     "sjb200_stage1", "sjb200_minify", "sjb200_validate_utf8",
     "sjb200_stage1_dev", "sjb200_minify_dev", "sjb200_validate_utf8_dev", "sjb200_stage1_dev_batch",
     "sjb200_document_table_dev", "sjb200_stage1_dev_enqueue", "sjb200_stage1_dev_finish", "sjb200_minify_dev_enqueue", "sjb200_minify_dev_finish",
@@ -85,6 +86,7 @@
         "sjb200_set_option": (C.c_int, [vp, C.c_char_p, C.c_long]),
         "sjb200_get_stat": (C.c_double, [vp, C.c_char_p]),
         "sjb200_get_debug_timeline": (C.c_long, [vp, vp, sz]),
+        "sjb200_get_launch_stamps": (C.c_long, [vp, vp, sz]),
         "sjb200_pin_host_memory": (C.c_int, [vp, vp, sz]),
         "sjb200_unpin_host_memory": (C.c_int, [vp, vp]),
         "sjb200_stage1": (C.c_int, [vp, vp, sz, C.c_int, vp, u32p]),
diff --git a/simdjson_b200/csrc/sjb200_capi.cu b/simdjson_b200/csrc/sjb200_capi.cu
--- a/simdjson_b200/csrc/sjb200_capi.cu
+++ b/simdjson_b200/csrc/sjb200_capi.cu
@@ -28,6 +28,14 @@
                                     CUtensorMapL2promotion, CUtensorMapFloatOOBfill);
 
 constexpr int kCarrySlots = 1024;
+constexpr int kTmapCacheEntries = 64;
+
+struct TmapCacheEntry {
+  const uint8_t *base = nullptr;
+  uint64_t rows = 0;
+  int box_rows = 0;
+  CUtensorMap map;
+};
 constexpr size_t kMaxBytes = 0xFFFFFFFFull;
 
 struct PendingCall {
@@ -60,6 +68,7 @@
   uint32_t *d_ticket = nullptr;
   unsigned long long *d_count_desc = nullptr;
   size_t desc_tiles = 0;
+  unsigned long long *d_stamps = nullptr; size_t stamps_cap = 0; size_t stamps_used = 0;
   StreamFinish *d_sfin = nullptr;
   uint32_t *d_doc_scratch = nullptr; size_t doc_scratch_words = 0; uint32_t *d_ndocs = nullptr;
   void *d_tok_scratch = nullptr; size_t tok_scratch_bytes = 0; TokenTotals *d_tok_tot = nullptr;
@@ -82,10 +91,12 @@
   uint32_t ev_last_docs = 1;
   uint8_t *h_doctab = nullptr; uint8_t *d_doctab = nullptr; size_t doctab_bytes = 0;
   long opt_debug_timeline = 0;
+  long opt_pdl = 1, opt_launch_stamps = 0;
   unsigned long long *d_debug = nullptr; size_t debug_tiles = 0; uint32_t debug_last_tiles = 0;
   unsigned long long launches = 0;
   unsigned long long ew_launches = 0;
   PFN_encodeTiled encode = nullptr;
+  TmapCacheEntry tmap_cache[kTmapCacheEntries];
   uint8_t *h_ring = nullptr; size_t ring_slot_bytes = 0; int ring_slots = 0;
   std::vector<cudaEvent_t> ring_events;
   CopyPool *pool = nullptr;
@@ -152,8 +163,8 @@
   cudaFree(c->d_count_desc); c->d_count_desc = nullptr;
   c->desc_tiles = 0;
   const size_t n = std::max(need, size_t(tiles_of(c->capacity)) + 1);
-  if (!dev_alloc(c, &c->d_count_desc, n, "cudaMalloc(count_desc)")) return false;
-  if (!ok(c, cudaMemsetAsync(c->d_count_desc, 0, n * sizeof(unsigned long long), c->stream), "memset desc")) return false;
+  if (!dev_alloc(c, &c->d_count_desc, 2 * n, "cudaMalloc(count_desc)")) return false;
+  if (!ok(c, cudaMemsetAsync(c->d_count_desc, 0, 2 * n * sizeof(unsigned long long), c->stream), "memset desc")) return false;
   if (!ok(c, cudaStreamSynchronize(c->stream), "sync")) return false;
   c->desc_tiles = n;
   c->epoch = 0;
@@ -161,15 +172,21 @@
 }
 bool ensure_desc(sjb200_ctx *c, size_t len) { return ensure_desc_n(c, tiles_of(len)); }
 
-bool next_epoch(sjb200_ctx *c, cudaStream_t launch_stream, uint32_t *epoch) {
+bool next_epoch(sjb200_ctx *c, cudaStream_t launch_stream, uint32_t *epoch, bool *wiped = nullptr) {
   c->epoch++;
+  if (wiped) *wiped = false;
   if (c->epoch >= (1u << 18)) {
-    if (!ok(c, cudaMemsetAsync(c->d_count_desc, 0, c->desc_tiles * sizeof(unsigned long long), launch_stream), "memset desc")) return false;
+    if (!ok(c, cudaMemsetAsync(c->d_count_desc, 0, 2 * c->desc_tiles * sizeof(unsigned long long), launch_stream), "memset desc")) return false;
     c->epoch = 1;
+    if (wiped) *wiped = true;
   }
   *epoch = c->epoch;
   return true;
 }
+
+uint32_t *launch_ticket(sjb200_ctx *c, int parity) { return c->d_ticket + 4 * parity; }
+uint32_t *launch_flags(sjb200_ctx *c, int parity) { return parity ? c->d_flags + 1 + kCarrySlots : c->d_flags; }
+unsigned long long *launch_desc(sjb200_ctx *c, int parity) { return c->d_count_desc + size_t(parity) * c->desc_tiles; }
 
 bool make_tensor_map(sjb200_ctx *c, CUtensorMap *map, const uint8_t *d_buf, size_t len, bool *usable, int box_rows = kScan4BoxRows) {
   memset(map, 0, sizeof(*map));
@@ -177,6 +194,13 @@
   const uint64_t rows = len / 128;
   if (!c->opt_use_tma || c->encode == nullptr || rows == 0) return true;
   if ((reinterpret_cast<uintptr_t>(d_buf) & 15u) != 0) return true;
+  const uintptr_t key = reinterpret_cast<uintptr_t>(d_buf);
+  TmapCacheEntry &ce = c->tmap_cache[((key >> 4) ^ (key >> 12) ^ rows ^ uint64_t(box_rows)) % kTmapCacheEntries];
+  if (ce.base == d_buf && ce.rows == rows && ce.box_rows == box_rows) {
+    *map = ce.map;
+    *usable = true;
+    return true;
+  }
   cuuint64_t dims[2] = {128, rows};
   cuuint64_t strides[1] = {128};
   cuuint32_t box[2] = {128, (cuuint32_t)box_rows};
@@ -188,6 +212,10 @@
     c->last_error = "cuTensorMapEncodeTiled failed (" + std::to_string(int(r)) + "); using plain loads";
     return true;
   }
+  ce.base = d_buf;
+  ce.rows = rows;
+  ce.box_rows = box_rows;
+  ce.map = *map;
   *usable = true;
   return true;
 }
@@ -235,7 +263,7 @@
 bool enqueue_scan(sjb200_ctx *c, int kind, const CUtensorMap *map, bool tma, const uint8_t *d_buf, size_t len, uint32_t tile_begin,
                   uint32_t ntiles, bool has_last_tile, uint32_t prev_word, uint32_t *d_idx, uint8_t *d_dst, int carry_in_slot,
                   cudaStream_t stream, int carry_out_slot = -1, bool write_sentinels = false, Carry *external_out = nullptr,
-                  Carry *host_out = nullptr, const XchgTarget *xchg = nullptr) {
+                  Carry *host_out = nullptr, const XchgTarget *xchg = nullptr, bool timed = true) {
   if (carry_out_slot < 0) carry_out_slot = (carry_in_slot < 0) ? 1 : (carry_in_slot ^ 1);
   ScanParams p;
   memset(&p, 0, sizeof(p));
@@ -270,7 +298,7 @@
     }
     if (c->d_debug) { cudaMemsetAsync(c->d_debug, 0, size_t(rows) * 64, stream); p.debug = c->d_debug; c->debug_last_tiles = rows; }
   }
-  cudaEvent_t e1 = time_begin(c, stream);
+  cudaEvent_t e1 = timed ? time_begin(c, stream) : nullptr;
   bool launched;
   if (use_scan4(c, kind)) {
     const uint32_t tpe = uint32_t(scan4_tiles_per_element());
@@ -344,10 +372,10 @@
   bool good = ok(c, cudaStreamCreateWithFlags(&c->stream, cudaStreamNonBlocking), "stream") &&
               ok(c, cudaStreamCreateWithFlags(&c->copy_stream, cudaStreamNonBlocking), "stream") &&
               ok(c, cudaStreamCreateWithFlags(&c->out_stream, cudaStreamNonBlocking), "stream") &&
-              dev_alloc(c, &c->d_carry, kCarrySlots, "cudaMalloc(carry)") && dev_alloc(c, &c->d_flags, 1 + kCarrySlots, "cudaMalloc(flags)") &&
-              dev_alloc(c, &c->d_ticket, 4, "cudaMalloc(ticket)") &&
-              ok(c, cudaMemset(c->d_ticket, 0, 4 * sizeof(uint32_t)), "memset ticket") &&
-              ok(c, cudaMemset(c->d_flags, 0, (1 + kCarrySlots) * sizeof(uint32_t)), "memset flags");
+              dev_alloc(c, &c->d_carry, kCarrySlots, "cudaMalloc(carry)") && dev_alloc(c, &c->d_flags, 2 + kCarrySlots, "cudaMalloc(flags)") &&
+              dev_alloc(c, &c->d_ticket, 8, "cudaMalloc(ticket)") &&
+              ok(c, cudaMemset(c->d_ticket, 0, 8 * sizeof(uint32_t)), "memset ticket") &&
+              ok(c, cudaMemset(c->d_flags, 0, (2 + kCarrySlots) * sizeof(uint32_t)), "memset flags");
   void *hp = nullptr;
   good = good && ok(c, cudaMallocHost(&hp, kCarrySlots * sizeof(Carry)), "cudaMallocHost");
   c->h_carry = static_cast<Carry *>(hp);
@@ -390,7 +418,7 @@
   DeviceGuard g(c->device);
   if (c->stream) cudaStreamSynchronize(c->stream);
   free_sized(c);
-  cudaFree(c->d_carry); cudaFree(c->d_flags); cudaFree(c->d_ticket); cudaFree(c->d_sfin); cudaFree(c->d_doc_scratch); cudaFree(c->d_ndocs); cudaFree(c->d_tok_scratch); cudaFree(c->d_tok_tot); cudaFree(c->d_tails); cudaFree(c->d_tail_ptrs); cudaFree(c->d_debug); cudaFree(c->d_park); cudaFree(c->d_doctab);
+  cudaFree(c->d_carry); cudaFree(c->d_flags); cudaFree(c->d_ticket); cudaFree(c->d_sfin); cudaFree(c->d_doc_scratch); cudaFree(c->d_ndocs); cudaFree(c->d_tok_scratch); cudaFree(c->d_tok_tot); cudaFree(c->d_tails); cudaFree(c->d_tail_ptrs); cudaFree(c->d_debug); cudaFree(c->d_park); cudaFree(c->d_doctab); cudaFree(c->d_stamps);
   if (c->h_doctab) cudaFreeHost(c->h_doctab);
   if (c->h_carry) cudaFreeHost(c->h_carry);
   if (c->h_flags) cudaFreeHost(c->h_flags);
@@ -434,6 +462,14 @@
   return long(n);
 }
 
+extern "C" long sjb200_get_launch_stamps(sjb200_ctx *c, unsigned long long *out, size_t max_launches) {
+  if (!c || !c->d_stamps || !out) return 0;
+  DeviceGuard g(c->device);
+  const size_t n = std::min(max_launches, c->stamps_used);
+  if (cudaDeviceSynchronize() != cudaSuccess || cudaMemcpy(out, c->d_stamps, n * 16, cudaMemcpyDeviceToHost) != cudaSuccess) { (void)cudaGetLastError(); return 0; }
+  return long(n);
+}
+
 extern "C" int sjb200_pin_host_memory(sjb200_ctx *c, void *ptr, size_t bytes) {
   if (!c || !ptr || bytes == 0) return SJB200_UNEXPECTED_ERROR;
   DeviceGuard g(c->device);
@@ -490,6 +526,8 @@
   else if (!strcmp(key, "tok_stage")) c->opt_tok_stage = value ? 1 : 0;
   else if (!strcmp(key, "time_kernel")) c->opt_time_kernel = value;
   else if (!strcmp(key, "debug_timeline")) c->opt_debug_timeline = value;
+  else if (!strcmp(key, "pdl")) c->opt_pdl = value ? 1 : 0;
+  else if (!strcmp(key, "launch_stamps")) c->opt_launch_stamps = value ? 1 : 0;
   else if (!strcmp(key, "chunk_bytes")) c->opt_chunk_bytes = std::max<long>(2 * kTileBytes, (value / (2 * kTileBytes)) * (2 * kTileBytes));
   else if (!strcmp(key, "force_grid")) c->opt_force_grid = value;
   else if (!strcmp(key, "ew_min_bytes")) c->opt_ew_min_bytes = value;
@@ -526,13 +564,15 @@
   return true;
 }
 
-void stage1_stream_epilogue(sjb200_ctx *c, PendingCall &pc) {
+bool stage1_stream_epilogue(sjb200_ctx *c, PendingCall &pc) {
   if (pc.mode == SJB200_STREAMING_PARTIAL || pc.mode == SJB200_STREAMING_FINAL) {
     c->launches++;
     const int slot = pc.carry_slot;
     if (!ok(c, launch_stream_finish(pc.d_buf, pc.d_idx, c->d_carry + slot, uint32_t(pc.len), pc.mode, c->d_sfin + slot, c->h_sfin + slot, pc.stream), "stream finish"))
       pc.early_error = SJB200_UNEXPECTED_ERROR;
-  }
+    return true;
+  }
+  return false;
 }
 
 void stage1_enqueue_into(sjb200_ctx *c, PendingCall &pc, const uint8_t *d_buf, size_t len, int mode, uint32_t *d_idx, cudaStream_t s, int slot) {
@@ -664,21 +704,11 @@
     c->doctab_bytes = off.back();
   }
   static_assert(sizeof(DocEntry) == 64 && sizeof(CUtensorMap) == 128, "table layout");
+  std::vector<uint32_t> g_elems_of(groups.size(), 0), g_tiles_of(groups.size(), 0);
   for (size_t g = 0; g < groups.size(); g++) {
     const std::vector<int> &G = groups[g];
-    if (G.size() == 1) {
-      PendingCall &pc = calls[size_t(G[0])];
-      CUtensorMap map;
-      bool tma = false;
-      map_for(c, kIndex, &map, pc.d_buf, pc.len, &tma);
-      if (!enqueue_scan(c, kIndex, &map, tma, pc.d_buf, pc.len, 0, tiles_of(pc.len), true, 0x20202020u, pc.d_idx, nullptr, -1, s, pc.carry_slot, true,
-                        nullptr, c->h_carry + pc.carry_slot))
-        pc.early_error = SJB200_UNEXPECTED_ERROR;
-      else
-        stage1_stream_epilogue(c, pc);
-      continue;
-    }
     const size_t n = G.size();
+    if (n == 1) continue;
     DocEntry *he = reinterpret_cast<DocEntry *>(c->h_doctab + off[g]);
     const size_t maps_at = off[g] + ((n * sizeof(DocEntry) + 127) & ~size_t(127));
     CUtensorMap *hm = reinterpret_cast<CUtensorMap *>(c->h_doctab + maps_at);
@@ -702,33 +732,82 @@
       elems += e.nelem;
       tiles += tiles_of(pc.len);
     }
+    g_elems_of[g] = elems;
+    g_tiles_of[g] = tiles;
+  }
+  if (off.back() > 0 && !ok(c, cudaMemcpyAsync(c->d_doctab, c->h_doctab, off.back(), cudaMemcpyHostToDevice, s), "H2D doc tables")) return SJB200_UNEXPECTED_ERROR;
+  std::vector<char> early(groups.size(), 1);
+  for (size_t g = 1; g < groups.size(); g++)
+    for (int i : groups[g])
+      for (int j : groups[g - 1])
+        if (ranges_overlap(calls[size_t(i)].d_buf, calls[size_t(i)].len, calls[size_t(j)].d_idx, out_bytes(calls[size_t(j)]))) early[g] = 0;
+  unsigned long long *stamps = nullptr;
+  c->stamps_used = 0;
+  if (c->opt_launch_stamps) {
+    if (c->stamps_cap < groups.size()) {
+      cudaFree(c->d_stamps); c->d_stamps = nullptr; c->stamps_cap = 0;
+      if (!dev_alloc(c, &c->d_stamps, 2 * groups.size(), "cudaMalloc(stamps)")) return SJB200_MEMALLOC;
+      c->stamps_cap = groups.size();
+    }
+    if (!ok(c, cudaMemsetAsync(c->d_stamps, 0, 16 * groups.size(), s), "memset stamps")) return SJB200_UNEXPECTED_ERROR;
+    stamps = c->d_stamps;
+    c->stamps_used = groups.size();
+  }
+  cudaEvent_t e1 = time_begin(c, s);
+  uint32_t timed_docs = 0;
+  bool chained = false;
+  int parity = 0;
+  for (size_t g = 0; g < groups.size(); g++) {
+    const std::vector<int> &G = groups[g];
+    if (G.size() == 1) {
+      PendingCall &pc = calls[size_t(G[0])];
+      CUtensorMap map;
+      bool tma = false;
+      map_for(c, kIndex, &map, pc.d_buf, pc.len, &tma);
+      if (!enqueue_scan(c, kIndex, &map, tma, pc.d_buf, pc.len, 0, tiles_of(pc.len), true, 0x20202020u, pc.d_idx, nullptr, -1, s, pc.carry_slot, true,
+                        nullptr, c->h_carry + pc.carry_slot, nullptr, false)) {
+        pc.early_error = SJB200_UNEXPECTED_ERROR;
+      } else {
+        timed_docs++;
+        stage1_stream_epilogue(c, pc);
+      }
+      chained = false;
+      continue;
+    }
+    const size_t n = G.size();
     ScanParams p;
     memset(&p, 0, sizeof(p));
     p.prev_word = 0x20202020u;
     p.check_eof = 1;
     p.write_sentinels = 1;
-    p.ntiles = tiles;
-    p.flags = c->d_flags;
-    p.count_desc = c->d_count_desc;
-    p.ticket = c->d_ticket;
+    p.ntiles = g_tiles_of[g];
     p.docs = reinterpret_cast<const DocEntry *>(c->d_doctab + off[g]);
     p.ndocs = uint32_t(n);
-    bool good = next_epoch(c, s, &p.epoch) &&
-                ok(c, cudaMemcpyAsync(c->d_doctab + off[g], c->h_doctab + off[g], off[g + 1] - off[g], cudaMemcpyHostToDevice, s), "H2D doc table");
+    p.early_input = early[g] ? 1u : 0u;
+    p.stamps = stamps ? stamps + 2 * g : nullptr;
+    bool wiped = false;
+    bool good = next_epoch(c, s, &p.epoch, &wiped);
+    const bool pdl = good && chained && !wiped && c->opt_pdl;
+    parity = pdl ? parity ^ 1 : 0;
+    p.flags = launch_flags(c, parity);
+    p.count_desc = launch_desc(c, parity);
+    p.ticket = launch_ticket(c, parity);
     if (good) {
       CUtensorMap unused;
       memset(&unused, 0, sizeof(unused));
-      cudaEvent_t e1 = time_begin(c, s);
-      good = ok(c, launch_scan4(&unused, p, grid_for(c, kIndex, elems), 0, s), "launch scan4 (documents)");
-      time_end(c, s, e1, good, uint32_t(n));
+      good = ok(c, launch_scan4(&unused, p, grid_for(c, kIndex, g_elems_of[g]), 0, s, pdl), "launch scan4 (documents)");
       c->launches += good ? 1 : 0;
-    }
+      timed_docs += good ? uint32_t(n) : 0u;
+    }
+    bool epilogue = false;
     for (size_t k = 0; k < n; k++) {
       PendingCall &pc = calls[size_t(G[k])];
-      if (good) stage1_stream_epilogue(c, pc);
+      if (good) epilogue = stage1_stream_epilogue(c, pc) || epilogue;
       else pc.early_error = SJB200_UNEXPECTED_ERROR;
     }
-  }
+    chained = good && !epilogue;
+  }
+  time_end(c, s, e1, timed_docs > 0, timed_docs);
   return SJB200_SUCCESS;
 }
 }
diff --git a/simdjson_b200/csrc/sjb200_kernels.cu b/simdjson_b200/csrc/sjb200_kernels.cu
--- a/simdjson_b200/csrc/sjb200_kernels.cu
+++ b/simdjson_b200/csrc/sjb200_kernels.cu
@@ -45,7 +45,7 @@
   }
 }
 
-cudaError_t launch_scan4(const CUtensorMap *tmap, const ScanParams &p, int grid, int mode, cudaStream_t stream) {
+cudaError_t launch_scan4(const CUtensorMap *tmap, const ScanParams &p, int grid, int mode, cudaStream_t stream, bool pdl) {
   static bool configured[64] = {};
   int dev = 0;
   cudaGetDevice(&dev);
@@ -54,6 +54,19 @@
     if (e == cudaSuccess) e = cudaFuncSetAttribute(scan4_minify_kernel, cudaFuncAttributeMaxDynamicSharedMemorySize, scan4::kSmemBytes4);
     if (e != cudaSuccess) return e;
     if (dev >= 0 && dev < 64) configured[dev] = true;
+  }
+  if (pdl && mode == 0) {
+    cudaLaunchAttribute attr;
+    attr.id = cudaLaunchAttributeProgrammaticStreamSerialization;
+    attr.val.programmaticStreamSerializationAllowed = 1;
+    cudaLaunchConfig_t cfg = {};
+    cfg.gridDim = dim3(unsigned(grid));
+    cfg.blockDim = dim3(unsigned(scan4::kThreads4));
+    cfg.dynamicSmemBytes = size_t(scan4::kSmemBytes4);
+    cfg.stream = stream;
+    cfg.attrs = &attr;
+    cfg.numAttrs = 1;
+    return cudaLaunchKernelEx(&cfg, scan4_kernel, *tmap, p);
   }
   if (mode == 2) scan4_minify_kernel<<<grid, scan4::kThreads4, scan4::kSmemBytes4, stream>>>(*tmap, p);
   else scan4_kernel<<<grid, scan4::kThreads4, scan4::kSmemBytes4, stream>>>(*tmap, p);
diff --git a/simdjson_b200/csrc/sjb200_kernels.cuh b/simdjson_b200/csrc/sjb200_kernels.cuh
--- a/simdjson_b200/csrc/sjb200_kernels.cuh
+++ b/simdjson_b200/csrc/sjb200_kernels.cuh
@@ -9,7 +9,7 @@
 namespace sjb200 {
 
 cudaError_t launch_scan4(const CUtensorMap *tmap, const ScanParams &p, int grid, int mode ,
-                         cudaStream_t stream);
+                         cudaStream_t stream, bool pdl = false);
 size_t scan4_park_words(int grid);
 int scan4_tiles_per_element();
 int scan4_parks_in_global();
diff --git a/simdjson_b200/csrc/sjb200_params.h b/simdjson_b200/csrc/sjb200_params.h
--- a/simdjson_b200/csrc/sjb200_params.h
+++ b/simdjson_b200/csrc/sjb200_params.h
@@ -64,6 +64,8 @@
   uint32_t xchg_kind;
   const DocEntry *docs;
   uint32_t ndocs;
+  uint32_t early_input;
+  unsigned long long *stamps;
 };
 
 #if defined(__CUDACC__)
diff --git a/simdjson_b200/csrc/sjb200_scan4.cuh b/simdjson_b200/csrc/sjb200_scan4.cuh
--- a/simdjson_b200/csrc/sjb200_scan4.cuh
+++ b/simdjson_b200/csrc/sjb200_scan4.cuh
@@ -109,13 +109,27 @@
   return r;
 }
 
+SJ_DEV void wait_previous_launch() {
+  sj_griddep_wait();
+  sj_griddep_launch_dependents();
+}
+
+SJ_DEV bool spun_out(uint32_t *spins) {
+  const uint32_t s = ++*spins;
+  if ((s & 0x7FFFFFFFu) <= kSpinLimit4) return false;
+  if (s & 0x80000000u) return true;
+  sj_griddep_wait();
+  *spins = 0x80000000u;
+  return false;
+}
+
 #ifndef SJB200_SCAN4_POLL_SCALE
 #define SJB200_SCAN4_POLL_SCALE 1
 #endif
 SJ_DEV bool wait_bar(sj_mbar_t *bar, uint32_t parity, const ScanParams &p, unsigned ns) {
   uint32_t spins = 0;
   while (!sj_mbar_try_wait(bar, parity)) {
-    if (++spins > kSpinLimit4) {
+    if (spun_out(&spins)) {
       sj_atomic_or(p.flags, kFlagInternal);
       return false;
     }
@@ -739,6 +753,7 @@
     SJ_TRACE4(6);
     SJ_TRACE4(7);
     if (!kEmitW && j >= uint32_t(kLag)) {
+      if (j == uint32_t(kLag)) wait_previous_launch();
       wait_bar(&S->resolved[ne % kNS], (ne / kNS) & 1u, p, 64);
       SJ_TRACE4(8);
       if (!SJB200_SCAN4_TRACE && p.debug != nullptr && warp == 0 && lane == 0) p.debug[uint64_t(S->ticket[ne % kNS]) * 8 + 2] = sj_globaltimer();
@@ -762,6 +777,7 @@
     sj_syncwarp();
     emit_role<kMode>(S, tmap, p, cin, lane, S->ring[warp][0], &S->full[warp][0], full_phase & 1u);
   } else {
+    if (ne < j) wait_previous_launch();
     while (ne < j) {
       wait_bar(&S->resolved[ne % kNS], (ne / kNS) & 1u, p, 64);
       if (kMin) {
@@ -783,6 +799,7 @@
   const uint64_t out_base = cin.count;
   const uint64_t launch_start = uint64_t(p.tile_begin) * kTileBytes;
   uint32_t *stg = reinterpret_cast<uint32_t *>(stage);
+  wait_previous_launch();
   for (;;) {
     uint32_t q = 0;
     if (lane == 0) q = sj_atomic_add(&S->emit_next, 1u);
@@ -793,7 +810,7 @@
       if (sj_mbar_try_wait(&S->resolved[e % kNS], (e / kNS) & 1u)) break;
       const uint32_t done = sj_ld_acquire_u32(&S->scan_done);
       if (done != 0xFFFFFFFFu && e >= done) return;
-      if (++spins > kSpinLimit4) {
+      if (spun_out(&spins)) {
         sj_atomic_or(p.flags, kFlagInternal);
         return;
       }
@@ -866,7 +883,7 @@
         needed = (1u << nk) - 1u;
       }
       if (!sj_any((pend & needed) != 0)) break;
-      if (++spins > kSpinLimit4) {
+      if (spun_out(&spins)) {
         sj_atomic_or(p.flags, kFlagInternal);
         break;
       }
@@ -977,7 +994,10 @@
     sj_syncwarp();
     if (lane == 0) sj_mbar_arrive(&S->resolved[ns]);
     if (!SJB200_SCAN4_TRACE && p.debug != nullptr && lane == 0) p.debug[uint64_t(t) * 8 + 4] = sj_globaltimer();
-    if (t == D.first_elem + D.nelem - 1) finalize_launch(p, D, cin, s_out, cin.count + base + mine_total, lane);
+    if (t == D.first_elem + D.nelem - 1) {
+      wait_previous_launch();
+      finalize_launch(p, D, cin, s_out, cin.count + base + mine_total, lane);
+    }
   }
 }
 
@@ -994,10 +1014,16 @@
   }
 #endif
   uint32_t first_ticket = 0;
-  if (tid == 0) first_ticket = sj_atomic_add(p.ticket, 1u);
+  unsigned long long t_entry = 0;
+  if (tid == 0) {
+    if (p.stamps != nullptr) t_entry = sj_globaltimer();
+    first_ticket = sj_atomic_add(p.ticket, 1u);
+  }
+  if (p.carry_in != nullptr || !p.early_input) wait_previous_launch();
   Carry cin;
   cin.count = 0; cin.state = 0; cin.ttable = 0; cin.flags = 0; cin.reserved = 0;
   if (p.carry_in != nullptr) cin = *p.carry_in;
+  if (tid == 0 && p.stamps != nullptr && first_ticket == 0) p.stamps[0] = t_entry;
   if (tid < unsigned(kNS)) {
     sj_mbar_init(&S->ticket_ready[tid], 1);
     sj_mbar_init(&S->scanned[tid], 1);
@@ -1064,6 +1090,7 @@
     sj_threadfence();
     const uint32_t done = sj_atomic_add(p.ticket + 1, 1u);
     if (done == sj_nctas() - 1) {
+      wait_previous_launch();
       p.ticket[0] = 0;
       p.ticket[1] = 0;
       p.ticket[2] = 0;
@@ -1085,6 +1112,7 @@
           sj_st_sys_u64(rec + 1, w1);
         }
       }
+      if (p.stamps != nullptr) p.stamps[1] = sj_globaltimer();
       sj_threadfence();
     }
   }
diff --git a/simdjson_b200/csrc/sjb200_simt.cuh b/simdjson_b200/csrc/sjb200_simt.cuh
--- a/simdjson_b200/csrc/sjb200_simt.cuh
+++ b/simdjson_b200/csrc/sjb200_simt.cuh
@@ -25,11 +25,18 @@
   pthread_barrier_t bar;
   uint8_t *smem;
 };
+struct GridDep {
+  GridDep *prev = nullptr;
+  std::atomic<unsigned> running{0};
+  std::atomic<unsigned> released{0};
+  std::atomic<uint8_t> *cta_released = nullptr;
+};
 struct ThreadCtx {
   unsigned tid = 0, cta = 0, nctas = 0;
   unsigned phase = 0;
   WarpShared *warp = nullptr;
   CtaShared *ctas = nullptr;
+  GridDep *dep = nullptr;
 };
 extern thread_local ThreadCtx tctx;
 
@@ -138,6 +145,19 @@
   return (unsigned long long)ts.tv_sec * 1000000000ull + (unsigned long long)ts.tv_nsec;
 }
 SJ_DEV uint32_t sj_clock32() { return uint32_t(sj_globaltimer()); }
+
+SJ_DEV void sj_griddep_wait() {
+  const simt::GridDep *d = simt::tctx.dep;
+  if (d == nullptr || d->prev == nullptr) return;
+  while (d->prev->running.load(std::memory_order_acquire) != 0) {
+    struct timespec ts = {0, 20000};
+    nanosleep(&ts, nullptr);
+  }
+}
+SJ_DEV void sj_griddep_launch_dependents() {
+  simt::GridDep *d = simt::tctx.dep;
+  if (d != nullptr && d->cta_released[simt::tctx.cta].exchange(1) == 0) d->released.fetch_add(1);
+}
 
 struct sj_tensor_map {
   const uint8_t *base;
@@ -297,6 +317,8 @@
   return t;
 }
 SJ_DEV uint32_t sj_clock32() { return uint32_t(clock64()); }
+SJ_DEV void sj_griddep_wait() { asm volatile("griddepcontrol.wait;" ::: "memory"); }
+SJ_DEV void sj_griddep_launch_dependents() { asm volatile("griddepcontrol.launch_dependents;" ::: "memory"); }
 
 typedef CUtensorMap sj_tensor_map;
 typedef unsigned long long sj_mbar_t;
diff --git a/simdjson_b200/implementation.py b/simdjson_b200/implementation.py
--- a/simdjson_b200/implementation.py
+++ b/simdjson_b200/implementation.py
@@ -6,6 +6,8 @@
 from .capi import (CAPACITY, EMPTY, MEMALLOC, REGULAR, SUCCESS, UNEXPECTED_ERROR, UNSUPPORTED_ARCHITECTURE, UTF8_ERROR)
 
 _LIB = None
+_DOC_DTYPE = np.dtype([("d_buf", np.uint64), ("len", np.uint64), ("d_idx", np.uint64), ("n_structural_indexes", np.uint32), ("error", np.int32)])
+assert _DOC_DTYPE.itemsize == C.sizeof(capi.Doc) and all(_DOC_DTYPE.fields[f][1] == getattr(capi.Doc, f).offset for f, _ in capi.Doc._fields_)
 
 
 def lib():
@@ -125,16 +127,14 @@
 
     def stage1_device_batch(self, d_bufs, d_idxs, mode=REGULAR, stream=None):
         n = len(d_bufs)
-        docs = (capi.Doc * n)()
-        for i in range(n):
-            docs[i].d_buf = d_bufs[i].data_ptr()
-            docs[i].len = d_bufs[i].numel()
-            docs[i].d_idx = d_idxs[i].data_ptr()
-            docs[i].n_structural_indexes = 0
-        rc = lib().sjb200_stage1_dev_batch(self._ctx, docs, n, mode, _stream_ptr(stream))
+        docs = np.zeros(n, dtype=_DOC_DTYPE)
+        docs["d_buf"] = [b.data_ptr() for b in d_bufs]
+        docs["len"] = [b.numel() for b in d_bufs]
+        docs["d_idx"] = [t.data_ptr() for t in d_idxs]
+        rc = lib().sjb200_stage1_dev_batch(self._ctx, docs.ctypes.data_as(C.POINTER(capi.Doc)), n, mode, _stream_ptr(stream))
         if rc != SUCCESS:
             raise RuntimeError("sjb200_stage1_dev_batch failed: " + self.last_cuda_error())
-        return [(docs[i].error, docs[i].n_structural_indexes) for i in range(n)]
+        return list(zip(docs["error"].tolist(), docs["n_structural_indexes"].tolist()))
 
     def stage1_device_enqueue(self, d_buf, mode=REGULAR, d_idx=None, stream=None):
         if d_idx is None:
```

New measurement: 1050, median of 6. +9.0%, better.
